# PaddlePaddle/Anakin

Hardware: AMD Instinct MI355X
Metric: ResNet50 INT8 images/sec + p50 latency @ batch 1/8, 1×MI355X (higher is better)
Workload: dtype int8

## Files before the change

### anakin_amd/csrc/api_chain.hip

```cpp
#include "api_internal.h"

enum : unsigned { CK_1X1 = 1, CK_3X3 = 2, CK_HEAD = 4, CK_PAIR = 8, CK_LED = CK_3X3 | CK_HEAD, CK_ANY = 15 };
static unsigned chain_kind(const saber_hip_chain* ch) { return !ch->c3 ? CK_1X1 : (ch->b2 ? CK_PAIR : (ch->b ? CK_3X3 : CK_HEAD)); }
static const struct { int c1; unsigned kinds; ChainForm f; } chain_forms[] = {
    {64, CK_ANY,            {4, 4, 4, 1, 1, CS_BASE, false}},
    {64, CK_ANY,            {2, 2, 4, 1, 1, CS_BASE, false}},
    {128, CK_1X1 | CK_LED,  {2, 2, 4, 1, 1, CS_BASE, false}},
    {128, CK_1X1 | CK_LED,  {1, 1, 4, 1, 1, CS_BASE, false}},
    {128, CK_1X1 | CK_LED,  {6, 2, 8, 1, 1, CS_W8, false}},
    {128, CK_1X1 | CK_LED,  {5, 1, 8, 1, 1, CS_W8, false}},
    {256, CK_1X1 | CK_LED,  {1, 1, 4, 1, 1, CS_BASE, false}},
    {256, CK_1X1,           {9, 1, 4, 2, 1, CS_SPLIT, false}},
    {256, CK_1X1,           {11, 1, 8, 2, 1, CS_SPLIT8, false}},
    {256, CK_LED,           {3, 1, 8, 1, 1, CS_W8, false}},
    {256, CK_3X3,           {7, 1, 8, 1, 2, CS_COOP2, true}},
    {256, CK_3X3,           {15, 2, 8, 1, 4, CS_COOP4, true}},
    {512, CK_1X1,           {1, 1, 4, 1, 1, CS_BASE, false}},
    {512, CK_1X1,           {9, 1, 4, 2, 1, CS_SPLIT, false}},
};
static void for_each_chain_form(const saber_hip_chain* ch, const std::function<void(const ChainForm&)>& fn) {
    for (const auto& r : chain_forms)
        if (r.c1 == ch->c1 && (r.kinds & chain_kind(ch))) fn(r.f);
}
static ChainForm chain_form_where(const saber_hip_chain* ch, const std::function<bool(const ChainForm& row, const ChainForm& found)>& take) {
    ChainForm f;
    for_each_chain_form(ch, [&](const ChainForm& c) { if (take(c, f)) f = c; });
    return f;
}
ChainForm chain_form(const saber_hip_chain* ch, int code) { return chain_form_where(ch, [&](const ChainForm& c, const ChainForm&) { return c.code == code; }); }
ChainForm chain_form_default(const saber_hip_chain* ch) { return chain_form_where(ch, [](const ChainForm&, const ChainForm& f) { return !f.code; }); }
ChainForm chain_form_plain(const saber_hip_chain* ch) { return chain_form_where(ch, [](const ChainForm& c, const ChainForm&) { return !c.placement; }); }
bool chain_form_valid(const saber_hip_chain* ch, int code) {
    const ChainForm f = chain_form(ch, code);
    return f.code && ch->d_stream[f.stream].p && (f.coop != 4 || ch->stage1);
}
std::string chain_form_name(const saber_hip_chain* ch) {
    const ChainForm& f = ch->form;
    const std::string c = std::to_string(ch->c1), w8 = f.waves == 8 && f.coop == 1 ? "_w8" : "";
    if (!ch->c3) return "chain1x1_c" + c + "_px" + std::to_string(16 * f.rows) + (f.split == 2 ? "_split2" : "") + w8;
    return std::string("conv3x3+") + (ch->b2 ? "conv1x1+pair1x1_c" : (ch->b ? "chain1x1_c" : "conv1x1_c")) + c + "_" + std::to_string(f.rows) + "x16" + w8 +
           (f.coop == 2 ? "_coop2" : "") + (f.coop == 4 ? "_coop4" : "");
}
void for_each_chain_candidate(const saber_hip_chain* ch, bool shared_device, const std::function<void(const ChainForm&)>& fn) {
    for_each_chain_form(ch, [&](const ChainForm& c) { if (!(shared_device && c.placement) && chain_form_valid(ch, c.code)) fn(c); });
}

static bool chain_1x1(const saber_hip_conv* o, bool sub_res_ok = false) {
    const saber_hip_conv_desc& d = o->d;
    return o->is_i8 && o->weights_set && !o->gpool && o->algo == ALGO_IGEMM_I8 && o->epi == EPI_I8_CONV && d.kh == 1 && d.kw == 1 &&
           d.stride_h == 1 && d.stride_w == 1 && d.pad_h == 0 && d.pad_w == 0 && d.group == 1 && !o->pair_k2 &&
           !o->pool_fused && !o->pool2 && !o->pre_quant && !o->pre_pad && o->c_eff == d.c && d.act_negative_slope == 0.f &&
           d.in_layout == SABER_HIP_NHWC && d.out_layout == SABER_HIP_NHWC && (d.res_stride <= 1 || sub_res_ok);
}
static void pack_chain_params(const saber_hip_conv* o, size_t chunks_pad, std::vector<uint8_t>& out) {
    const int K = o->d.k;
    out.assign(chunks_pad * 16, 0);
    for (int k4 = 0; k4 < K / 4; ++k4) {
        float* f = (float*)(out.data() + (size_t)k4 * 48);
        int* ip = (int*)(out.data() + (size_t)k4 * 48 + 32);
        for (int r = 0; r < 4; ++r) {
            const int k = k4 * 4 + r;
            f[r] = o->scale_host.empty() ? 1.f : o->scale_host[k];
            f[4 + r] = (o->has_bias && !o->bias_p_host.empty()) ? o->bias_p_host[k] : 0.f;
            ip[r] = o->comp_host.empty() ? 0 : o->comp_host[k];
        }
    }
}
static void pack_chain_weights(const int8_t* w, int K, int C, int mfg, int wave, std::vector<uint8_t>& out, int kbase = 0,
                               int nw = 4, int ks0 = 0) {
    const int kw = K / nw, groups = kw / (16 * mfg), ksn = C / 64;
    for (int g = 0; g < groups; ++g)
        for (int ksi = 0; ksi < ksn; ++ksi)
            for (int mf = 0; mf < mfg; ++mf) {
                const int ks = (ks0 + ksi) % ksn;
                for (int lane = 0; lane < 64; ++lane) {
                    const int rho = lane & 15, kq = lane >> 4;
                    const int ch = kbase + wave * kw + g * 16 * mfg + (rho >> 2) * 4 * mfg + mf * 4 + (rho & 3);
                    const int8_t* src = w + (size_t)ch * C + ks * 64 + kq * 16;
                    out.insert(out.end(), (const uint8_t*)src, (const uint8_t*)src + 16);
                }
            }
}
static void pack_chain_weights3(const int8_t* w, int C, int wave, std::vector<uint8_t>& out, int nw = 4, int kbase = 0, int kcount = 0) {
    const int kw = (kcount ? kcount : C) / nw, mf0 = kw / 16, ksn = C / 64;
    for (int tap = 0; tap < 9; ++tap)
        for (int ks = 0; ks < ksn; ++ks)
            for (int mf = 0; mf < mf0; ++mf)
                for (int lane = 0; lane < 64; ++lane) {
                    const int rho = lane & 15, kq = lane >> 4;
                    const int ch = kbase + wave * kw + (rho >> 2) * 4 * mf0 + mf * 4 + (rho & 3);
                    for (int t = 0; t < 16; ++t) {
                        const int c = ks * 64 + kq * 16 + t;
                        out.push_back((uint8_t)w[((size_t)ch * C + c) * 9 + tap]);
                    }
                }
}
static void pack_frag1(const int8_t* w, int C, int ch_base, int mfg, int mf, int ks, std::vector<uint8_t>& out) {
    for (int lane = 0; lane < 64; ++lane) {
        const int rho = lane & 15, kq = lane >> 4;
        const int8_t* src = w + (size_t)(ch_base + (rho >> 2) * 4 * mfg + mf * 4 + (rho & 3)) * C + ks * 64 + kq * 16;
        out.insert(out.end(), (const uint8_t*)src, (const uint8_t*)src + 16);
    }
}
static void pack_frag3(const int8_t* w, int C, int ch_base, int tap, int ks, std::vector<uint8_t>& out) {
    for (int lane = 0; lane < 64; ++lane) {
        const int rho = lane & 15, kq = lane >> 4;
        for (int t = 0; t < 16; ++t) out.push_back((uint8_t)w[((size_t)(ch_base + rho) * C + ks * 64 + kq * 16 + t) * 9 + tap]);
    }
}
static void pack_coop4_stream(const saber_hip_conv* c3, const saber_hip_conv* a, const saber_hip_conv* b, std::vector<uint8_t>& out) {
    const int C = 256, K1 = 1024;
    for (int q = 0; q < 4; ++q)
        for (int w = 0; w < 8; ++w) {
            const int nt = w & 3, kh = w >> 2;
            for (int tap = 0; tap < 9; ++tap)
                for (int kl = 0; kl < 2; ++kl) pack_frag3(c3->wq_oihw.data(), C, q * 64 + nt * 16, tap, kh * 2 + kl, out);
            for (int i = 0; i < 4; ++i)
                for (int mf = 0; mf < 2; ++mf) pack_frag1(a->wq_oihw.data(), C, q * 256 + w * 32, 2, mf, (q + i) & 3, out);
            for (int jj = 0; b && jj < 8; ++jj) {
                const int j = jj < 2 ? kh * 2 + jj : 4 + kh * 6 + (jj - 2);
                pack_frag1(b->wq_oihw.data(), K1, q * 64 + nt * 16, 1, 0, (q * 4 + j) & 15, out);
            }
        }
}
static void pack_stage_head_stream(const saber_hip_conv* a, const saber_hip_conv* b, std::vector<uint8_t>& out) {
    const int C0 = 512;
    for (int q = 0; q < 4; ++q)
        for (int w = 0; w < 8; ++w) {
            const int nt = w & 3, kh = w >> 2;
            for (int ks = 0; ks < 8; ++ks)
                for (int mf = 0; mf < 2; ++mf) pack_frag1(a->wq_oihw.data(), C0, q * 256 + w * 32, 2, mf, ks, out);
            for (int j = 0; j < 4; ++j) pack_frag1(b->wq_oihw.data(), C0, q * 64 + nt * 16, 1, 0, kh * 4 + j, out);
        }
}
static void pack_stage1_c128_stream(const saber_hip_conv* c3, const saber_hip_conv* a, const saber_hip_conv* b, std::vector<uint8_t>& out) {
    const int C = 128, K1 = 512;
    for (int w = 0; w < 8; ++w) {
        for (int tap = 0; tap < 9; ++tap)
            for (int ks = 0; ks < 2; ++ks) pack_frag3(c3->wq_oihw.data(), C, w * 16, tap, ks, out);
        for (int ks = 0; ks < 2; ++ks)
            for (int mf = 0; mf < 4; ++mf) pack_frag1(a->wq_oihw.data(), C, w * 64, 4, mf, ks, out);
        for (int ks = 0; ks < 8; ++ks) pack_frag1(b->wq_oihw.data(), K1, w * 16, 1, 0, ks, out);
    }
}
int saber_hip_conv2d_stem_pair_create(saber_hip_conv_t* stem, const saber_hip_conv_t* a, const saber_hip_conv_t* b, saber_hip_stem_pair_t** out) {
    if (!stem || !a || !b || !out) return fail(SABER_HIP_INVALID_VALUE, "null argument");
    const saber_hip_conv_desc& ds = stem->d;
    if (!stem->pool_fused || !stem->weights_set || ds.k != 64 || (ds.out_dtype != SABER_HIP_U8 && ds.out_dtype != SABER_HIP_S8))
        return fail(SABER_HIP_INVALID_VALUE, "stem pair: the head must be the fused stem conv + max pooling with 64 output channels (8-bit)");
    auto plain1x1 = [&](const saber_hip_conv* o) {
        const saber_hip_conv_desc& d = o->d;
        return o->is_i8 && o->weights_set && o->algo == ALGO_IGEMM_I8 && o->epi == EPI_I8_CONV && d.res_mode == SABER_HIP_RES_NONE &&
               !o->pair_k2 && !o->pool_fused && !o->pool2 && !o->pre_quant && !o->pre_pad && d.kh == 1 && d.kw == 1 && d.stride_h == 1 &&
               d.stride_w == 1 && d.pad_h == 0 && d.pad_w == 0 && d.group == 1 && d.c == 64 && o->c_eff == 64 && d.k % 32 == 0 &&
               d.in_layout == SABER_HIP_NHWC && d.out_layout == SABER_HIP_NHWC && d.act_negative_slope == 0.f &&
               (d.out_dtype == SABER_HIP_S8 || d.out_dtype == SABER_HIP_U8) && d.n == ds.n && d.h == stem->pool_oh && d.w == stem->pool_ow &&
               (o->x_dtype == DT_U8) == (ds.out_dtype == SABER_HIP_U8) && (int)o->wq_oihw.size() == d.k * 64;
    };
    if (!plain1x1(a) || !plain1x1(b) || a->d.k + b->d.k > 320)
        return fail(SABER_HIP_INVALID_VALUE, "stem pair: two plain 1x1 / stride-1 INT8 convs (64 -> k, k % 32 == 0, k_a + k_b <= 320, 8-bit NHWC outputs) "
                                              "on the pooled tensor");
    auto* sp = new saber_hip_stem_pair();
    sp->stem = stem; sp->a = a; sp->b = b;
    const int K1 = a->d.k, Kt = K1 + b->d.k;
    std::vector<int8_t> wcat((size_t)Kt * 64);
    std::memcpy(wcat.data(), a->wq_oihw.data(), (size_t)K1 * 64);
    std::memcpy(wcat.data() + (size_t)K1 * 64, b->wq_oihw.data(), (size_t)b->d.k * 64);
    std::vector<uint8_t> w, pa, pb, prm(256 * 16, 0);
    w.reserve((size_t)Kt * 64);
    for (int g = 0; g < Kt / 32; ++g)
        for (int mf = 0; mf < 2; ++mf) pack_frag1(wcat.data(), 64, g * 32, 2, mf, 0, w);
    pack_chain_params(a, (size_t)K1 / 4 * 3, pa);
    pack_chain_params(b, (size_t)b->d.k / 4 * 3, pb);
    std::memcpy(prm.data(), pa.data(), pa.size());
    std::memcpy(prm.data() + pa.size(), pb.data(), pb.size());
    hipError_t e = sp->d_w.upload(w);
    if (e == hipSuccess) e = sp->d_prm.upload(prm);
    if (e != hipSuccess) {
        delete sp;
        return hip_fail(e, "stem pair: device copies");
    }
    *out = sp;
    return SABER_HIP_OK;
}
void saber_hip_conv2d_stem_pair_destroy(saber_hip_stem_pair_t* sp) { delete sp; }
int saber_hip_conv2d_stem_pair_run(saber_hip_stem_pair_t* sp, const void* x, void* y_pool, void* y_a, void* y_b, void* workspace,
                                   saber_hip_stream_t stream) {
    if (g_capture) return capture_unsupported("saber_hip_conv2d_stem_pair_run (an executor-level object: saber_hip_net_optimize forms it itself)");
    if (!sp || !x || !y_a || !y_b) return fail(SABER_HIP_INVALID_VALUE, "null argument");
    saber_hip_conv* op = sp->stem;
    if (op->ws_bytes && !workspace) return fail(SABER_HIP_INVALID_VALUE, "workspace required");
    saber_mi355x::StemPairKArgs ka;
    const int rc = stem_pool_args(op, x, y_pool, workspace, (hipStream_t)stream, &ka.c);
    if (rc) return rc;
    ka.t.w = sp->d_w.p; ka.t.prm = sp->d_prm.p; ka.t.y1 = y_a; ka.t.y2 = y_b;
    ka.t.K1 = sp->a->d.k; ka.t.K2 = sp->b->d.k;
    ka.t.relu1 = sp->a->d.act == SABER_HIP_ACT_RELU; ka.t.relu2 = sp->b->d.act == SABER_HIP_ACT_RELU;
    ka.t.u8_1 = sp->a->d.out_dtype == SABER_HIP_U8; ka.t.u8_2 = sp->b->d.out_dtype == SABER_HIP_U8;
    HIP_TRY(saber_mi355x::launch_conv_stem_pool_pair(op->pre_quant ? 1 : 0, ka, (hipStream_t)stream));
    return SABER_HIP_OK;
}
saber_hip_chain::~saber_hip_chain() {
    if (h_coop_err) (void)hipHostFree(h_coop_err);
    delete stage1;
}
static unsigned div_magic(int d) { return d >= 2 ? (unsigned)((0x100000000ull + (unsigned)d - 1) / (unsigned)d) : 0u; }
static int stage_build(saber_hip_chain* const* chains, int n, bool per_image, saber_hip_chain* tail, saber_hip_chain_stage** out,
                       const saber_hip_conv* head_a = nullptr, const saber_hip_conv* head_b = nullptr) {
    if (!chains || n <= 0 || n > saber_mi355x::STAGE4_LONG || !out) return fail(SABER_HIP_INVALID_VALUE, "stage: 1..24 chains");
    if (head_a || head_b) {
        if (!head_a || !head_b) return fail(SABER_HIP_INVALID_VALUE, "null argument");
        if (!chains[0] || chains[0]->c1 != 256) return fail(SABER_HIP_INVALID_VALUE, "stage: a head goes with a C = 256 stage only");
        if (!per_image) return fail(SABER_HIP_INVALID_VALUE, "stage: a head needs an image per XCD");
        for (const saber_hip_conv* o : {head_a, head_b})
            if (o->d.res_mode != SABER_HIP_RES_NONE) return fail(SABER_HIP_INVALID_VALUE, "stage: the head's convs carry no residual");
        for (const saber_hip_conv* o : {head_a, head_b}) {
            const saber_hip_conv_desc& d = o->d;
            if (!o->is_i8 || !o->weights_set || o->algo != ALGO_IGEMM_I8 || o->epi != EPI_I8_CONV || o->pair_k2 || o->pool_fused || o->pool2 || o->gpool ||
                o->pre_quant || o->pre_pad || d.kh != 1 || d.kw != 1 || d.stride_h != 1 || d.stride_w != 1 || d.pad_h != 0 || d.pad_w != 0 || d.group != 1 ||
                o->c_eff != d.c || d.act_negative_slope != 0.f || d.in_layout != SABER_HIP_NHWC || d.out_layout != SABER_HIP_NHWC ||
                (d.out_dtype != SABER_HIP_S8 && d.out_dtype != SABER_HIP_U8))
                return fail(SABER_HIP_INVALID_VALUE, "stage: the head must be two plain 1x1 / stride 1 / pad 0 INT8 NHWC convs with weights set");
        }
        if (head_a->d.c != 512 || head_b->d.c != 512) return fail(SABER_HIP_INVALID_VALUE, "stage: the head's convs read 512 channels");
        if (head_a->d.k != 1024 || head_b->d.k != 256) return fail(SABER_HIP_INVALID_VALUE, "stage: the head's convs write 1024 and 256 channels");
        const saber_hip_conv_desc &d0 = chains[0]->a->d, &da = head_a->d, &db = head_b->d;
        if (!chains[0]->c3 || da.n != d0.n || da.h != d0.h || da.w != d0.w || db.n != d0.n || db.h != d0.h || db.w != d0.w || head_a->x_dtype != head_b->x_dtype ||
            da.out_dtype != SABER_HIP_S8 || (db.out_dtype == SABER_HIP_U8) != (chains[0]->c3->x_dtype == DT_U8))
            return fail(SABER_HIP_INVALID_VALUE, "stage: the head's outputs must be the first block's shortcut (s8) and 3x3 input (its dtype), one input tensor");
    }
    if (tail) {
        if (!chains[0] || chains[0]->c1 != 256 || tail->c1 != 256) return fail(SABER_HIP_INVALID_VALUE, "stage: a tail goes with a C = 256 stage only");
        if (n < 2 || !per_image || n + 1 > saber_mi355x::STAGE4_LONG) return fail(SABER_HIP_INVALID_VALUE, "stage: a tail needs 2..23 blocks, an image per XCD");
        if (!tail->c3 || tail->b || tail->b2 || tail->c3->d.stride_h != 2 || tail->c3->d.stride_w != 2)
            return fail(SABER_HIP_INVALID_VALUE, "stage: the tail must be a conv3x3 / stride 2 + conv1x1 chain without a second 1x1 conv");
        if (tail->a->d.res_stride != 2) return fail(SABER_HIP_INVALID_VALUE, "stage: the tail's shortcut must be sub-sampled by 2");
    }
    if (n > 1 && !per_image) return fail(SABER_HIP_INVALID_VALUE, "stage: several blocks need an image per XCD");
    if (n < 2 && chains[0] && chains[0]->c1 == 128) return fail(SABER_HIP_INVALID_VALUE, "stage: at C = 128 a stage is at least two blocks");
    const saber_hip_chain* c0 = chains[0];
    std::vector<saber_mi355x::StageBlk> blk;
    for (int k = 0; k < n; ++k) {
        const saber_hip_chain* ch = chains[k];
        const uint8_t* stream = !ch ? nullptr : (ch->c1 == 256 ? ch->d_stream[CS_COOP4].p : (ch->c1 == 128 ? ch->d_stream_stage1.p : nullptr));
        if (!ch || ch->c1 != c0->c1 || !ch->c3 || !ch->b || !stream || ch->c3->d.stride_h != 1)
            return fail(SABER_HIP_INVALID_VALUE, "stage: every block must be a conv3x3 (stride 1) + conv1x1 + conv1x1 chain at C = 256 (or all at C = 128)");
        const saber_hip_conv_desc& da = ch->a->d;
        if (da.n != c0->a->d.n || da.h != c0->a->d.h || da.w != c0->a->d.w) return fail(SABER_HIP_INVALID_VALUE, "stage: blocks of one tensor shape");
        if (k && ((ch->c3->x_dtype == DT_U8) != (chains[k - 1]->b->d.out_dtype == SABER_HIP_U8)))
            return fail(SABER_HIP_INVALID_VALUE, "stage: a block's 3x3 conv reads what the previous block's last conv writes");
        saber_mi355x::StageBlk B;
        std::memset(&B, 0, sizeof B);
        B.wstream = stream; B.prm0 = ch->d_prm0.p; B.prm1 = ch->d_prm1.p; B.prm2 = ch->d_prm2.p;
        B.coeff_conv = da.coeff_conv; B.scale_conv = ch->a->out_scale; B.coeff_res = da.coeff_res; B.scale_res = da.scale_res;
        B.in0_u8 = ch->c3->x_dtype == DT_U8; B.relu0 = ch->c3->d.act == SABER_HIP_ACT_RELU;
        B.in_u8 = ch->a->x_dtype == DT_U8; B.relu1 = da.act == SABER_HIP_ACT_RELU; B.res_relu = da.res_act == SABER_HIP_ACT_RELU;
        B.relu2 = ch->b->d.act == SABER_HIP_ACT_RELU; B.out_u8_2 = ch->b->d.out_dtype == SABER_HIP_U8;
        blk.push_back(B);
    }
    const saber_hip_conv_desc& d0 = c0->a->d;
    if (tail) {
        const saber_hip_conv_desc &d3 = tail->c3->d, &da = tail->a->d;
        if (d3.n != d0.n || d3.h != d0.h || d3.w != d0.w || da.res_h != d0.h || da.res_w != d0.w)
            return fail(SABER_HIP_INVALID_VALUE, "stage: the tail's 3x3 conv and shortcut read tensors of the blocks' shape");
        if ((tail->c3->x_dtype == DT_U8) != (chains[n - 1]->b->d.out_dtype == SABER_HIP_U8))
            return fail(SABER_HIP_INVALID_VALUE, "stage: the tail's 3x3 conv reads what the last block's last conv writes");
    }
    saber_hip_chain_stage* st = new saber_hip_chain_stage();
    st->chains.assign(chains, chains + n);
    st->c1 = c0->c1;
    st->n = d0.n; st->h = d0.h; st->w = d0.w;
    st->tiles_x = (d0.w + 15) / 16;
    st->tiles_per_img = st->tiles_x * ((d0.h + 1) / 2);
    st->per_image = per_image;
    const int wg_per_tile = st->c1 == 256 ? 4 : 1;
    const bool fits = d0.n <= 8 && st->tiles_per_img * wg_per_tile <= 32 &&
                      (st->c1 == 256 ? st->tiles_x == 1 : (st->tiles_x == 1 || st->tiles_x == 2 || st->tiles_x == 4));
    if ((per_image && !fits) || (st->c1 == 128 && !per_image)) {
        delete st;
        return fail(SABER_HIP_INVALID_VALUE, "stage: an image per XCD needs batch <= 8 and <= 32 workgroups per image (C = 256: width <= 16, <= 8 tiles "
                    "of 2 x 16 pixels; C = 128: width <= 64, <= 32 tiles)");
    }
    const size_t tiles = (size_t)d0.n * st->tiles_per_img;
    hipError_t e = hipSuccess;
    if (tail) {
        std::vector<uint8_t> ts;
        pack_coop4_stream(tail->c3, tail->a, nullptr, ts);
        e = st->d_tail_stream.upload(ts);
        const saber_hip_conv_desc& da = tail->a->d;
        saber_mi355x::StageBlk B;
        std::memset(&B, 0, sizeof B);
        B.wstream = st->d_tail_stream.p; B.prm0 = tail->d_prm0.p; B.prm1 = tail->d_prm1.p; B.prm2 = tail->d_prm0.p;
        B.coeff_conv = da.coeff_conv; B.scale_conv = tail->a->out_scale; B.coeff_res = da.coeff_res; B.scale_res = da.scale_res;
        B.in0_u8 = tail->c3->x_dtype == DT_U8; B.relu0 = tail->c3->d.act == SABER_HIP_ACT_RELU;
        B.in_u8 = tail->a->x_dtype == DT_U8; B.relu1 = da.act == SABER_HIP_ACT_RELU; B.res_relu = da.res_act == SABER_HIP_ACT_RELU;
        blk.push_back(B);
        st->tail = tail;
    }
    if (head_a) {
        std::vector<uint8_t> hs, p1, p2;
        pack_stage_head_stream(head_a, head_b, hs);
        pack_chain_params(head_a, (size_t)head_a->d.k / 4 * 3, p1);
        pack_chain_params(head_b, ((size_t)head_b->d.k / 4 * 3 + 63) / 64 * 64 + 64, p2);
        if (e == hipSuccess) e = st->d_head_stream.upload(hs);
        if (e == hipSuccess) e = st->d_head_prm1.upload(p1);
        if (e == hipSuccess) e = st->d_head_prm2.upload(p2);
        saber_mi355x::StageBlk B;
        std::memset(&B, 0, sizeof B);
        B.wstream = st->d_head_stream.p; B.prm0 = st->d_head_prm2.p; B.prm1 = st->d_head_prm1.p; B.prm2 = st->d_head_prm2.p;
        B.in_u8 = head_a->x_dtype == DT_U8; B.relu1 = head_a->d.act == SABER_HIP_ACT_RELU;
        B.relu2 = head_b->d.act == SABER_HIP_ACT_RELU; B.out_u8_2 = head_b->d.out_dtype == SABER_HIP_U8;
        blk.insert(blk.begin(), B);
        st->head_a = head_a; st->head_b = head_b;
    }
    if (e == hipSuccess) e = st->d_blk.upload(blk);
    if (e == hipSuccess && st->c1 == 256) e = st->d_grp_ctr.alloc_zero(tiles * 32);
    if (e == hipSuccess) e = st->d_img_ctr.alloc_zero((size_t)d0.n * (st->tiles_per_img + 1) * 16);
    if (e == hipSuccess) e = st->d_xcc.alloc_zero(tiles * 32);
    if (e == hipSuccess && st->c1 == 256) e = st->d_xch.alloc_zero(tiles * 32 * 256);
    if (e == hipSuccess) e = hipHostMalloc((void**)&st->h_err, sizeof(unsigned), hipHostMallocMapped);
    if (e != hipSuccess) {
        delete st;
        return hip_fail(e, "stage: device buffers");
    }
    *st->h_err = 0u;
    *out = st;
    return SABER_HIP_OK;
}
template <int MAXB>
static int stage_launch(saber_hip_chain_stage* st, const void* x, const void* res, void* const* y1, void* const* y2, void* y_tail, void* y_head, hipStream_t s) {
    saber_mi355x::Stage4KArgs<MAXB> k;
    std::memset(&k, 0, sizeof k);
    k.x = x; k.res = res; k.zero = zero_page();
    if (!k.zero) return fail(SABER_HIP_RUNTIME_ERROR, "stage: zero page");
    k.blk = st->d_blk.p + (st->head_a ? 1 : 0); k.grp_ctr = st->d_grp_ctr.p; k.img_ctr = st->d_img_ctr.p; k.xch = st->d_xch.p; k.xcc = st->d_xcc.p; k.err = st->h_err;
    k.nblk = (int)st->chains.size(); k.N = st->n; k.H = st->h; k.W = st->w;
    k.tiles_x = st->tiles_x; k.tiles_per_img = st->tiles_per_img;
    k.mg_tiles_x = div_magic(st->tiles_x); k.mg_tpi = div_magic(st->tiles_per_img); k.mg_wpi = div_magic(st->tiles_per_img * 4);
    k.per_image = st->per_image;
    for (int i = 0; i < k.nblk; ++i) { k.y1[i] = y1[i]; k.y2[i] = y2[i]; }
    if (y_tail) k.y1[k.nblk] = y_tail;
    k.head_y = y_head;
    HIP_TRY(st->c1 == 256 ? saber_mi355x::launch_conv_stage4(k, y_tail != nullptr, y_head != nullptr, s) : saber_mi355x::launch_conv_stage1_c128(k, s));
    return SABER_HIP_OK;
}
int stage_run(saber_hip_chain_stage* st, const void* x, const void* res, void* const* y1, void* const* y2, hipStream_t s, void* y_tail, void* y_head) {
    if (y_tail && !st->tail) return fail(SABER_HIP_INVALID_VALUE, "stage: created without a tail");
    if (y_head && !st->head_a) return fail(SABER_HIP_INVALID_VALUE, "stage: created without a head");
    if (*(volatile unsigned*)st->h_err) {
        *(volatile unsigned*)st->h_err = 0u;
        return fail(SABER_HIP_RUNTIME_ERROR, "cooperative stage: an earlier launch's workgroups did not share an XCD or timed out at a barrier "
                    "(its outputs are not valid)");
    }
    return (int)st->chains.size() + (y_tail ? 1 : 0) <= saber_mi355x::STAGE4_SHORT ? stage_launch<saber_mi355x::STAGE4_SHORT>(st, x, res, y1, y2, y_tail, y_head, s)
                                                                                   : stage_launch<saber_mi355x::STAGE4_LONG>(st, x, res, y1, y2, y_tail, y_head, s);
}
int saber_hip_conv2d_stage_create(saber_hip_chain_t* const* chains, int n, saber_hip_chain_stage_t** out) {
    if (!xcd_round_robin()) return fail(SABER_HIP_UNIMPL, "stage: this device does not place workgroup b on XCD b % 8");
    return stage_build(chains, n, true, nullptr, out);
}
int saber_hip_conv2d_stage_create_tail(saber_hip_chain_t* const* chains, int n, saber_hip_chain_t* tail, saber_hip_chain_stage_t** out) {
    if (!tail) return fail(SABER_HIP_INVALID_VALUE, "null argument");
    if (!xcd_round_robin()) return fail(SABER_HIP_UNIMPL, "stage: this device does not place workgroup b on XCD b % 8");
    return stage_build(chains, n, true, tail, out);
}
int saber_hip_conv2d_stage_create_head(saber_hip_chain_t* const* chains, int n, saber_hip_chain_t* tail, const saber_hip_conv_t* head_a,
                                       const saber_hip_conv_t* head_b, saber_hip_chain_stage_t** out) {
    if (!head_a || !head_b) return fail(SABER_HIP_INVALID_VALUE, "null argument");
    if (!xcd_round_robin()) return fail(SABER_HIP_UNIMPL, "stage: this device does not place workgroup b on XCD b % 8");
    return stage_build(chains, n, true, tail, out, head_a, head_b);
}
void saber_hip_conv2d_stage_destroy(saber_hip_chain_stage_t* st) { delete st; }
int saber_hip_conv2d_stage_run(saber_hip_chain_stage_t* st, const void* x, const void* res, void* const* y1, void* const* y2, saber_hip_stream_t stream) {
    if (g_capture) return capture_unsupported("saber_hip_conv2d_stage_run (saber_hip_net_optimize forms stages itself)");
    if (!st || !x || !res || !y1 || !y2) return fail(SABER_HIP_INVALID_VALUE, "null argument");
    for (size_t i = 0; i < st->chains.size(); ++i)
        if (!y1[i] || !y2[i]) return fail(SABER_HIP_INVALID_VALUE, "stage: an output pointer per block");
    return stage_run(st, x, res, y1, y2, (hipStream_t)stream);
}
int saber_hip_conv2d_stage_run_tail(saber_hip_chain_stage_t* st, const void* x, const void* res, void* const* y1, void* const* y2, void* y_tail,
                                    saber_hip_stream_t stream) {
    if (g_capture) return capture_unsupported("saber_hip_conv2d_stage_run_tail (saber_hip_net_optimize forms stages itself)");
    if (!st || !x || !res || !y1 || !y2 || !y_tail) return fail(SABER_HIP_INVALID_VALUE, "null argument");
    for (size_t i = 0; i < st->chains.size(); ++i)
        if (!y1[i] || !y2[i]) return fail(SABER_HIP_INVALID_VALUE, "stage: an output pointer per block");
    return stage_run(st, x, res, y1, y2, (hipStream_t)stream, y_tail);
}
int saber_hip_conv2d_stage_run_head(saber_hip_chain_stage_t* st, const void* x_head, void* y_head_b, void* const* y1, void* const* y2, void* y_tail,
                                    saber_hip_stream_t stream) {
    if (g_capture) return capture_unsupported("saber_hip_conv2d_stage_run_head (saber_hip_net_optimize forms stages itself)");
    if (!st || !x_head || !y_head_b || !y1 || !y2) return fail(SABER_HIP_INVALID_VALUE, "null argument");
    for (size_t i = 0; i < st->chains.size(); ++i)
        if (!y1[i] || !y2[i]) return fail(SABER_HIP_INVALID_VALUE, "stage: an output pointer per block");
    return stage_run(st, x_head, nullptr, y1, y2, (hipStream_t)stream, y_tail, y_head_b);
}
static void pack_chain_stream(const saber_hip_chain* ch, ChainStream layout, std::vector<uint8_t>& out) {
    const saber_hip_conv *c3 = ch->c3, *a = ch->a, *b = ch->b;
    const int c = ch->c1, k1 = ch->k1, k2 = ch->k2, c2 = b ? b->d.c : 0, k2w = k2 / 2;
    const int nw = layout == CS_BASE || layout == CS_SPLIT ? 4 : 8;
    const int8_t *w3 = c3 ? c3->wq_oihw.data() : nullptr, *wa = a->wq_oihw.data(), *wb = b ? b->wq_oihw.data() : nullptr;
    std::vector<int8_t> wcat;
    if (ch->b2) {
        wcat.assign(b->wq_oihw.begin(), b->wq_oihw.end());
        wcat.insert(wcat.end(), ch->b2->wq_oihw.begin(), ch->b2->wq_oihw.end());
        wb = wcat.data();
    }
    auto mfg = [&](int k) { return ch->b2 ? 2 : std::min(4, k / nw / 16); };
    switch (layout) {
    case CS_BASE: case CS_W8:
        for (int w = 0; w < nw; ++w) {
            if (c3) pack_chain_weights3(w3, c, w, out, nw);
            pack_chain_weights(wa, k1, c, 4, w, out, 0, nw);
            if (b) pack_chain_weights(wb, k2, c2, mfg(k2), w, out, 0, nw);
        }
        break;
    case CS_SPLIT: case CS_SPLIT8:
        for (int half = 0; half < 2; ++half)
            for (int w = 0; w < nw; ++w) {
                pack_chain_weights(wa, k1, c, 4, w, out, 0, nw);
                pack_chain_weights(wb, k2w, c2, mfg(k2w), w, out, half * k2w, nw);
            }
        break;
    case CS_COOP2:
        for (int half = 0; half < 2; ++half)
            for (int w = 0; w < nw; ++w) {
                pack_chain_weights3(w3, c, w, out, nw, half * (c / 2), c / 2);
                pack_chain_weights(wa, k1 / 2, c, 4, w, out, half * (k1 / 2), nw, half * (c / 128));
                pack_chain_weights(wb, k2w, c2, 1, w, out, half * k2w, nw, half * (c2 / 128));
            }
        break;
    default: pack_coop4_stream(c3, a, b, out);
    }
}
static int chain_build(saber_hip_conv* c3, saber_hip_conv* a, saber_hip_conv* b, saber_hip_chain_t** out, saber_hip_conv* b2 = nullptr) {
    if (!a || !out || (!b && !c3) || (b2 && (!b || !c3))) return fail(SABER_HIP_INVALID_VALUE, "null argument");
    const bool pair2 = b2 != nullptr;
    const bool strided = c3 && (!b || pair2) && c3->d.stride_h == 2 && c3->d.stride_w == 2;
    if (pair2 && !strided) return fail(SABER_HIP_INVALID_VALUE, "chain: a sibling pair follows the strided head (conv3x3 / stride 2 + conv1x1 + eltwise) only");
    if (!chain_1x1(a, strided) || (b && !chain_1x1(b)) || (b2 && !chain_1x1(b2)))
        return fail(SABER_HIP_INVALID_VALUE, "chain: both ops must be plain 1x1 stride-1 INT8 NHWC convs with weights set");
    if (strided != (a->d.res_stride > 1) || (strided && a->d.res_stride != 2))
        return fail(SABER_HIP_INVALID_VALUE, "chain: a stride-2 head goes with a shortcut sub-sampled by 2 (and only with one)");
    const saber_hip_conv_desc& da = a->d;
    if (da.res_mode != SABER_HIP_RES_ELTWISE || da.out_dtype != SABER_HIP_S8 || (da.res_has_dtype && da.res_dtype != SABER_HIP_S8))
        return fail(SABER_HIP_INVALID_VALUE, "chain: the first conv must carry the fused eltwise epilogue with s8 residual and output");
    if (b) {
        const saber_hip_conv_desc& db = b->d;
        if (db.res_mode != SABER_HIP_RES_NONE || b->x_dtype != DT_S8 || (db.out_dtype != SABER_HIP_S8 && db.out_dtype != SABER_HIP_U8))
            return fail(SABER_HIP_INVALID_VALUE, "chain: the second conv must be a plain s8-input conv with an 8-bit output");
        if (db.n != da.n || db.h != a->oh || db.w != a->ow || db.c != da.k || (!pair2 && db.k != da.c))
            return fail(SABER_HIP_INVALID_VALUE, "chain: shapes must be C -> 4C -> C with C in {64,128,256,512} on the same pixels");
    }
    if (pair2) {
        const saber_hip_conv_desc &db = b->d, &d2 = b2->d;
        if (d2.res_mode != SABER_HIP_RES_NONE || b2->x_dtype != DT_S8 || (d2.out_dtype != SABER_HIP_S8 && d2.out_dtype != SABER_HIP_U8) || d2.n != da.n ||
            d2.h != a->oh || d2.w != a->ow || d2.c != da.k || da.c != 64 || db.k % 32 || db.k + d2.k != 640 || d2.k <= 0)
            return fail(SABER_HIP_INVALID_VALUE, "chain: the sibling pair after a strided head: 64 -> 256 (+ eltwise) -> k_b | k_b2 with k_b + k_b2 = 640, k_b % 32 == 0, 8-bit outputs");
    }
    if (!conv1x1_chain_ok(da.c, da.k, da.c))
        return fail(SABER_HIP_INVALID_VALUE, "chain: shapes must be C -> 4C -> C with C in {64,128,256,512} on the same pixels");
    if (c3) {
        const saber_hip_conv_desc& d3 = c3->d;
        const bool ok = c3->is_i8 && c3->weights_set && c3->algo == ALGO_IGEMM_I8 && c3->epi == EPI_I8_CONV && d3.kh == 3 && d3.kw == 3 &&
                        d3.stride_h == (strided ? 2 : 1) && d3.stride_w == d3.stride_h && d3.pad_h == 1 && d3.pad_w == 1 && d3.dil_h == 1 && d3.dil_w == 1 &&
                        d3.group == 1 && !c3->pair_k2 && !c3->pool_fused && !c3->pool2 && !c3->pre_quant && !c3->pre_pad &&
                        c3->c_eff == d3.c && d3.act_negative_slope == 0.f && d3.in_layout == SABER_HIP_NHWC &&
                        d3.out_layout == SABER_HIP_NHWC && d3.res_mode == SABER_HIP_RES_NONE && d3.c == da.c && d3.k == da.c &&
                        d3.n == da.n && c3->oh == da.h && c3->ow == da.w && da.c <= 256 &&
                        (d3.out_dtype == SABER_HIP_S8 || d3.out_dtype == SABER_HIP_U8) &&
                        (d3.out_dtype == SABER_HIP_U8) == (a->x_dtype == DT_U8);
        if (!ok) return fail(SABER_HIP_INVALID_VALUE, "chain: the head must be the 3x3 pad-1 INT8 conv (C -> C, C <= 256; stride 1, or 2 in front of a lone 1x1 conv) whose 8-bit output the first 1x1 conv reads");
    }
    saber_hip_chain* ch = new saber_hip_chain();
    const int k2 = b ? b->d.k + (pair2 ? b2->d.k : 0) : 0;
    ch->c3 = c3; ch->a = a; ch->b = b; ch->b2 = b2; ch->c1 = da.c; ch->k1 = da.k; ch->k2 = k2;
    ch->form = chain_form_default(ch);
    std::vector<uint8_t> p0, p1, p2;
    hipError_t e = hipSuccess;
    for (int l = 0; l < CS_COUNT && e == hipSuccess; ++l) {
        bool needed = false;
        for_each_chain_form(ch, [&](const ChainForm& f) { needed = needed || (f.stream == l && (!f.placement || xcd_round_robin())); });
        if (!needed) continue;
        std::vector<uint8_t> stream;
        pack_chain_stream(ch, (ChainStream)l, stream);
        e = ch->d_stream[l].upload(stream);
    }
    pack_chain_params(a, (size_t)da.k / 4 * 3, p1);
    if (b) pack_chain_params(b, ((size_t)k2 / 4 * 3 + 63) / 64 * 64 + 64, p2);
    if (pair2) {
        std::vector<uint8_t> pb2;
        pack_chain_params(b2, (size_t)b2->d.k / 4 * 3, pb2);
        std::memcpy(p2.data() + (size_t)b->d.k / 4 * 48, pb2.data(), pb2.size());
    }
    if (e == hipSuccess && ch->d_stream[CS_COOP2].p) {
        ch->coop_tiles = da.n * da.h * ((da.w + 15) / 16);
        e = ch->d_coop_ctr.alloc_zero((size_t)ch->coop_tiles * 32);
        if (e == hipSuccess) e = ch->d_coop_xcc.alloc_zero((size_t)ch->coop_tiles * 32);
        if (e == hipSuccess) e = ch->d_coop_xch.alloc_zero((size_t)ch->coop_tiles * 16 * da.c);
        if (e == hipSuccess) e = hipHostMalloc((void**)&ch->h_coop_err, sizeof(unsigned), hipHostMallocMapped);
        if (e == hipSuccess) *ch->h_coop_err = 0u;
    }
    if (e == hipSuccess && da.c == 128 && c3 && b && c3->d.stride_h == 1 && xcd_round_robin()) {
        std::vector<uint8_t> s1;
        pack_stage1_c128_stream(c3, a, b, s1);
        e = ch->d_stream_stage1.upload(s1);
    }
    if (e == hipSuccess) e = ch->d_prm1.upload(p1);
    if (e == hipSuccess && b) e = ch->d_prm2.upload(p2);
    if (e == hipSuccess && c3) {
        pack_chain_params(c3, ((size_t)da.c / 4 * 3 + 63) / 64 * 64 + 64, p0);
        e = ch->d_prm0.upload(p0);
    }
    if (e != hipSuccess) {
        delete ch;
        return hip_fail(e, "chain: device copies");
    }
    if (ch->d_stream[CS_COOP4].p) {
        const int rc = stage_build(&ch, 1, false, nullptr, &ch->stage1);
        if (rc != SABER_HIP_OK) {
            delete ch;
            return rc;
        }
    }
    *out = ch;
    return SABER_HIP_OK;
}
int saber_hip_conv2d_chain_create(saber_hip_conv_t* a, saber_hip_conv_t* b, saber_hip_chain_t** out) {
    if (!b) return fail(SABER_HIP_INVALID_VALUE, "null argument");
    return chain_build(nullptr, a, b, out);
}
int saber_hip_conv2d_chain_create3(saber_hip_conv_t* conv3x3, saber_hip_conv_t* a, saber_hip_conv_t* b, saber_hip_chain_t** out) {
    if (!conv3x3) return fail(SABER_HIP_INVALID_VALUE, "null argument");
    return chain_build(conv3x3, a, b, out);
}
int saber_hip_conv2d_chain_create3_pair(saber_hip_conv_t* conv3x3, saber_hip_conv_t* a, saber_hip_conv_t* pair_a, saber_hip_conv_t* pair_b,
                                        saber_hip_chain_t** out) {
    if (!conv3x3 || !pair_a || !pair_b) return fail(SABER_HIP_INVALID_VALUE, "null argument");
    return chain_build(conv3x3, a, pair_a, out, pair_b);
}
void saber_hip_conv2d_chain_destroy(saber_hip_chain_t* ch) { delete ch; }
int saber_hip_conv2d_chain_set_tile(saber_hip_chain_t* ch, int tn) {
    if (!ch) return fail(SABER_HIP_INVALID_VALUE, "null argument");
    if (!chain_form_valid(ch, tn)) return fail(SABER_HIP_INVALID_VALUE, "chain: no kernel form with that code for this chain");
    ch->form = chain_form(ch, tn);
    return SABER_HIP_OK;
}
int saber_hip_conv2d_chain_get_tile(const saber_hip_chain_t* ch) { return ch ? ch->form.code : 0; }
int saber_hip_conv2d_chain_run(saber_hip_chain_t* ch, const void* x, const void* res, void* y_a, void* y_b,
                               saber_hip_stream_t stream) {
    return saber_hip_conv2d_chain_run3(ch, x, res, y_a, y_b, nullptr, stream);
}
int saber_hip_conv2d_chain_run3(saber_hip_chain_t* ch, const void* x, const void* res, void* y_a, void* y_b, void* y_c,
                                saber_hip_stream_t stream) {
    if (g_capture) return capture_unsupported("saber_hip_conv2d_chain_run (saber_hip_net_optimize forms chains itself)");
    if (!ch || !x || !res || !y_a || (ch->b && !y_b) || (ch->b2 && !y_c)) return fail(SABER_HIP_INVALID_VALUE, "null argument");
    const saber_hip_conv *a = ch->a, *b = ch->b;
    ChainKArgs k;
    std::memset(&k, 0, sizeof k);
    k.x = x; k.res = res;
    const ChainForm f = ch->form;
    k.wstream = ch->d_stream[f.stream].p;
    k.prm1 = ch->d_prm1.p;
    k.prm2 = ch->d_prm2.p;
    k.y1 = y_a; k.y2 = y_b;
    k.M = a->d.n * a->oh * a->ow;
    k.in_u8 = a->x_dtype == DT_U8;
    k.relu1 = a->d.act == SABER_HIP_ACT_RELU;
    k.res_relu = a->d.res_act == SABER_HIP_ACT_RELU;
    k.coeff_conv = a->d.coeff_conv; k.scale_conv = a->out_scale; k.coeff_res = a->d.coeff_res; k.scale_res = a->d.scale_res;
    if (b) {
        k.relu2 = b->d.act == SABER_HIP_ACT_RELU;
        k.out_u8_2 = b->d.out_dtype == SABER_HIP_U8;
    }
    if (ch->b2) {
        k.y2b = y_c;
        k.k2_split = b->d.k;
        k.relu2b = ch->b2->d.act == SABER_HIP_ACT_RELU;
        k.out_u8_2b = ch->b2->d.out_dtype == SABER_HIP_U8;
    }
    if (ch->c3) {
        k.prm0 = ch->d_prm0.p;
        k.zero = zero_page();
        if (!k.zero) return fail(SABER_HIP_RUNTIME_ERROR, "chain: zero page");
        k.N = a->d.n; k.H = a->d.h; k.W = a->d.w;
        k.tiles_x = (k.W + 15) / 16;
        k.tiles_per_img = k.tiles_x * ((k.H + f.rows - 1) / f.rows);
        k.mg_tiles_x = div_magic(k.tiles_x);
        k.mg_tpi = div_magic(k.tiles_per_img);
        k.in0_u8 = ch->c3->x_dtype == DT_U8;
        k.relu0 = ch->c3->d.act == SABER_HIP_ACT_RELU;
        k.s0 = ch->c3->d.stride_h;
        k.H0 = ch->c3->d.h; k.W0 = ch->c3->d.w;
        if (a->d.res_stride > 1) { k.res_sub = a->d.res_stride; k.res_H = a->d.res_h; k.res_W = a->d.res_w; }
    }
    if (f.coop == 4) {
        const int rc = stage_run(ch->stage1, x, res, &y_a, &y_b, (hipStream_t)stream);
        if (rc != SABER_HIP_OK) ch->form = chain_form_plain(ch);
        return rc;
    }
    if (f.coop == 2) {
        if (*(volatile unsigned*)ch->h_coop_err) {
            *(volatile unsigned*)ch->h_coop_err = 0u;
            ch->form = chain_form_plain(ch);
            return fail(SABER_HIP_RUNTIME_ERROR, "cooperative chain: an earlier launch's workgroup pairs did not share an XCD or timed out at their "
                        "barrier (its outputs are not valid); the chain now runs the single-workgroup form");
        }
        const CoopKArgs ck{k, ch->d_coop_ctr.p, ch->d_coop_xch.p, ch->d_coop_xcc.p, ch->h_coop_err, ch->coop_tiles};
        HIP_TRY(launch_conv_chain_coop(ck, (hipStream_t)stream));
        return SABER_HIP_OK;
    }
    HIP_TRY(launch_conv1x1_chain(k, ch->c1, ch->k1, ch->k2, f.rows, f.waves, f.split, ch->c3 ? 1 : 0, (hipStream_t)stream));
    return SABER_HIP_OK;
}
```

### anakin_amd/csrc/api_internal.h

```cpp
#pragma once
#include "../../include/saber_hip.h"
#include "kernels.h"

#include <cmath>
#include <cstdio>
#include <algorithm>
#include <cstdlib>
#include <cstring>
#include <functional>
#include <memory>
#include <mutex>
#include <string>
#include <utility>
#include <type_traits>
#include <vector>

using namespace saber_mi355x;

namespace saber_api {

extern thread_local std::string g_err;
inline int fail(int code, const std::string& msg) {
    g_err = msg;
    return code;
// ... 197 lines not shown
    DevBuf<uint8_t> d_head_stream, d_head_prm1, d_head_prm2;
    DevBuf<saber_mi355x::StageBlk> d_blk;
    DevBuf<unsigned long long> d_grp_ctr, d_img_ctr;
    DevBuf<uint8_t> d_xch;
    DevBuf<unsigned> d_xcc;
    unsigned* h_err = nullptr;
    int c1 = 0, n = 0, h = 0, w = 0, tiles_x = 0, tiles_per_img = 0;
    bool per_image = false;
    ~saber_hip_chain_stage() {
        if (h_err) (void)hipHostFree(h_err);
    }
};

struct saber_hip_sep {
    saber_hip_conv* dw = nullptr;
    saber_hip_conv* pw = nullptr;
    int form = 0;
    DevBuf<uint8_t> d_wdw, d_wpw, d_prm;
    DevBuf<float> d_dw_bias, d_dw_scale;
    std::string name;
};

struct saber_hip_ir {
    saber_hip_conv* expand = nullptr;
    saber_hip_conv* dw = nullptr;
    saber_hip_conv* project = nullptr;
    int form = 0;
    DevBuf<uint8_t> d_we, d_eprm, d_wdw, d_wp, d_pprm;
    DevBuf<float> d_dw_bias, d_dw_scale;
    std::string name;
};

struct saber_hip_fire {
    saber_hip_conv* squeeze = nullptr;
    saber_hip_conv* e1 = nullptr;
    saber_hip_conv* e3 = nullptr;
    int form = 0;
    DevBuf<uint8_t> d_ws, d_sprm, d_w1, d_prm1, d_w3, d_prm3;
    std::string name;
};

struct saber_hip_fc {
    saber_hip_fc_desc d;
    saber_hip_conv* conv = nullptr;
    bool pre_quant = false;
    float in_scale = 1.f;
};

namespace saber_api {
struct EventPair {
    hipEvent_t e0 = nullptr, e1 = nullptr;
    hipError_t init() {
        hipError_t e = hipEventCreate(&e0);
        return e != hipSuccess ? e : hipEventCreate(&e1);
    }
    ~EventPair() {
        if (e0) (void)hipEventDestroy(e0);
        if (e1) (void)hipEventDestroy(e1);
    }
};
struct ColdBench {
    size_t kBytes = (size_t)64 << 20;
    void* buf = nullptr;
    std::vector<hipEvent_t> ev;
    int reps = 0;
    hipError_t init(int r, size_t bytes = 0) {
        if (bytes) kBytes = std::min<size_t>(std::max<size_t>(bytes, (size_t)64 << 20), (size_t)512 << 20) & ~(size_t)0xfffff;
        reps = r < 3 ? 3 : (r > 32 ? 32 : r);
        hipError_t e = hipMalloc(&buf, kBytes + 256);
        if (e != hipSuccess) return e;
        e = hipMemset(buf, 1, kBytes + 256);
        if (e != hipSuccess) return e;
        ev.assign(2 * (size_t)reps, nullptr);
        for (hipEvent_t& x : ev)
            if ((e = hipEventCreate(&x)) != hipSuccess) return e;
        return hipStreamSynchronize(nullptr);
    }
    ~ColdBench() {
        for (hipEvent_t x : ev)
            if (x) (void)hipEventDestroy(x);
        if (buf) (void)hipFree(buf);
    }
    float run(hipStream_t s, const std::function<int()>& fn) {
        if (fn() != 0) return -1.f;
        for (int r = 0; r < reps; ++r) {
            if (launch_l2_flush(buf, kBytes, (unsigned*)((char*)buf + kBytes), s) != hipSuccess) return -1.f;
            if (hipEventRecord(ev[2 * r], s) != hipSuccess) return -1.f;
            if (fn() != 0) return -1.f;
            if (hipEventRecord(ev[2 * r + 1], s) != hipSuccess) return -1.f;
        }
        if (hipEventSynchronize(ev[2 * reps - 1]) != hipSuccess) return -1.f;
        std::vector<float> t(reps);
        for (int r = 0; r < reps; ++r)
            if (hipEventElapsedTime(&t[r], ev[2 * r], ev[2 * r + 1]) != hipSuccess) return -1.f;
        std::sort(t.begin(), t.end());
        return t[reps / 2] * 1000.f;
    }
};

extern thread_local ColdBench* g_cold;
int time_enqueued(hipStream_t s, const std::function<int()>& fn, int warm_iters, float* t);
extern thread_local std::vector<unsigned long long>* g_used_kernels;
constexpr float g_reuse_tol = 0.03f;
struct ColdScope {
    ColdBench local;
    bool owner = false;
    hipError_t enter(int reps, size_t flush_bytes = 0) {
        const char* w = std::getenv("SABER_HIP_AUTOTUNE_WARM");
        if (w && w[0] == '1') return hipSuccess;
        if (g_cold) return hipSuccess;
        hipError_t e = local.init(reps, flush_bytes);
        if (e != hipSuccess) return e;
        g_cold = &local;
        owner = true;
        return hipSuccess;
    }
    ~ColdScope() {
        if (owner) g_cold = nullptr;
    }
};

}

namespace saber_api {
enum OpKind { OP_CONV, OP_CONV_PAIR, OP_FC, OP_QUANT, OP_DEQUANT, OP_TRANSPOSE_IN, OP_ELT_I8, OP_ELT_F32, OP_POOL_I8, OP_POOL_F32, OP_POOL_F32_I8, OP_FC_Q, OP_SOFTMAX, OP_RELU_F32, OP_ACT_F32, OP_CONCAT };
enum Launch { LAUNCH_NONE, LAUNCH_OWN, LAUNCH_CHAIN, LAUNCH_CHAIN3, LAUNCH_STAGE, LAUNCH_STEM_PAIR, LAUNCH_SEP, LAUNCH_IR, LAUNCH_FIRE };
struct NetOp {
    OpKind kind;
    std::string name;
    saber_hip_conv* conv = nullptr;
    saber_hip_fc* fc = nullptr;
    int in = -1, in2 = -1, out = -1, out2 = -1;
    std::vector<int> ins, cat_c;
    std::vector<float> cat_m;
    Launch launch = LAUNCH_OWN;
    int absorbed_by = -1;
    bool skip = false;
    std::string res_note;
    saber_hip_chain* chain = nullptr;
    int chain_out = -1;
    bool chain_on = false;
    saber_hip_chain* chain3 = nullptr;
    int chain3_res = -1, chain3_y1 = -1, chain3_y2 = -1;
    int chain3_y3 = -1;
    bool led_on = false;
    saber_hip_chain_stage* stage = nullptr;
    int stage_n = 0;
    bool stage_on = false;
    bool stage_name_kept = false;
    bool tail_on = false;
    int tail_of = -1;
    bool head_on = false;
    int head_of = -1;
    saber_hip_stem_pair* stem_pair = nullptr;
    int stem_y1 = -1, stem_y2 = -1;
    saber_hip_sep* sep = nullptr;
    int sep_out = -1;
    bool sep_on = false;
    saber_hip_ir* ir = nullptr;
    int ir_out = -1;
    bool ir_on = false;
    saber_hip_fire* fire = nullptr;
    int fire_out = -1;
    bool fire_on = false;
    int lane = 0;
    bool record = false;
    int p[16] = {0};
    float f[6] = {0};
    size_t count = 0;
};
template <typename F>
inline void op_for_each_input(const NetOp& o, F&& f) {
    if (o.kind == OP_CONCAT) {
        for (int t : o.ins) f(t);
        return;
    }
    if (o.in >= 0) f(o.in);
    if (o.in2 >= 0) f(o.in2);
}
inline int op_reads(const NetOp& o, int t) {
    int n = 0;
    op_for_each_input(o, [&](int u) { n += u == t; });
    return n;
}
inline bool op_touches(const NetOp& o, int t) { return op_reads(o, t) || o.out == t || o.out2 == t; }
}

struct saber_hip_net {
    std::vector<size_t> tensor_bytes;
    std::vector<size_t> tensor_off;
    std::vector<void*> tensor_ext;
    std::vector<std::pair<const void*, int>> captured_ptr;
    void* ptr(int id) const {
        if (id < 0) return nullptr;
        if ((size_t)id < tensor_ext.size() && tensor_ext[id]) return tensor_ext[id];
        return (void*)(arena + tensor_off[id]);
    }
    std::vector<NetOp> ops;
    char* arena = nullptr;
    size_t arena_bytes = 0, ws_off = 0, ws_bytes = 0;
    hipGraph_t graph = nullptr;
    hipGraphExec_t exec = nullptr;
    bool finalized = false;
    bool compacted = false;
    bool shared_device = false;
    bool reproducible_fp32 = false;
    bool inplace_external = false;
    int coop_fallbacks = 0;
    hipStream_t side = nullptr;
    hipEvent_t ev_start = nullptr, ev_join = nullptr;
    std::vector<hipEvent_t> ev_op;
    std::vector<int> writer;
    bool lanes_ready = false, has_side = false;
    std::vector<saber_hip_conv*> owned;
    std::vector<saber_hip_chain*> owned_chains;
    std::vector<saber_hip_chain_stage*> owned_stages;
    std::vector<saber_hip_stem_pair*> owned_stem_pairs;
    std::vector<saber_hip_sep*> owned_seps;
    std::vector<saber_hip_ir*> owned_irs;
    std::vector<saber_hip_fire*> owned_fires;
};

namespace saber_api {
struct Capture;
extern thread_local Capture* g_capture;
int capture_conv(saber_hip_conv* op, const void* x, void* y, const void* res);
int capture_fc(saber_hip_fc* fc, const void* x, float* y, bool quantised_input);
int capture_unsupported(const char* what);
int capture_concat(size_t pixels, int n_inputs, const void* const* xs, const int* channels, const float* mult, int dtype, void* y);
int capture_stream_op(OpKind kind, const char* name, const int* p, int np, const float* f, int nf, size_t count, const void* in,
                      size_t in_bytes, const void* in2, size_t in2_bytes, void* out, size_t out_bytes, void* out2, size_t out2_bytes);
}

bool sel_valid(const saber_hip_conv* op, const saber_api::ConvSel& s);
int sel_set(saber_hip_conv* op, const saber_api::ConvSel& s);
void sel_release_unused(saber_hip_conv* op);
void sel_name(saber_hip_conv* op);
unsigned long long sel_kernel_key(const saber_hip_conv* op, const saber_api::ConvSel& s);
int sel_launch(saber_hip_conv* op, saber_mi355x::ConvKArgs& a, hipStream_t s);
void for_each_candidate(const saber_hip_conv* op, const saber_api::ConvSel* best, const std::function<void(const saber_api::ConvSel&)>& fn);
bool dw_ok(const saber_hip_conv* op);
bool group_ok(const saber_hip_conv* op);
bool stem_ok(const saber_hip_conv* op);
bool fc_small_ok(const saber_hip_conv* op);
bool b3_tile_ok(const saber_hip_conv* op, int tile, int ks);
int dw_static_form(const saber_hip_conv* op);
int group_static_form(const saber_hip_conv* op);
constexpr long DW_STRIP_MIN_LANES = 150000;
void conv_fill_args(const saber_hip_conv* op, saber_mi355x::ConvKArgs& a, const void* x, void* y, const void* res);
int stem_pool_args(const saber_hip_conv* op, const void* x, void* y, void* workspace, hipStream_t s, saber_mi355x::ConvKArgs* a);
bool xcd_round_robin();
int split_prepare(saber_hip_conv* op);
bool img_conv_ok(const saber_hip_conv* op);
int img_conv_prepare(saber_hip_conv* op);
int pw_prepare(saber_hip_conv* op);
bool pw_eligible(const saber_hip_conv* op);
int img_conv_run(saber_hip_conv* op, const void* x, void* y, const void* res, void* y_pool, hipStream_t stream);
void img_conv_release(saber_hip_conv* op);
int net_launch(saber_hip_net* net, const NetOp& o, hipStream_t s);
bool fc_softmax_ok(const saber_hip_fc* fc, bool quantised_input = false);
int fc_run_softmax(saber_hip_fc* fc, const void* x, float* y, float* prob, void* workspace, hipStream_t s, bool quantised_input);
int fc_softmax_prepare(saber_hip_fc* fc);
int concat_check(int n_inputs, const int* channels, const float* mult, int dtype, int* row_bytes);
void net_resolve(saber_hip_net* net);
void net_drop_graph(saber_hip_net* net);
void net_set_chain_mode(saber_hip_net* net, int ia, int mode);
int net_chain_mode(const saber_hip_net* net, int ia);
void net_set_stage(saber_hip_net* net, int i0, bool on);
void net_set_head(saber_hip_net* net, int i0, bool on);
void net_set_tail(saber_hip_net* net, int i0, bool on);
ChainForm chain_form(const saber_hip_chain* ch, int code);
bool chain_form_valid(const saber_hip_chain* ch, int code);
ChainForm chain_form_default(const saber_hip_chain* ch);
ChainForm chain_form_plain(const saber_hip_chain* ch);
std::string chain_form_name(const saber_hip_chain* ch);
void for_each_chain_candidate(const saber_hip_chain* ch, bool shared_device, const std::function<void(const ChainForm&)>& fn);
bool conv_sep_ok(const saber_hip_conv* dw, const saber_hip_conv* pw, std::string* why);
bool sep_form_valid(const saber_hip_sep* sp, int code);
void for_each_sep_form(const saber_hip_sep* sp, const std::function<void(int code)>& fn);
int sep_static_form(const saber_hip_sep* sp);
void net_set_sep(saber_hip_net* net, int i, int code);
bool conv_ir_ok(const saber_hip_conv* expand, const saber_hip_conv* dw, const saber_hip_conv* project, std::string* why);
bool ir_form_valid(const saber_hip_ir* ir, int code);
void for_each_ir_form(const saber_hip_ir* ir, const std::function<void(int code)>& fn);
int ir_static_form(const saber_hip_ir* ir);
void net_set_ir(saber_hip_net* net, int i, int code);
bool conv_fire_ok(const saber_hip_conv* squeeze, const saber_hip_conv* e1, const saber_hip_conv* e3, std::string* why);
bool fire_form_valid(const saber_hip_fire* fr, int code);
void for_each_fire_form(const saber_hip_fire* fr, const std::function<void(int code)>& fn);
int fire_static_form(const saber_hip_fire* fr);
void net_set_fire(saber_hip_net* net, int i, int code);
int stage_run(saber_hip_chain_stage* st, const void* x, const void* res, void* const* y1, void* const* y2, hipStream_t s, void* y_tail = nullptr,
              void* y_head = nullptr);
```

### anakin_amd/csrc/api_net.hip

```cpp
#include "api_internal.h"

#include <atomic>
static std::atomic<int> g_coop_fallbacks_total{0};

void net_drop_graph(saber_hip_net* net) {
    if (net->exec) (void)hipGraphExecDestroy(net->exec);
    if (net->graph) (void)hipGraphDestroy(net->graph);
    net->exec = nullptr;
    net->graph = nullptr;
}
int net_launch(saber_hip_net* net, const NetOp& o, hipStream_t s) {
    auto T = [&](int id) -> void* { return net->ptr(id); };
    void* ws = net->arena + net->ws_off;
    switch (o.kind) {
    case OP_CONV:
        switch (o.launch) {
        case LAUNCH_NONE: return SABER_HIP_OK;
        case LAUNCH_STAGE: {
            void* y1[saber_mi355x::STAGE4_LONG];
            void* y2[saber_mi355x::STAGE4_LONG];
            const NetOp* ops = &o;
            for (int k = 0; k < o.stage_n; ++k) {
                y1[k] = T(ops[3 * k].chain3_y1);
                y2[k] = T(ops[3 * k].chain3_y2);
            }
            void* const y_tail = o.tail_on ? T(ops[3 * o.stage_n].chain3_y1) : nullptr;
            const int rc = o.head_on ? stage_run(o.stage, T(ops[-1].in), nullptr, y1, y2, s, y_tail, T(o.in))
                                     : stage_run(o.stage, T(o.in), T(o.chain3_res), y1, y2, s, y_tail);
            if (rc == SABER_HIP_RUNTIME_ERROR) {
                ++net->coop_fallbacks;
                ++g_coop_fallbacks_total;
                net_set_stage(net, (int)(&o - net->ops.data()), false);
                net_drop_graph(net);
            }
            return rc;
        }
        case LAUNCH_STEM_PAIR: return saber_hip_conv2d_stem_pair_run(o.stem_pair, T(o.in), nullptr, T(o.stem_y1), T(o.stem_y2), ws, s);
        case LAUNCH_CHAIN3: {
            const int rc = saber_hip_conv2d_chain_run3(o.chain3, T(o.in), T(o.chain3_res), T(o.chain3_y1), T(o.chain3_y2), T(o.chain3_y3), s);
            if (rc == SABER_HIP_RUNTIME_ERROR) {
                ++net->coop_fallbacks;
                ++g_coop_fallbacks_total;
            }
            return rc;
        }
        case LAUNCH_CHAIN: return saber_hip_conv2d_chain_run(o.chain, T(o.in), T(o.in2), T(o.out), T(o.chain_out), s);
        case LAUNCH_SEP: return saber_hip_conv2d_sep_run(o.sep, T(o.in), nullptr, T(o.sep_out), s);
        case LAUNCH_IR: return saber_hip_conv2d_ir_run(o.ir, T(o.in), nullptr, nullptr, T(o.ir_out), s);
        case LAUNCH_FIRE: return saber_hip_conv2d_fire_run(o.fire, T(o.in), nullptr, T(o.fire_out), s);
        case LAUNCH_OWN: break;
        }
        if (o.conv->gpool) return saber_hip_conv2d_run_gpool(o.conv, T(o.in), T(o.out), T(o.in2), T(o.out2), s);
        return saber_hip_conv2d_run(o.conv, T(o.in), T(o.out), T(o.in2), ws, s);
    case OP_CONV_PAIR:
        if (o.skip) return SABER_HIP_OK;
        return saber_hip_conv2d_run_pair(o.conv, T(o.in), T(o.out), T(o.out2), s);
    case OP_FC:
        if (o.out2 >= 0) return fc_run_softmax(o.fc, T(o.in), (float*)T(o.out), (float*)T(o.out2), ws, s, false);
        return saber_hip_fc_run(o.fc, T(o.in), (float*)T(o.out), ws, s);
    case OP_QUANT:
        return saber_hip_quantize_nchw_to_nhwc(o.p[0], o.p[1], o.p[2], o.p[3], o.p[4], o.p[5], o.f[0],
                                               (const float*)T(o.in), T(o.out), s);
    case OP_DEQUANT:
        return saber_hip_dequantize_nhwc_to_nchw(o.p[0], o.p[1], o.p[2], o.p[3], o.p[4], o.f[0], T(o.in),
                                                 (float*)T(o.out), s);
    case OP_TRANSPOSE_IN:
        return saber_hip_transpose_nchw_to_nhwc_f32(o.p[0], o.p[1], o.p[2], o.p[3], o.p[4], (const float*)T(o.in),
                                                    (float*)T(o.out), s);
    case OP_ELT_I8:
        return saber_hip_eltwise_sum_i8(o.count, (const int8_t*)T(o.in), (const int8_t*)T(o.in2), o.f[0], o.f[1],
                                        o.f[2], o.f[3], o.p[0], (int8_t*)T(o.out), s);
    case OP_ELT_F32:
        return saber_hip_eltwise_sum_f32(o.count, (const float*)T(o.in), (const float*)T(o.in2), o.f[0], o.f[1],
                                         o.p[0], (float*)T(o.out), s);
    case OP_POOL_I8:
        return saber_hip_pool2d_i8_nhwc(o.p[0], o.p[1], o.p[2], o.p[3], o.p[4], o.p[5], o.p[6], o.p[7], o.p[8],
                                        o.p[9], o.p[10], o.p[11], o.p[12], o.p[13], o.p[14], T(o.in), T(o.out), s);
    case OP_POOL_F32:
        return saber_hip_pool2d_f32(o.p[0], o.p[1], o.p[2], o.p[3], o.p[4], o.p[5], o.p[6], o.p[7], o.p[8], o.p[9],
                                    o.p[10], o.p[11], o.p[12], o.p[13], (const float*)T(o.in), (float*)T(o.out), s);
    case OP_POOL_F32_I8:
        return saber_hip_pool2d_f32_from_i8_q(o.p[0], o.p[1], o.p[2], o.p[3], o.p[4], o.p[5], o.p[6], o.p[7], o.p[8],
                                              o.p[9], o.p[10], o.p[11], o.p[12], o.p[13], o.f[0], T(o.in),
                                              (float*)T(o.out), o.f[1], (int8_t*)T(o.out2), s);
    case OP_FC_Q:
        if (o.out2 >= 0) return fc_run_softmax(o.fc, T(o.in), (float*)T(o.out), (float*)T(o.out2), ws, s, true);
        return saber_hip_fc_run_q(o.fc, (const int8_t*)T(o.in), (float*)T(o.out), s);
    case OP_SOFTMAX:
        if (o.skip) return SABER_HIP_OK;
        return saber_hip_softmax_f32(o.p[0], o.p[1], (const float*)T(o.in), (float*)T(o.out), s);
    case OP_RELU_F32: return saber_hip_relu_f32(o.count, (const float*)T(o.in), (float*)T(o.out), s);
    case OP_ACT_F32: return saber_hip_activation_f32(o.p[0], o.count, o.f[0], o.f[1], (const float*)T(o.in), (float*)T(o.out), s);
    case OP_CONCAT: {
        if (o.skip) return SABER_HIP_OK;
        const void* xs[CONCAT_MAX_INPUTS];
        for (size_t k = 0; k < o.ins.size(); ++k) xs[k] = T(o.ins[k]);
        return saber_hip_concat_nhwc(o.count, (int)o.ins.size(), xs, o.cat_c.data(), o.cat_m.empty() ? nullptr : o.cat_m.data(), o.p[0], T(o.out), s);
    }
    }
    return SABER_HIP_UNIMPL;
}


int saber_hip_net_create(saber_hip_net_t** out) {
    *out = new saber_hip_net();
    return SABER_HIP_OK;
}
int saber_hip_net_add_tensor(saber_hip_net_t* net, size_t bytes) {
    net->tensor_bytes.push_back(bytes);
    net->tensor_ext.push_back(nullptr);
    return (int)net->tensor_bytes.size() - 1;
}
int saber_hip_net_num_tensors(const saber_hip_net_t* net) { return net ? (int)net->tensor_bytes.size() : 0; }
size_t saber_hip_net_tensor_bytes(const saber_hip_net_t* net, int id) {
    return (net && id >= 0 && id < (int)net->tensor_bytes.size()) ? net->tensor_bytes[id] : 0;
}
int saber_hip_net_bind_tensor(saber_hip_net_t* net, int id, void* ptr) {
    if (!net || id < 0 || id >= (int)net->tensor_bytes.size()) return fail(SABER_HIP_INVALID_VALUE, "bad tensor id");
    if (net->finalized && !ptr && !net->tensor_ext[id]) return SABER_HIP_OK;
    if (net->finalized && !net->tensor_ext[id]) return fail(SABER_HIP_INVALID_VALUE, "bind_tensor: an arena tensor cannot become external after finalize");
    if (net->finalized && !ptr) return fail(SABER_HIP_INVALID_VALUE, "bind_tensor: an external tensor has no arena slot to fall back to after finalize");
    net->tensor_ext[id] = ptr;
    net_drop_graph(net);
    return SABER_HIP_OK;
}
int saber_hip_net_tensor_of_ptr(const saber_hip_net_t* net, const void* ptr) {
    if (!net) return -1;
    for (const auto& pr : net->captured_ptr)
        if (pr.first == ptr) return pr.second;
    return -1;
}
static int push(saber_hip_net* net, NetOp&& o) {
    const int nt = (int)net->tensor_bytes.size();
    if (o.in >= nt || o.in2 >= nt || o.out >= nt || o.in < 0 || o.out < 0) return fail(SABER_HIP_INVALID_VALUE, "bad tensor id");
    net->ops.push_back(std::move(o));
    return (int)net->ops.size() - 1;
}
int saber_hip_net_add_conv(saber_hip_net_t* net, saber_hip_conv_t* op, int in_id, int out_id, int res_id) {
    NetOp o;
    o.kind = OP_CONV; o.conv = op; o.in = in_id; o.out = out_id; o.in2 = res_id;
    o.name = std::string("conv:") + op->algo_name;
    if (op->ws_bytes > net->ws_bytes) net->ws_bytes = op->ws_bytes;
    return push(net, std::move(o));
}
int saber_hip_net_add_conv_pair(saber_hip_net_t* net, saber_hip_conv_t* op, int in_id, int out_a_id, int out_b_id) {
    if (!op || !op->pair_k2) return fail(SABER_HIP_INVALID_VALUE, "not a sibling pair");
    if (out_b_id < 0 || out_b_id >= (int)net->tensor_bytes.size()) return fail(SABER_HIP_INVALID_VALUE, "bad tensor id");
    NetOp o;
    o.kind = OP_CONV_PAIR; o.conv = op; o.in = in_id; o.out = out_a_id; o.out2 = out_b_id;
    o.name = std::string("conv:") + op->algo_name;
    return push(net, std::move(o));
}
int saber_hip_net_add_fc(saber_hip_net_t* net, saber_hip_fc_t* op, int in_id, int out_id) {
    NetOp o;
    o.kind = OP_FC; o.fc = op; o.in = in_id; o.out = out_id;
    o.name = std::string("fc:") + op->conv->algo_name;
    const size_t w = saber_hip_fc_workspace_bytes(op);
    if (w > net->ws_bytes) net->ws_bytes = w;
    return push(net, std::move(o));
}
int saber_hip_net_add_quantize(saber_hip_net_t* net, int n, int c, int h, int w, int c_pad, int out_dtype, float scale,
                               int in_id, int out_id) {
    NetOp o;
    o.kind = OP_QUANT; o.in = in_id; o.out = out_id; o.name = "quantize_nchw_to_nhwc";
    o.p[0] = n; o.p[1] = c; o.p[2] = h; o.p[3] = w; o.p[4] = c_pad; o.p[5] = out_dtype; o.f[0] = scale;
    return push(net, std::move(o));
}
int saber_hip_net_add_dequantize(saber_hip_net_t* net, int n, int c, int h, int w, int in_dtype, float scale,
                                 int in_id, int out_id) {
    NetOp o;
    o.kind = OP_DEQUANT; o.in = in_id; o.out = out_id; o.name = "dequantize_nhwc_to_nchw";
    o.p[0] = n; o.p[1] = c; o.p[2] = h; o.p[3] = w; o.p[4] = in_dtype; o.f[0] = scale;
    return push(net, std::move(o));
}
int saber_hip_net_add_transpose_in_f32(saber_hip_net_t* net, int n, int c, int h, int w, int c_pad, int in_id,
                                       int out_id) {
// ... 337 lines not shown
}
int saber_hip_net_capture(saber_hip_net_t* net, saber_hip_stream_t stream) {
    hipStream_t s = (hipStream_t)stream;
    net_drop_graph(net);
    if (net_coop_error_pending(net)) return saber_hip_net_status(net);
    HIP_TRY(hipStreamBeginCapture(s, hipStreamCaptureModeThreadLocal));
    int rc = saber_hip_net_run(net, stream);
    hipError_t e = hipStreamEndCapture(s, &net->graph);
    if (rc == SABER_HIP_OK && e != hipSuccess) rc = hip_fail(e, "hipStreamEndCapture");
    if (rc == SABER_HIP_OK && (e = hipGraphInstantiate(&net->exec, net->graph, nullptr, nullptr, 0)) != hipSuccess) rc = hip_fail(e, "hipGraphInstantiate");
    if (rc != SABER_HIP_OK) net_drop_graph(net);
    return rc;
}
int saber_hip_net_replay(saber_hip_net_t* net, saber_hip_stream_t stream) {
    if (!net->exec) return fail(SABER_HIP_INVALID_VALUE, "net not captured");
    if (net_coop_error_pending(net)) return saber_hip_net_status(net);
    HIP_TRY(hipGraphLaunch(net->exec, (hipStream_t)stream));
    return SABER_HIP_OK;
}
int saber_hip_net_coop_fallbacks(const saber_hip_net_t* net) { return net ? net->coop_fallbacks : 0; }
int saber_hip_coop_fallbacks_total(void) { return g_coop_fallbacks_total.load(); }
static void conv_work(const saber_hip_conv* c, double& bytes, double& flops) {
    const saber_hip_conv_desc& d = c->d;
    const double esz_in = d.in_dtype == SABER_HIP_F32 ? 4 : 1, esz_out = d.out_dtype == SABER_HIP_F32 ? 4 : 1;
    const double esz_w = c->is_i8 ? 1 : 4;
    const double in_el = (double)d.n * d.h * d.w * d.c;
    const int oh = c->oh, ow = c->ow;
    const double out_el = (double)d.n * ((c->pool_fused || c->pool2) ? c->pool_oh * c->pool_ow : oh * ow) * d.k;
    bytes += in_el * esz_in + out_el * esz_out + (double)d.k * (d.c / d.group) * d.kh * d.kw * esz_w;
    if (d.res_mode != SABER_HIP_RES_NONE) bytes += (double)d.n * oh * ow * d.k * esz_out;
    flops += 2.0 * d.n * oh * ow * (double)d.k * (d.c / d.group) * d.kh * d.kw;
}
int saber_hip_net_op_work(const saber_hip_net_t* net, int index, double* bytes, double* flops) {
    if (!net || index < 0 || index >= (int)net->ops.size() || !bytes || !flops) return fail(SABER_HIP_INVALID_VALUE, "bad argument");
    *bytes = 0; *flops = 0;
    const NetOp& o = net->ops[index];
    auto tb = [&](int t) { return t >= 0 ? (double)net->tensor_bytes[t] : 0.0; };
    switch (o.kind) {
    case OP_CONV:
        if (o.skip) return SABER_HIP_OK;
        conv_work(o.conv, *bytes, *flops);
        for (int j = index + 1; j < (int)net->ops.size(); ++j)
            if (net->ops[j].absorbed_by == index && net->ops[j].conv) conv_work(net->ops[j].conv, *bytes, *flops);
        return SABER_HIP_OK;
    case OP_CONV_PAIR:
        if (!o.skip) conv_work(o.conv, *bytes, *flops);
        return SABER_HIP_OK;
    case OP_FC:
    case OP_FC_Q: {
        const saber_hip_fc_desc& d = o.fc->d;
        const double esz = d.int8_weights ? 1 : 4;
        *bytes = (double)d.m * d.k * (o.kind == OP_FC_Q || d.in_dtype != SABER_HIP_F32 ? 1 : 4) + (double)d.m * d.n * 4 + (double)d.n * d.k * esz;
        *flops = 2.0 * d.m * d.n * d.k;
        if (o.out2 >= 0) *bytes += 2.0 * tb(o.out2);
        return SABER_HIP_OK;
    }
    default:
        if (o.skip) return SABER_HIP_OK;
        *bytes = tb(o.out) + tb(o.out2);
        op_for_each_input(o, [&](int t) { *bytes += tb(t); });
        return SABER_HIP_OK;
    }
}
int saber_hip_net_time_pass(saber_hip_net_t* net, saber_hip_stream_t stream, int iters, float* out_us) {
    if (!net || !net->finalized || iters <= 0 || !out_us) return fail(SABER_HIP_INVALID_VALUE, "bad argument");
    hipStream_t s = (hipStream_t)stream;
    const size_t n = net->ops.size();
    struct Events {
        std::vector<hipEvent_t> v;
        ~Events() {
            for (hipEvent_t e : v)
                if (e) (void)hipEventDestroy(e);
        }
    } evs;
    evs.v.assign(n + 1, nullptr);
    std::vector<hipEvent_t>& ev = evs.v;
    for (auto& e : ev) HIP_TRY(hipEventCreate(&e));
    std::vector<double> acc(n, 0.0);
    for (int it = 0; it < iters + 1; ++it) {
        HIP_TRY(hipEventRecord(ev[0], s));
        size_t last = 0;
        std::vector<size_t> prev(n, 0);
        for (size_t i = 0; i < n; ++i) {
            const NetOp& o = net->ops[i];
            int rc = net_launch(net, o, s);
            if (rc) return rc;
            prev[i] = last;
            if (o.skip) continue;
            HIP_TRY(hipEventRecord(ev[i + 1], s));
            last = i + 1;
        }
        HIP_TRY(hipEventSynchronize(ev[last]));
        if (!it) continue;
        for (size_t i = 0; i < n; ++i) {
            const NetOp& o = net->ops[i];
            if (o.skip) continue;
            float ms = 0;
            HIP_TRY(hipEventElapsedTime(&ms, ev[prev[i]], ev[i + 1]));
            acc[i] += ms;
        }
    }
    for (size_t i = 0; i < n; ++i) out_us[i] = (float)(acc[i] * 1000.0 / iters);
    return SABER_HIP_OK;
}
int saber_hip_net_time_op_in_pass(saber_hip_net_t* net, saber_hip_stream_t stream, int index, int iters, float* out_us) {
    if (!net || !net->finalized || iters <= 0 || !out_us || index < 0 || index >= (int)net->ops.size())
        return fail(SABER_HIP_INVALID_VALUE, "bad argument");
    hipStream_t s = (hipStream_t)stream;
    EventPair evp;
    HIP_TRY(evp.init());
    double acc = 0.0;
    for (int it = 0; it < iters + 1; ++it) {
        for (size_t i = 0; i < net->ops.size(); ++i) {
            if ((int)i == index) HIP_TRY(hipEventRecord(evp.e0, s));
            int rc = net_launch(net, net->ops[i], s);
            if (rc) return rc;
            if ((int)i == index) HIP_TRY(hipEventRecord(evp.e1, s));
        }
        HIP_TRY(hipStreamSynchronize(s));
        float ms = 0;
        HIP_TRY(hipEventElapsedTime(&ms, evp.e0, evp.e1));
        if (it) acc += ms;
    }
    *out_us = (float)(acc * 1000.0 / iters);
    return SABER_HIP_OK;
}
int saber_hip_net_time_ops(saber_hip_net_t* net, saber_hip_stream_t stream, int iters, float* out_us) {
    hipStream_t s = (hipStream_t)stream;
    EventPair evp;
    HIP_TRY(evp.init());
    hipEvent_t e0 = evp.e0, e1 = evp.e1;
    for (size_t i = 0; i < net->ops.size(); ++i) {
        int rc = net_launch(net, net->ops[i], s);
        if (rc) return rc;
        HIP_TRY(hipEventRecord(e0, s));
        for (int it = 0; it < iters; ++it) net_launch(net, net->ops[i], s);
        HIP_TRY(hipEventRecord(e1, s));
        HIP_TRY(hipEventSynchronize(e1));
        float ms = 0;
        HIP_TRY(hipEventElapsedTime(&ms, e0, e1));
        out_us[i] = ms * 1000.f / iters;
    }
    return SABER_HIP_OK;
}
int saber_hip_net_tensor_unwritten(const saber_hip_net_t* net, int id) {
    if (id < 0 || id >= (int)net->tensor_bytes.size()) return 0;
    if (net->tensor_bytes[id] == 0) return 1;
    for (const NetOp& o : net->ops) {
        const Launch by = o.skip ? net->ops[o.absorbed_by].launch : o.launch;
        if (o.out == id && (o.launch == LAUNCH_CHAIN3 || o.launch == LAUNCH_STEM_PAIR || o.launch == LAUNCH_SEP || (o.chain3 && by == LAUNCH_STAGE))) return 1;
        if (o.out == id && (o.launch == LAUNCH_IR || (o.skip && by == LAUNCH_IR && (int)(&o - net->ops.data()) == o.absorbed_by + 1))) return 1;
        if (o.out == id && o.kind == OP_CONV && (o.launch == LAUNCH_FIRE || (o.skip && by == LAUNCH_FIRE))) return 1;
        if (o.launch == LAUNCH_STAGE && o.head_on && o.chain3_res == id) return 1;
    }
    return 0;
}
int saber_hip_net_status(saber_hip_net_t* net) {
    if (!net || !net->finalized) return fail(SABER_HIP_INVALID_VALUE, "net not finalized");
    int bad = 0;
    for (size_t i = 0; i < net->ops.size(); ++i) {
        NetOp& o = net->ops[i];
        if (o.stage && o.stage->h_err && *(volatile unsigned*)o.stage->h_err) {
            *(volatile unsigned*)o.stage->h_err = 0u;
            if (o.stage_on) net_set_stage(net, (int)i, false);
            ++bad;
        }
        saber_hip_chain* ch = o.chain3;
        if (ch) {
            unsigned* words[2] = {ch->h_coop_err, ch->stage1 ? ch->stage1->h_err : nullptr};
            for (unsigned* w : words)
                if (w && *(volatile unsigned*)w) {
                    *(volatile unsigned*)w = 0u;
                    if (ch->form.placement) ch->form = chain_form_plain(ch);
                    ++bad;
                }
        }
    }
    if (!bad) return SABER_HIP_OK;
    net->coop_fallbacks += bad;
    g_coop_fallbacks_total += bad;
    net_resolve(net);
    net_drop_graph(net);
    return fail(SABER_HIP_RUNTIME_ERROR, "a cooperative launch of the last pass did not complete (workgroups on different XCDs, or a hand-off "
                "timed out: another kernel held the CUs); its outputs are not valid - those sites now launch block by block: run the pass again");
}
int saber_hip_net_inject_coop_error(saber_hip_net_t* net) {
    if (!net) return fail(SABER_HIP_INVALID_VALUE, "null argument");
    for (NetOp& o : net->ops)
        if (o.stage && o.stage_on && o.stage->h_err) { *(volatile unsigned*)o.stage->h_err = 1u; return SABER_HIP_OK; }
    for (NetOp& o : net->ops) {
        if (o.stage && o.stage->h_err) { *(volatile unsigned*)o.stage->h_err = 1u; return SABER_HIP_OK; }
        if (o.chain3 && o.chain3->h_coop_err) { *(volatile unsigned*)o.chain3->h_coop_err = 1u; return SABER_HIP_OK; }
    }
    return fail(SABER_HIP_INVALID_VALUE, "the net has no cooperative launch site");
}
int saber_hip_net_num_launches(const saber_hip_net_t* net) {
    int n = 0;
    for (const NetOp& o : net->ops) n += o.skip ? 0 : 1;
    return n;
}
void saber_hip_net_destroy(saber_hip_net_t* net) {
    if (!net) return;
    net_drop_graph(net);
    if (net->arena) (void)hipFree(net->arena);
    for (saber_hip_stem_pair* sp : net->owned_stem_pairs) saber_hip_conv2d_stem_pair_destroy(sp);
    for (saber_hip_chain_stage* st : net->owned_stages) saber_hip_conv2d_stage_destroy(st);
    for (saber_hip_chain* c : net->owned_chains) saber_hip_conv2d_chain_destroy(c);
    for (saber_hip_sep* sp : net->owned_seps) saber_hip_conv2d_sep_destroy(sp);
    for (saber_hip_ir* ir : net->owned_irs) saber_hip_conv2d_ir_destroy(ir);
    for (saber_hip_fire* fr : net->owned_fires) saber_hip_conv2d_fire_destroy(fr);
    for (saber_hip_conv* c : net->owned) saber_hip_conv2d_destroy(c);
    for (hipEvent_t e : net->ev_op)
        if (e) (void)hipEventDestroy(e);
    if (net->ev_start) (void)hipEventDestroy(net->ev_start);
    if (net->ev_join) (void)hipEventDestroy(net->ev_join);
    if (net->side) (void)hipStreamDestroy(net->side);
    delete net;
}
```

### anakin_amd/csrc/api_net_autotune.hip

```cpp
#include "api_internal.h"

static saber_hip_conv* net_op_conv(saber_hip_net* net, int index) {
    if (index < 0 || index >= (int)net->ops.size()) return nullptr;
    NetOp& o = net->ops[index];
    if (o.kind == OP_CONV || o.kind == OP_CONV_PAIR) return o.conv;
    if (o.kind == OP_FC || o.kind == OP_FC_Q) return o.fc ? o.fc->conv : nullptr;
    return nullptr;
}
int saber_hip_net_get_choice(saber_hip_net_t* net, int index) {
    saber_hip_conv* c = net_op_conv(net, index);
    int choice = (c && !c->pool_fused && (c->algo <= ALGO_IGEMM_F32 || dw_ok(c) || group_ok(c))) ? saber_hip_conv2d_get_tile(c) : 0;
    if (!c) return choice;
    const NetOp& o = net->ops[index];
    if (o.chain) choice |= (1 << 28) | ((o.chain_on ? o.chain->form.code : 0) << 24);
    if (o.chain3) choice |= (1 << 29) | ((o.led_on ? o.chain3->form.code : 0) << 24);
    if (o.sep) choice |= (3 << 28) | ((o.sep_on ? o.sep->form : 0) << 24);
    if (o.ir) choice |= (int)0x80000000u | ((o.ir_on ? o.ir->form : 0) << 24);
    if (o.fire) choice |= (int)0x80000000u | ((o.fire_on ? o.fire->form : 0) << 24);
    if (o.stage && o.stage_on) choice |= 1 << 30;
    if (o.stage && o.stage_on && o.tail_on) choice |= (int)0x80000000u;
    if (o.head_of >= 0 && net->ops[o.head_of].stage_on && net->ops[o.head_of].head_on) choice |= 1 << 29;
    return choice;
}
int saber_hip_net_stage_blocks(const saber_hip_net_t* net, int index) {
    if (!net || index < 0 || index >= (int)net->ops.size()) return 0;
    return net->ops[index].stage ? net->ops[index].stage_n : 0;
}
int saber_hip_net_stage_head(const saber_hip_net_t* net, int index) {
    if (!net || index < 1 || index >= (int)net->ops.size() || !net->ops[index].stage) return -1;
    return net->ops[index - 1].head_of == index ? index - 1 : -1;
}
int saber_hip_net_set_choice(saber_hip_net_t* net, int index, int choice) {
    saber_hip_conv* c = net_op_conv(net, index);
    const bool ir_bits = c && net->ops[index].ir && ((unsigned)choice >> 30) == 2u;
    const int ir_tn = (choice >> 24) & 15;
    if (ir_bits && ir_tn && !ir_form_valid(net->ops[index].ir, ir_tn)) return saber_hip_conv2d_ir_set_tile(net->ops[index].ir, ir_tn);
    const bool fire_bits = c && net->ops[index].fire && ((unsigned)choice >> 30) == 2u;
    if (fire_bits && ir_tn && !fire_form_valid(net->ops[index].fire, ir_tn)) return saber_hip_conv2d_fire_set_tile(net->ops[index].fire, ir_tn);
    if (fire_bits && !(choice & 0xffffff)) {
        net_set_fire(net, index, ir_tn);
        net_drop_graph(net);
        return SABER_HIP_OK;
    }
    if (ir_bits && !(choice & 0xffffff)) {
        net_set_ir(net, index, ir_tn);
        net_drop_graph(net);
        return SABER_HIP_OK;
    }
    if (!c || !choice || c->pool_fused || (c->algo > ALGO_IGEMM_F32 && !dw_ok(c) && !group_ok(c))) return SABER_HIP_OK;
    if (net->reproducible_fp32 && !c->is_i8) return SABER_HIP_OK;
    if (net->ops[index].kind == OP_CONV_PAIR && index > 0 && net->ops[index - 1].stem_pair) return SABER_HIP_OK;
    const int chain_bits = (choice >> 24) & 63;
    const bool stage_on = ((choice >> 30) & 1) && !net->shared_device;
    const bool tail_on = stage_on && (((unsigned)choice >> 31) & 1u);
    choice &= 0xffffff;
    if (net->shared_device && ((choice >> 16) & 0xff) == 11) choice &= ~(0xf << 12);
    NetOp& o = net->ops[index];
    saber_hip_chain* ch = index + 1 >= (int)net->ops.size() ? nullptr : ((o.chain3 && (chain_bits & 32)) ? o.chain3 : ((o.chain && (chain_bits & 16)) ? o.chain : nullptr));
    int tn = chain_bits & 15;
    if (ch && net->shared_device && chain_form(ch, tn).placement) tn = chain_form_plain(ch).code;
    if (ch && tn && !chain_form_valid(ch, tn)) return saber_hip_conv2d_chain_set_tile(ch, tn);
    const bool sep_bits = o.sep && (chain_bits & 48) == 48;
    if (sep_bits && tn && !sep_form_valid(o.sep, tn)) return saber_hip_conv2d_sep_set_tile(o.sep, tn);
    int rc = choice ? saber_hip_conv2d_set_tile(c, choice) : SABER_HIP_OK;
    if (rc) return rc;
    o.res_note.clear();
    o.stage_name_kept = false;
    if (ch && tn) (void)saber_hip_conv2d_chain_set_tile(ch, tn);
    const bool in_stage = o.chain3 && o.skip && !o.stage && o.tail_of < 0;
    const int mode = ch ? net_chain_mode(net, ch == o.chain3 ? index + 1 : index) : 0;
    if (ch && ch == o.chain3) net_set_chain_mode(net, index + 1, (tn || in_stage) ? 2 : std::min(mode, 1));
    else if (ch) net_set_chain_mode(net, index, mode == 2 ? 2 : (tn ? 1 : 0));
    if (o.stage) net_set_stage(net, index, stage_on);
    if (o.stage) net_set_tail(net, index, tail_on);
    if (o.head_of >= 0) net_set_head(net, o.head_of, (chain_bits & 32) && !net->shared_device);
    if (sep_bits) net_set_sep(net, index, tn);
    if (ir_bits) net_set_ir(net, index, ir_tn);
    if (fire_bits) net_set_fire(net, index, ir_tn);
    net_resolve(net);
    net_drop_graph(net);
    return SABER_HIP_OK;
}

static int net_consolidate_kernels(saber_hip_net* net, hipStream_t s) {
    if (net->has_side) return SABER_HIP_OK;
    if (const char* e = std::getenv("SABER_HIP_NO_CONSOLIDATE"))
        if (e[0] == '1') return SABER_HIP_OK;
    struct Site { int op; unsigned long long key; ConvSel choice; };
    auto conv_of = [&](const NetOp& o) -> saber_hip_conv* {
        if (o.launch != LAUNCH_OWN) return nullptr;
        if (o.kind != OP_CONV && o.kind != OP_CONV_PAIR) return nullptr;
        if (net->reproducible_fp32 && o.conv && !o.conv->is_i8) return nullptr;
        return (o.conv && !o.conv->pool_fused && o.conv->algo <= ALGO_IGEMM_F32) ? o.conv : nullptr;
    };
    auto collect = [&]() {
        std::vector<Site> v;
        for (int i = 0; i < (int)net->ops.size(); ++i)
            if (saber_hip_conv* c = conv_of(net->ops[i])) v.push_back({i, sel_kernel_key(c, c->sel), c->sel});
        return v;
    };
    EventPair ev;
    HIP_TRY(ev.init());
    auto forward_ms = [&](float* ms) -> int {
        int rc = 0;
        for (int i = 0; i < 3 && !rc; ++i) rc = saber_hip_net_run(net, s);
        if (rc) return rc;
        HIP_TRY(hipEventRecord(ev.e0, s));
        for (int i = 0; i < 30 && !rc; ++i) rc = saber_hip_net_run(net, s);
        HIP_TRY(hipEventRecord(ev.e1, s));
        HIP_TRY(hipEventSynchronize(ev.e1));
        HIP_TRY(hipEventElapsedTime(ms, ev.e0, ev.e1));
        return rc;
    };
    std::vector<Site> sites = collect();
    for (size_t si = 0; si < sites.size(); ++si) {
        const Site cur = sites[si];
        if ((cur.key >> 8 & 0xff) != 5) continue;
        int uses = 0;
        for (const Site& t : sites) uses += t.key == cur.key;
        if (uses != 1) continue;
        saber_hip_conv* c = conv_of(net->ops[cur.op]);
        std::vector<Site> alts;
        for (const Site& t : sites) {
            if (t.op == cur.op || (t.key & 0xff) != (cur.key & 0xff) || (t.key >> 8 & 0xff) != 5 || t.key == cur.key) continue;
            if ((net->ops[t.op].kind == OP_CONV_PAIR) != (net->ops[cur.op].kind == OP_CONV_PAIR)) continue;
            bool dup = false;
            for (const Site& a : alts) dup |= a.key == t.key;
            if (!dup) alts.push_back(t);
        }
        if (alts.empty()) continue;
        float base = 0.f, base2 = 0.f;
        int rc = forward_ms(&base);
        if (rc) return rc;
        ConvSel best_c = cur.choice;
        float best = base;
        for (const Site& a : alts) {
            const ConvSel cc = sel_igemm(cur.choice, a.choice.tile, a.choice.ks, a.choice.dma);
            float ms = 0.f;
            if (sel_set(c, cc) != SABER_HIP_OK) continue;
            if (forward_ms(&ms) != SABER_HIP_OK) { (void)hipGetLastError(); continue; }
            if (ms < best) { best = ms; best_c = cc; }
        }
        (void)sel_set(c, cur.choice);
        if (best < base * 0.996f) {
            rc = forward_ms(&base2);
            if (rc) return rc;
            if (best < base2 * 0.996f) {
                (void)sel_set(c, best_c);
                net_resolve(net);
                sites = collect();
            }
        }
    }
    return saber_hip_net_run(net, s);
}

int saber_hip_net_autotune(saber_hip_net_t* net, saber_hip_stream_t stream, int iters) {
    if (net->inplace_external)
        return fail(SABER_HIP_INVALID_VALUE, "autotune: an in-place sum of this captured list accumulates into a tensor of the caller's that the "
                    "list itself never writes - timing passes would change it (run the pass that writes it inside the capture)");
    net_drop_graph(net);
    auto T = [&](int id) -> void* { return net->ptr(id); };
    ColdScope scope;
    HIP_TRY(scope.enter(iters < 7 ? 7 : (iters > 15 ? 15 : iters), net->arena_bytes > ((size_t)256 << 20) ? net->arena_bytes : 0));
    std::vector<unsigned long long> used_kernels;
    struct UsedScope {
        UsedScope(std::vector<unsigned long long>* v) { g_used_kernels = g_cold ? v : nullptr; }
        ~UsedScope() { g_used_kernels = nullptr; }
    } used_scope(&used_kernels);
    for (NetOp& o : net->ops) {
        if (o.kind == OP_CONV_PAIR && o.skip && &o != net->ops.data() && (&o)[-1].stem_pair) continue;
        if (net->reproducible_fp32 && o.conv && !o.conv->is_i8) continue;
        if (net->reproducible_fp32 && o.fc && o.fc->conv && !o.fc->conv->is_i8) continue;
        if (o.kind == OP_CONV_PAIR) {
            int rc = saber_hip_conv2d_autotune_pair(o.conv, T(o.in), T(o.out), T(o.out2), stream, iters);
            if (rc) return rc;
            continue;
        }
        saber_hip_conv* c = o.kind == OP_CONV ? o.conv : ((o.kind == OP_FC || o.kind == OP_FC_Q) ? o.fc->conv : nullptr);
        if (!c) continue;
        const void* xin = T(o.in);
        if (o.kind == OP_FC && o.fc->pre_quant) {
            int rq = net_launch(net, o, (hipStream_t)stream);
            if (rq) return rq;
            xin = net->arena + net->ws_off;
        }
        int rc = saber_hip_conv2d_autotune(c, xin, T(o.out), T(o.in2), net->arena + net->ws_off, stream, iters);
        if (rc) return rc;
        o.res_note.clear();
    }
    net_resolve(net);
    const char* log_env = std::getenv("SABER_HIP_AUTOTUNE_LOG");
    const bool log_cands = g_cold && log_env && log_env[0] == '1';
    auto log_cand = [&](const saber_hip_conv* c, const std::string& name, float t) {
        if (log_cands) std::fprintf(stderr, "autotune [%dx%dx%d c%d k%d %dx%d] %-40s %8.2f us\n", c->d.n, c->d.h, c->d.w, c->d.c, c->d.k, c->d.kh, c->d.kw, name.c_str(), t);
    };
    for (size_t i = 0; i < net->ops.size(); ++i)
        if (net->ops[i].stage) net_set_stage(net, (int)i, false);
    for (size_t i = 0; i < net->ops.size(); ++i) {
        NetOp& A = net->ops[i];
        const int ia = (int)i;
        NetOp* H = (ia > 0 && net->ops[ia - 1].chain3) ? &net->ops[ia - 1] : nullptr;
        if (!A.chain && !H) continue;
        const int first = H ? ia - 1 : ia;
        const int last = (A.chain || (H && H->chain3->b2)) ? ia + 1 : ia;
        hipStream_t s = (hipStream_t)stream;
        auto run_all = [&]() -> int {
            int rc = 0;
            for (int k = first; k <= last; ++k) rc |= net_launch(net, net->ops[k], s);
            return rc;
        };
        auto timed = [&](float* t) { return time_enqueued(s, run_all, 20, t); };
        float best = 0.f;
        int best_mode = 0, best_tn = 0;
        net_set_chain_mode(net, ia, 0);
        int rc = timed(&best);
        if (rc) return rc;
        log_cand(A.conv, "separate", best);
        for (int mode = A.chain ? 1 : 2; mode <= (H ? 2 : 1); ++mode) {
            saber_hip_chain* ch = mode == 2 ? H->chain3 : A.chain;
            for_each_chain_candidate(ch, net->shared_device, [&](const ChainForm& f) {
                float ms = -1.f;
                if (saber_hip_conv2d_chain_set_tile(ch, f.code) != SABER_HIP_OK) return;
                net_set_chain_mode(net, ia, mode);
                const int rt = timed(&ms);
                log_cand(A.conv, (mode == 2 ? H->name : A.name).substr(5), ms);
                if (rt == SABER_HIP_OK && ms < best) { best = ms; best_mode = mode; best_tn = f.code; }
            });
        }
        if (best_mode) (void)saber_hip_conv2d_chain_set_tile(best_mode == 2 ? H->chain3 : A.chain, best_tn);
        net_set_chain_mode(net, ia, best_mode);
        rc = run_all();
        if (rc) return rc;
    }
    for (size_t i = 0; i < net->ops.size(); ++i) {
        NetOp& H0 = net->ops[i];
        if (!H0.stage || net->shared_device) continue;
        const bool has_tail = H0.stage->tail != nullptr;
        const bool has_head = saber_hip_net_stage_head(net, (int)i) >= 0;
        const int first = (int)i, last = first + 3 * H0.stage_n - 1 + (has_tail ? 2 : 0);
        hipStream_t s = (hipStream_t)stream;
        auto run_all = [&]() -> int {
            int rc = 0;
            for (int k = first - (has_head ? 1 : 0); k <= last; ++k) rc |= net_launch(net, net->ops[k], s);
            return rc;
        };
        auto timed = [&](float* t) { return time_enqueued(s, run_all, 20, t); };
        std::vector<int> modes(H0.stage_n), tns(H0.stage_n);
        for (int k = 0; k < H0.stage_n; ++k) {
            modes[k] = net_chain_mode(net, first + 3 * k + 1);
            tns[k] = net->ops[first + 3 * k].chain3->form.code;
        }
        float sep = 0.f, one = 0.f;
        int rc = timed(&sep);
        if (rc) return rc;
        log_cand(H0.conv, "separate", sep);
        net_set_stage(net, first, true);
        net_set_tail(net, first, false);
        bool ok = timed(&one) == SABER_HIP_OK && hipStreamSynchronize(s) == hipSuccess && !*(volatile unsigned*)H0.stage->h_err;
        log_cand(H0.conv, H0.name.substr(5), ok ? one : -1.f);
        if (ok && has_tail) {
            float wt = 0.f;
            net_set_tail(net, first, true);
            const bool ok_t = timed(&wt) == SABER_HIP_OK && hipStreamSynchronize(s) == hipSuccess && !*(volatile unsigned*)H0.stage->h_err;
            log_cand(H0.conv, H0.name.substr(5), ok_t ? wt : -1.f);
            if (*(volatile unsigned*)H0.stage->h_err) ok = false;
            else if (ok_t && wt < one) one = wt;
            else net_set_tail(net, first, false);
        }
        if (ok && one < sep && has_head) {
            float wh = 0.f;
            net_set_head(net, first, true);
            const bool ok_h = timed(&wh) == SABER_HIP_OK && hipStreamSynchronize(s) == hipSuccess && !*(volatile unsigned*)H0.stage->h_err;
            log_cand(H0.conv, H0.name.substr(5), ok_h ? wh : -1.f);
            if (*(volatile unsigned*)H0.stage->h_err) ok = false;
            else if (ok_h && wh < one * 0.99f) one = wh;
            else net_set_head(net, first, false);
        }
        if (!ok || one >= sep) {
            *(volatile unsigned*)H0.stage->h_err = 0u;
            net_set_stage(net, first, false);
            for (int k = 0; k < H0.stage_n; ++k) {
                (void)saber_hip_conv2d_chain_set_tile(net->ops[first + 3 * k].chain3, tns[k]);
                net_set_chain_mode(net, first + 3 * k + 1, modes[k]);
            }
        }
        rc = run_all();
        if (rc) return rc;
    }
    for (size_t i = 0; i + 1 < net->ops.size(); ++i) {
        NetOp& D = net->ops[i];
        if (!D.sep) continue;
        hipStream_t s = (hipStream_t)stream;
        auto run_all = [&]() -> int { return net_launch(net, net->ops[i], s) | net_launch(net, net->ops[i + 1], s); };
        auto timed = [&](float* t) { return time_enqueued(s, run_all, 20, t); };
        float best = 0.f;
        int best_code = 0;
        net_set_sep(net, (int)i, 0);
        int rc = timed(&best);
        if (rc) return rc;
        log_cand(D.conv, "separate", best);
        for_each_sep_form(D.sep, [&](int code) {
            float us = -1.f;
            net_set_sep(net, (int)i, code);
            const int rt = timed(&us);
            log_cand(D.conv, D.name.substr(5), us);
            if (rt == SABER_HIP_OK && us < best) { best = us; best_code = code; }
        });
        net_set_sep(net, (int)i, best_code);
        rc = run_all();
        if (rc) return rc;
    }
    for (size_t i = 0; i + 2 < net->ops.size(); ++i) {
        NetOp& E = net->ops[i];
        if (!E.ir) continue;
        hipStream_t s = (hipStream_t)stream;
        auto run_all = [&]() -> int { return net_launch(net, net->ops[i], s) | net_launch(net, net->ops[i + 1], s) | net_launch(net, net->ops[i + 2], s); };
        auto timed = [&](float* t) { return time_enqueued(s, run_all, 20, t); };
        float best = 0.f;
        int best_code = 0;
        net_set_ir(net, (int)i, 0);
        int rc = timed(&best);
        if (rc) return rc;
        log_cand(E.conv, "separate", best);
        for_each_ir_form(E.ir, [&](int code) {
            float us = -1.f;
            net_set_ir(net, (int)i, code);
            const int rt = timed(&us);
            log_cand(E.conv, E.name.substr(5), us);
            if (rt == SABER_HIP_OK && us < best) { best = us; best_code = code; }
        });
        net_set_ir(net, (int)i, best_code);
        rc = run_all();
        if (rc) return rc;
    }
    for (size_t i = 0; i + 3 < net->ops.size(); ++i) {
        NetOp& Q = net->ops[i];
        if (!Q.fire) continue;
        hipStream_t s = (hipStream_t)stream;
        auto run_all = [&]() -> int {
            int r = 0;
            for (size_t j = i; j <= i + 3; ++j) r |= net_launch(net, net->ops[j], s);
            return r;
        };
        auto timed = [&](float* t) { return time_enqueued(s, run_all, 20, t); };
        float best = 0.f;
        int best_code = 0;
        net_set_fire(net, (int)i, 0);
        int rc = timed(&best);
        if (rc) return rc;
        log_cand(Q.conv, "separate", best);
        for_each_fire_form(Q.fire, [&](int code) {
            float us = -1.f;
            net_set_fire(net, (int)i, code);
            const int rt = timed(&us);
            log_cand(Q.conv, Q.name.substr(5), us);
            if (rt == SABER_HIP_OK && us < best) { best = us; best_code = code; }
        });
        net_set_fire(net, (int)i, best_code);
        rc = run_all();
        if (rc) return rc;
    }
    return g_cold ? net_consolidate_kernels(net, (hipStream_t)stream) : SABER_HIP_OK;
}
```

### anakin_amd/csrc/api_net_optimize.hip

```cpp
#include "api_internal.h"

void net_resolve(saber_hip_net* net) {
    std::vector<NetOp>& ops = net->ops;
    const int n = (int)ops.size();
    enum { IN_CHAIN, IN_STAGE, IN_STEM, IN_SEP, IN_IR, IN_FIRE };
    static const char* const covered[] = {"conv:(in the chain launch)", "conv:(in the stage launch)", "conv:(in the stem launch)", "conv:(in the separable launch)",
                                          "conv:(in the inverted-residual launch)", "conv:(in the fire launch)"};
    std::vector<int> in(n, IN_CHAIN);
    for (NetOp& o : ops) {
        o.launch = LAUNCH_OWN;
        o.absorbed_by = -1;
    }
    auto absorb = [&](int j, int by, int what) {
        ops[j].launch = LAUNCH_NONE;
        ops[j].absorbed_by = by;
        in[j] = what;
    };
    for (int i = 0; i < n; ++i) {
        NetOp& o = ops[i];
        if (o.launch == LAUNCH_NONE) continue;
        if ((o.kind == OP_FC || o.kind == OP_FC_Q) && o.out2 >= 0) {
            for (int j = i + 1; j < n; ++j)
                if (ops[j].kind == OP_SOFTMAX && ops[j].out == o.out2) { absorb(j, i, IN_CHAIN); break; }
        }
// ... 364 lines not shown
            if (P.kind != OP_CONV_PAIR || !P.conv || P.lane || P.in != S.out || !P.conv->pair_src_a || !P.conv->pair_src_b) continue;
            if (readers(S.out) != 1) continue;
            saber_hip_stem_pair* sp = nullptr;
            if (saber_hip_conv2d_stem_pair_create(S.conv, P.conv->pair_src_a, P.conv->pair_src_b, &sp) != SABER_HIP_OK) continue;
            net->owned_stem_pairs.push_back(sp);
            S.stem_pair = sp;
            S.stem_y1 = P.out;
            S.stem_y2 = P.out2;
            ++removed;
        }
        net_resolve(net);
    }
    bool two_lanes = false;
    for (const NetOp& o : ops) two_lanes |= o.lane != 0;
    if (two_lanes) flags &= ~(16 | 32);
    if ((flags & SABER_HIP_NET_FIRE) && !two_lanes) {
        auto free_op = [&](size_t j) {
            const NetOp& o = ops[j];
            if (o.chain || o.chain3 || o.stem_pair || o.sep || o.stage || o.skip || o.lane || in_ir(o)) return false;
            if (j > 0 && (ops[j - 1].chain || ops[j - 1].chain3 || ops[j - 1].stem_pair || ops[j - 1].sep)) return false;
            return !(j > 1 && ops[j - 2].chain3 != nullptr);
        };
        for (size_t i = 0; i + 3 < ops.size(); ++i) {
            NetOp& Q = ops[i];
            NetOp& A = ops[i + 1];
            NetOp& B = ops[i + 2];
            NetOp& K = ops[i + 3];
            if (Q.kind != OP_CONV || A.kind != OP_CONV || B.kind != OP_CONV || K.kind != OP_CONCAT || !Q.conv || !A.conv || !B.conv) continue;
            if (!free_op(i) || !free_op(i + 1) || !free_op(i + 2) || !free_op(i + 3)) continue;
            if (Q.in2 >= 0 || A.in2 >= 0 || B.in2 >= 0 || Q.out2 >= 0 || A.out2 >= 0 || B.out2 >= 0 || A.in != Q.out || B.in != Q.out) continue;
            if (K.ins.size() != 2 || K.ins[0] != A.out || K.ins[1] != B.out || K.p[0] != SABER_HIP_U8) continue;
            bool copy = true;
            for (float m : K.cat_m) copy = copy && m == 1.0f;
            if (!copy || readers(Q.out) != 2 || readers(A.out) != 1 || readers(B.out) != 1) continue;
            if (K.cat_c[0] != A.conv->d.k || K.cat_c[1] != B.conv->d.k || K.count != (size_t)Q.conv->d.n * Q.conv->oh * Q.conv->ow) continue;
            saber_hip_fire* fr = nullptr;
            if (saber_hip_conv2d_fire_create(Q.conv, A.conv, B.conv, &fr) != SABER_HIP_OK) continue;
            net->owned_fires.push_back(fr);
            Q.fire = fr;
            Q.fire_out = K.out;
            net_set_fire(net, (int)i, fire_static_form(fr));
            ++removed;
            i += 3;
        }
    }
    if ((flags & SABER_HIP_NET_INVERTED_RESIDUAL) && !two_lanes) {
        auto taken = [&](size_t j) {
            const NetOp& o = ops[j];
            if (o.chain || o.chain3 || o.stem_pair || o.sep || o.stage || in_ir(o)) return true;
            if (j > 0 && (ops[j - 1].chain || ops[j - 1].chain3 || ops[j - 1].stem_pair || ops[j - 1].sep)) return true;
            return j > 1 && ops[j - 2].chain3 != nullptr;
        };
        for (size_t i = 0; i + 2 < ops.size(); ++i) {
            NetOp& E = ops[i];
            NetOp& D = ops[i + 1];
            NetOp& P = ops[i + 2];
            if (E.kind != OP_CONV || D.kind != OP_CONV || P.kind != OP_CONV || !E.conv || !D.conv || !P.conv || E.skip || D.skip || P.skip || E.lane ||
                D.lane || P.lane || E.in2 >= 0 || D.in2 >= 0 || E.out2 >= 0 || D.out2 >= 0 || P.out2 >= 0 || D.in != E.out || P.in != D.out)
                continue;
            if (taken(i) || taken(i + 1) || taken(i + 2)) continue;
            if (readers(E.out) != 1 || readers(D.out) != 1) continue;
            const bool elt = P.conv->d.res_mode == SABER_HIP_RES_ELTWISE;
            if (elt ? P.in2 != E.in : P.in2 >= 0) continue;
            saber_hip_ir* ir = nullptr;
            if (saber_hip_conv2d_ir_create(E.conv, D.conv, P.conv, &ir) != SABER_HIP_OK) continue;
            net->owned_irs.push_back(ir);
            E.ir = ir;
            E.ir_out = P.out;
            net_set_ir(net, (int)i, ir_static_form(ir));
            ++removed;
            i += 2;
        }
    }
    if ((flags & SABER_HIP_NET_SEPARABLE) && !two_lanes) {
        for (size_t i = 0; i + 1 < ops.size(); ++i) {
            NetOp& D = ops[i];
            NetOp& P = ops[i + 1];
            if (D.kind != OP_CONV || P.kind != OP_CONV || !D.conv || !P.conv || D.sep || D.skip || P.skip || D.lane || P.lane || D.chain || D.chain3 ||
                D.stem_pair || P.chain || P.chain3 || P.stem_pair || P.sep || in_ir(D) || in_ir(P) || D.in2 >= 0 || P.in2 >= 0 || D.out2 >= 0 || P.out2 >= 0 || P.in != D.out)
                continue;
            if (!D.conv->is_i8 || !dw_ok(D.conv)) continue;
            if (readers(D.out) != 1) continue;
            saber_hip_sep* sp = nullptr;
            if (saber_hip_conv2d_sep_create(D.conv, P.conv, &sp) != SABER_HIP_OK) continue;
            net->owned_seps.push_back(sp);
            D.sep = sp;
            D.sep_out = P.out;
            net_set_sep(net, (int)i, sep_static_form(sp));
            ++removed;
        }
    }
    if (flags & 16) {
        for (size_t i = 0; i + 1 < ops.size(); ++i) {
            NetOp& A = ops[i];
            NetOp& B = ops[i + 1];
            if (A.kind != OP_CONV || B.kind != OP_CONV || !A.conv || !B.conv || A.chain || A.skip || B.chain || A.lane || B.lane ||
                A.chain3 || B.chain3 || in_ir(A) || in_ir(B))
                continue;
            if (A.conv->d.res_mode != SABER_HIP_RES_ELTWISE || B.in != A.out || A.in2 < 0 || B.in2 >= 0) continue;
            saber_hip_chain* ch = nullptr;
            if (saber_hip_conv2d_chain_create(A.conv, B.conv, &ch) != SABER_HIP_OK) continue;
            net->owned_chains.push_back(ch);
            A.chain = ch;
            A.chain_out = B.out;
            net_set_chain_mode(net, (int)i, ch->c1 <= 256 ? 1 : 0);
            if (A.chain_on) ++removed;
        }
    }
    if (flags & 32) {
        for (size_t i = 0; i + 2 < ops.size(); ++i) {
            NetOp& Hd = ops[i];
            NetOp& A = ops[i + 1];
            NetOp& B = ops[i + 2];
            if (!A.chain || Hd.kind != OP_CONV || !Hd.conv || Hd.chain3 || Hd.chain || Hd.skip || Hd.lane || Hd.in2 >= 0 ||
                A.in != Hd.out)
                continue;
            if (readers(Hd.out) != 1) continue;
            saber_hip_chain* ch = nullptr;
            if (saber_hip_conv2d_chain_create3(Hd.conv, A.conv, B.conv, &ch) != SABER_HIP_OK) continue;
            net->owned_chains.push_back(ch);
            Hd.chain3 = ch;
            Hd.chain3_res = A.in2; Hd.chain3_y1 = A.out; Hd.chain3_y2 = B.out;
            const bool was = A.chain_on;
            net_set_chain_mode(net, (int)i + 1, ch->c1 <= 128 ? 2 : (was ? 1 : 0));
            if (Hd.led_on) removed += was ? 1 : 2;
        }
        for (size_t i = 0; i + 1 < ops.size(); ++i) {
            NetOp& Hd = ops[i];
            NetOp& A = ops[i + 1];
            if (A.chain || A.skip || A.kind != OP_CONV || !A.conv || A.conv->d.res_mode != SABER_HIP_RES_ELTWISE || A.in2 < 0 || A.lane ||
                Hd.kind != OP_CONV || !Hd.conv || Hd.chain3 || Hd.chain || Hd.skip || Hd.lane || Hd.in2 >= 0 || A.in != Hd.out || in_ir(Hd) || in_ir(A))
                continue;
            if (readers(Hd.out) != 1) continue;
            saber_hip_chain* ch = nullptr;
            NetOp* P = (flags & 1024) && i + 2 < ops.size() ? &ops[i + 2] : nullptr;
            if (P && (P->kind != OP_CONV_PAIR || P->lane || P->skip || P->in != A.out || !P->conv || !P->conv->pair_src_a || !P->conv->pair_src_b)) P = nullptr;
            if (P) {
                if (readers(A.out) != 1 || saber_hip_conv2d_chain_create3_pair(Hd.conv, A.conv, const_cast<saber_hip_conv*>(P->conv->pair_src_a),
                                                                   const_cast<saber_hip_conv*>(P->conv->pair_src_b), &ch) != SABER_HIP_OK)
                    P = nullptr;
            }
            if (!P && saber_hip_conv2d_chain_create3(Hd.conv, A.conv, nullptr, &ch) != SABER_HIP_OK) continue;
            net->owned_chains.push_back(ch);
            Hd.chain3 = ch;
            Hd.chain3_res = A.in2; Hd.chain3_y1 = A.out; Hd.chain3_y2 = P ? P->out : -1; Hd.chain3_y3 = P ? P->out2 : -1;
            net_set_chain_mode(net, (int)i + 1, ch->c1 <= 128 ? 2 : 0);
            if (Hd.led_on) removed += P ? 2 : 1;
        }
    }
    if ((flags & 256) && (flags & 32) && !two_lanes) {
        for (size_t i = 0; i + 2 < ops.size();) {
            auto block_ok = [&](size_t j) {
                return j + 2 < ops.size() && ops[j].chain3 && ops[j].chain3->b && !ops[j].stage && ops[j].chain3_y2 >= 0 &&
                       ((ops[j].chain3->c1 == 256 && ops[j].chain3->stage1) || (ops[j].chain3->c1 == 128 && ops[j].chain3->d_stream_stage1.p));
            };
            if (!block_ok(i)) { ++i; continue; }
            std::vector<saber_hip_chain*> run{ops[i].chain3};
            while ((int)run.size() < saber_mi355x::STAGE4_LONG) {
                const size_t p = i + 3 * (run.size() - 1), j = p + 3;
                if (!block_ok(j) || ops[j].chain3->c1 != run[0]->c1 || ops[j].in != ops[p].chain3_y2 || ops[j].chain3_res != ops[p].chain3_y1) break;
                run.push_back(ops[j].chain3);
            }
            if (run.size() >= 2) {
                saber_hip_chain_stage* st = nullptr;
                const size_t pl = i + 3 * (run.size() - 1), jt = pl + 3;
                saber_hip_chain* tail = nullptr;
                if (jt + 1 < ops.size() && run[0]->c1 == 256 && ops[jt].chain3 && !ops[jt].chain3->b && !ops[jt].chain3->b2 && !ops[jt].stage &&
                    ops[jt].chain3->c1 == 256 && ops[jt].chain3->c3->d.stride_h == 2 && ops[jt].in == ops[pl].chain3_y2 &&
                    ops[jt].chain3_res == ops[pl].chain3_y1 && ops[jt].chain3_y1 >= 0)
                    tail = ops[jt].chain3;
                const saber_hip_conv *head_a = nullptr, *head_b = nullptr;
                if (i >= 1 && run[0]->c1 == 256 && ops[i - 1].kind == OP_CONV_PAIR && !ops[i - 1].skip && !ops[i - 1].lane && ops[i - 1].conv &&
                    ops[i - 1].conv->pair_src_a && ops[i - 1].conv->pair_src_b && !(i >= 3 && ops[i - 3].chain3 && ops[i - 3].chain3->b2)) {
                    const NetOp& P = ops[i - 1];
                    const int t_res = ops[i].chain3_res, t_x = ops[i].in;
                    const bool fwd = P.out == t_res && P.out2 == t_x, rev = P.out == t_x && P.out2 == t_res;
                    if ((fwd || rev) && t_res != t_x && readers(t_res) == 1 && readers(t_x) == 1) {
                        head_a = fwd ? P.conv->pair_src_a : P.conv->pair_src_b;
                        head_b = fwd ? P.conv->pair_src_b : P.conv->pair_src_a;
                    }
                }
                if (head_a && saber_hip_conv2d_stage_create_head(run.data(), (int)run.size(), tail, head_a, head_b, &st) != SABER_HIP_OK) head_a = head_b = nullptr;
                if (!head_a && tail && saber_hip_conv2d_stage_create_tail(run.data(), (int)run.size(), tail, &st) != SABER_HIP_OK) tail = nullptr;
                if (head_a || tail || saber_hip_conv2d_stage_create(run.data(), (int)run.size(), &st) == SABER_HIP_OK) {
                    net->owned_stages.push_back(st);
                    ops[i].stage = st;
                    ops[i].stage_n = (int)run.size();
                    if (tail) ops[jt].tail_of = (int)i;
                    if (head_a) ops[i - 1].head_of = (int)i;
                    int before = 0;
                    for (size_t k = 0; k < run.size(); ++k) before += 3 - (ops[i + 3 * k].skip + ops[i + 3 * k + 1].skip + ops[i + 3 * k + 2].skip);
                    if (tail) before += 2 - (ops[jt].skip + ops[jt + 1].skip);
                    const bool on = run[0]->a->d.n >= 4 && run[0]->c1 == 256;
                    net_set_stage(net, (int)i, on);
                    if (on) removed += before - 1;
                }
            }
            i += 3 * run.size();
        }
    }
    if (flags & 4096) {
        for (size_t i = 0; i + 1 < ops.size(); ++i) {
            NetOp& F = ops[i];
            if (dead[i] || (F.kind != OP_FC && F.kind != OP_FC_Q) || !F.fc || F.out2 >= 0 || F.lane) continue;
            size_t j = i + 1;
            while (j < ops.size() && dead[j]) ++j;
            if (j >= ops.size()) break;
            NetOp& S = ops[j];
            if (S.kind != OP_SOFTMAX || S.in != F.out || S.skip || S.lane || S.p[0] != F.fc->d.m || S.p[1] != F.fc->d.n) continue;
            if (F.kind == OP_FC && F.fc->pre_quant) continue;
            if (!fc_softmax_ok(F.fc, F.kind == OP_FC_Q) || fc_softmax_prepare(F.fc) != SABER_HIP_OK) continue;
            F.out2 = S.out;
            ++removed;
        }
    }
    if (net->shared_device) {
        for (NetOp& o : ops) {
            saber_hip_conv* c = (o.kind == OP_FC || o.kind == OP_FC_Q) ? (o.fc ? o.fc->conv : nullptr) : o.conv;
            if (c) {
                c->no_placement = true;
                if (c->sel.fam == FAM_B3 && c->sel.ksplit) (void)sel_set(c, sel_b3(c->sel, c->sel.tile, c->sel.ks, 0));
            }
            for (saber_hip_chain* ch : {o.chain, o.chain3})
                if (ch && ch->form.placement) ch->form = chain_form_plain(ch);
        }
    }
    net_resolve(net);
    net->ws_bytes = 0;
    for (const NetOp& o : ops) {
        size_t w = 0;
        if ((o.kind == OP_CONV) && o.conv) w = o.conv->ws_bytes;
        if (o.kind == OP_FC && o.fc) w = saber_hip_fc_workspace_bytes(o.fc);
        if (w > net->ws_bytes) net->ws_bytes = w;
    }
    return removed;
}
```

### anakin_amd/csrc/conv_stage_coop.hip

```cpp
#include "coop_sync.h"

namespace saber_mi355x {

template <int MAXB, bool TAIL, bool HEAD>
__global__ __launch_bounds__(512) void conv_stage4_c256_kernel(const Stage4KArgs<MAXB> ka) {
    constexpr int C1 = 256, K1 = 1024, K2 = 256, NW = 8;
    constexpr int F0 = 18, F1 = 8, F2 = 8;
    constexpr int FB = F0 + F1 + F2, FT = F0 + F1;
    constexpr int K0Q = C1 / 4, K1Q = K1 / 4, K2Q = K2 / 4;
    constexpr int CH1 = C1 / 16, PCH = CH1 + 1, HW = 18, HP = 4 * HW;
    constexpr int HCH = (HP * PCH + 63) / 64 * 64;
    constexpr int CPRW = K1Q / 16;
    constexpr int P0C = (K0Q / 4 * 3 + 63) / 64 * 64, P1C = K1Q / 4 * 3, P2C = (K2Q / 4 * 3 + 63) / 64 * 64;
    constexpr int MPC = K0Q / 16 + 1;
    constexpr int YPC = (K1 - K1Q) / 16 + 1;
    constexpr int YCH = (32 * YPC + 63) / 64 * 64;
    static_assert(P1C % 64 == 0 && (32 * CPRW) == 64 * NW, "DMA granularity");
    __shared__ v4i halo[HCH];
    __shared__ v4i tile[32 * CPRW];
    __shared__ v4i ptile[YCH];
    __shared__ v4i mid_own[32 * MPC];
    __shared__ v4i red[4 * 2 * 64];
    __shared__ v4i prm0[P0C];
    __shared__ v4i prm1[P1C];
// ... 592 lines not shown
    wait_vm_older_than<F0 + 2>();
    __builtin_amdgcn_s_barrier();
    SABER_TL(1);
    unsigned my_xcc;
    asm volatile("s_getreg_b32 %0, hwreg(HW_REG_XCC_ID)" : "=s"(my_xcc));
    my_xcc = (my_xcc & 7u) + 1u;
    if (rem == 0 && tid == 0) ka.xcc[(size_t)t * 32 + 4] = my_xcc;

    StageBlk B = ka.blk[0];
    for (int k = 0; k < ka.nblk; ++k) {
        const v4i z = {0, 0, 0, 0};
        v4i fs[F1 - 2 + F2];
        {
            const v4i* wsb = stream_of(B);
#pragma unroll
            for (int r = 0; r < F1 - 2 + F2; ++r) {
                fs[r] = wsb[(F0 + 2 + r) * 64];
                asm volatile("" ::: "memory");
            }
        }
        {
            const int xm0 = B.in0_u8 ? (int)0x80808080u : 0;
            const int c0 = wave * 16 + fq * 4;
            const v4i* pp = prm0 + (c0 / 4) * 3;
            v4i acc0 = pp[2], acc1 = acc0;
            const v4i* hb = halo + frow * PCH + fq;
#pragma unroll
            for (int s = 0; s < F0; ++s) {
                const int kl = s % 2, tap = s / 2;
                const int dy = tap / 3, dx = tap % 3;
                v4i b0 = hb[(dy * HW + dx) * PCH + kl * 4];
                v4i b1 = hb[((dy + 1) * HW + dx) * PCH + kl * 4];
                b0.x ^= xm0; b0.y ^= xm0; b0.z ^= xm0; b0.w ^= xm0;
                b1.x ^= xm0; b1.y ^= xm0; b1.z ^= xm0; b1.w ^= xm0;
                acc0 = mma_step(fr[s], b0, acc0);
                acc1 = mma_step(fr[s], b1, acc1);
            }
            const float lo0 = B.relu0 ? 0.f : -3.0e38f;
            const float off0 = B.in_u8 ? 0.f : 128.f;
            const unsigned xo0 = B.in_u8 ? 0u : 0x80808080u;
            const unsigned o0 = chain_out_pack(acc0, z, __builtin_bit_cast(v4f, pp[1]), __builtin_bit_cast(v4f, pp[0]), lo0, off0, xo0);
            const unsigned o1 = chain_out_pack(acc1, z, __builtin_bit_cast(v4f, pp[1]), __builtin_bit_cast(v4f, pp[0]), lo0, off0, xo0);
            *(unsigned*)((char*)mid + frow * (MPC * 16) + c0) = o0;
            *(unsigned*)((char*)mid + (16 + frow) * (MPC * 16) + c0) = o1;
        }
        asm volatile("s_waitcnt lgkmcnt(0)" ::: "memory");
        __builtin_amdgcn_s_barrier();
        SABER_TL(2);

        {
            const int xmask = B.in_u8 ? (int)0x80808080u : 0;
            const int cg = wave * 64 + fq * 16;
            const v4i* pp = prm1 + (cg / 4) * 3;
            v4i acc[2][4];
#pragma unroll
            for (int m = 0; m < 2; ++m)
#pragma unroll
                for (int mf = 0; mf < 4; ++mf) acc[m][mf] = pp[mf * 3 + 2];
#pragma unroll
            for (int ks = 0; ks < 2; ++ks)
#pragma unroll
                for (int m = 0; m < 2; ++m) {
                    v4i bo = mid[(m * 16 + frow) * MPC + ks * 4 + fq];
                    bo.x ^= xmask; bo.y ^= xmask; bo.z ^= xmask; bo.w ^= xmask;
#pragma unroll
                    for (int mf = 0; mf < 4; ++mf) {
                        const int f = ks * 4 + mf;
                        acc[m][mf] = mma_step(f < 2 ? fr[F0 + f] : fs[f - 2], bo, acc[m][mf]);
                    }
                }
            const float lo_s8 = B.relu1 ? 0.f : -128.f;
            const float res_lo = B.res_relu ? 0.f : -3.0e38f;
#pragma unroll
            for (int m = 0; m < 2; ++m) {
                v4i* tp = tile + (m * 16 + frow) * CPRW + ((cg / 16) ^ frow);
                const v4i rs = *tp;
                v4i o;
                o.x = (int)chain_elt_pack(acc[m][0], z, __builtin_bit_cast(v4f, pp[1]), __builtin_bit_cast(v4f, pp[0]), (unsigned)rs.x, lo_s8, res_lo, B);
                o.y = (int)chain_elt_pack(acc[m][1], z, __builtin_bit_cast(v4f, pp[4]), __builtin_bit_cast(v4f, pp[3]), (unsigned)rs.y, lo_s8, res_lo, B);
                o.z = (int)chain_elt_pack(acc[m][2], z, __builtin_bit_cast(v4f, pp[7]), __builtin_bit_cast(v4f, pp[6]), (unsigned)rs.z, lo_s8, res_lo, B);
                o.w = (int)chain_elt_pack(acc[m][3], z, __builtin_bit_cast(v4f, pp[10]), __builtin_bit_cast(v4f, pp[9]), (unsigned)rs.w, lo_s8, res_lo, B);
                *tp = o;
            }
        }
        asm volatile("s_waitcnt lgkmcnt(0)" ::: "memory");
        __builtin_amdgcn_s_barrier();
#pragma unroll
        for (int j = 0; j < 32 * CPRW / 512; ++j) {
            const int L = tid + j * 512;
            const int px = L / CPRW, c = (L % CPRW) ^ (px & 15);
            bool okp;
            const int pp_ = pix(px, okp);
            if (okp) *(v4i*)((char*)ka.y1[k] + (size_t)pp_ * K1 + c * 16) = tile[L];
        }
        SABER_TL(4);
        const StageBlk Bn = ka.blk[k + 1 < ka.nblk ? k + 1 : k];
        if (k + 1 < ka.nblk) {
            const v4i* wsb = stream_of(Bn);
#pragma unroll
            for (int r = 0; r < F0 + 2; ++r) {
                fr[r] = wsb[r * 64];
                asm volatile("" ::: "memory");
            }
        }

        {
            const int c2 = wave * 16 + fq * 4;
            const v4i* pp = prm2 + (c2 / 4) * 3;
            v4i acc0 = pp[2], acc1 = acc0;
#pragma unroll
            for (int ks = 0; ks < F2; ++ks) {
                const int ch = (ks * 4 + fq) ^ frow;
                acc0 = mma_step(fs[F1 - 2 + ks], tile[frow * CPRW + ch], acc0);
                acc1 = mma_step(fs[F1 - 2 + ks], tile[(16 + frow) * CPRW + ch], acc1);
            }
            const float lo2 = B.relu2 ? 0.f : -3.0e38f;
            const float off2 = B.out_u8_2 ? 0.f : 128.f;
            const unsigned xm2 = B.out_u8_2 ? 0u : 0x80808080u;
            const unsigned o0 = chain_out_pack(acc0, z, __builtin_bit_cast(v4f, pp[1]), __builtin_bit_cast(v4f, pp[0]), lo2, off2, xm2);
            const unsigned o1 = chain_out_pack(acc1, z, __builtin_bit_cast(v4f, pp[1]), __builtin_bit_cast(v4f, pp[0]), lo2, off2, xm2);
            if (ok0) *(unsigned*)((char*)ka.y2[k] + (size_t)p0 * K2 + c2) = o0;
            if (ok1) *(unsigned*)((char*)ka.y2[k] + (size_t)p1 * K2 + c2) = o1;
        }
        SABER_TL(6);
        if (k + 1 < ka.nblk) {
            asm volatile("s_waitcnt vmcnt(0)" ::: "memory");
            __builtin_amdgcn_s_barrier();
            unsigned long long* const e_k = e_up + (k & 1);
            if (wave == 0 && lane == 0) {
                (void)__hip_atomic_fetch_add(e_k, 1ull, __ATOMIC_RELAXED, __HIP_MEMORY_SCOPE_WORKGROUP);
                (void)__hip_atomic_fetch_add(e_k + 16, 1ull, __ATOMIC_RELAXED, __HIP_MEMORY_SCOPE_WORKGROUP);
            }
            dma_prm(Bn);
            if (wave == 0) {
                const unsigned long long one = (unsigned long long)ka.tiles_x;
                coop_wait_mask2(e_k, (ty > 0 ? 2 * one : one) - 1, e_k + 16, (ty + 1 < tile_rows ? 2 * one : one) - 1, ka.err);
            }
            __builtin_amdgcn_s_barrier();
            dma_halo(ka.y2[k], true);
            wait_vm_older_than<0>();
            __builtin_amdgcn_s_barrier();
            B = Bn;
            SABER_TL(7);
        }
    }
    if (tid == 0 && ka.err) {
        const unsigned first = (unsigned)L2Reader(ka.xcc).load16((unsigned)(n * ka.tiles_per_img) * 128u + 16u).x;
        if (first && first != my_xcc) __hip_atomic_fetch_add(ka.err, 1u, __ATOMIC_RELAXED, __HIP_MEMORY_SCOPE_SYSTEM);
    }
    SABER_TL_FLUSH();
}

template <int MAXB>
static hipError_t launch_stage1(const Stage4KArgs<MAXB>& ka, hipStream_t s) {
    if (ka.nblk <= 1 || ka.nblk > MAXB || ka.N <= 0 || !ka.blk || !ka.xcc || !ka.per_image || !ka.img_ctr ||
        (ka.tiles_x != 1 && ka.tiles_x != 2 && ka.tiles_x != 4))
        return hipErrorInvalidValue;
    const dim3 grid((ka.N + 7) / 8 * ka.tiles_per_img * 8), block(512);
    hipLaunchKernelGGL(conv_stage1_c128_kernel<MAXB>, grid, block, 0, s, ka);
    return hipGetLastError();
}
hipError_t launch_conv_stage1_c128(const Stage4KArgs<STAGE4_SHORT>& a, hipStream_t s) { return launch_stage1(a, s); }
hipError_t launch_conv_stage1_c128(const Stage4KArgs<STAGE4_LONG>& a, hipStream_t s) { return launch_stage1(a, s); }
template <int MAXB>
static hipError_t launch_stage4(const Stage4KArgs<MAXB>& ka, bool tail, bool head, hipStream_t s) {
    if (tail && (ka.nblk < 2 || ka.nblk + 1 > MAXB || !ka.y1[ka.nblk])) return hipErrorInvalidValue;
    if (head && (!ka.per_image || !ka.img_ctr || ka.tiles_x != 1 || !ka.head_y)) return hipErrorInvalidValue;
    if (ka.nblk <= 0 || ka.nblk > MAXB || ka.N <= 0 || !ka.blk || !ka.grp_ctr || !ka.xch || !ka.xcc ||
        (ka.nblk > 1 && (!ka.per_image || !ka.img_ctr || ka.tiles_x != 1)))
        return hipErrorInvalidValue;
    const int tiles = ka.N * ka.tiles_per_img;
    const dim3 grid(ka.per_image ? (ka.N + 7) / 8 * ka.tiles_per_img * 4 * 8 : (tiles + 7) / 8 * 32), block(512);
    if (head && tail) hipLaunchKernelGGL((conv_stage4_c256_kernel<MAXB, true, true>), grid, block, 0, s, ka);
    else if (head) hipLaunchKernelGGL((conv_stage4_c256_kernel<MAXB, false, true>), grid, block, 0, s, ka);
    else if (tail) hipLaunchKernelGGL((conv_stage4_c256_kernel<MAXB, true, false>), grid, block, 0, s, ka);
    else hipLaunchKernelGGL((conv_stage4_c256_kernel<MAXB, false, false>), grid, block, 0, s, ka);
    return hipGetLastError();
}
hipError_t launch_conv_stage4(const Stage4KArgs<STAGE4_SHORT>& a, bool tail, bool head, hipStream_t s) { return launch_stage4(a, tail, head, s); }
hipError_t launch_conv_stage4(const Stage4KArgs<STAGE4_LONG>& a, bool tail, bool head, hipStream_t s) { return launch_stage4(a, tail, head, s); }

}
```

### anakin_amd/csrc/kernels.h

```cpp
#pragma once
#include <hip/hip_runtime.h>
#include <stddef.h>
#include <stdint.h>

#ifdef SABER_TIMELINE
extern __device__ unsigned long long* saber_tl_buf;
#define SABER_TL_DECL unsigned long long tl_[16] = {0, 0, 0, 0, 0, 0, 0, 0, 0, 0, 0, 0, 0, 0, 0, 0}
#define SABER_TL(i) tl_[i] = wall_clock64()
#define SABER_TL_FLUSH()                                                                   \
    do {                                                                                   \
        if (threadIdx.x == 0 && saber_tl_buf)                                              \
            for (int i_ = 0; i_ < 16; ++i_) saber_tl_buf[(size_t)blockIdx.x * 16 + i_] = tl_[i_]; \
    } while (0)
#else
#define SABER_TL_DECL do { } while (0)
#define SABER_TL(i) do { } while (0)
#define SABER_TL_FLUSH() do { } while (0)
#endif

namespace saber_mi355x {

enum { DT_F32 = 0, DT_S8 = 1, DT_U8 = 2 };

enum {
    EPI_I8_CONV = 0,
    EPI_I8_FC_S8 = 1,
    EPI_I8_FC_U8 = 2,
    EPI_F32 = 3,
    EPI_I8_RAW_S32 = 4
};
enum { RES_NONE = 0, RES_SUM_INPLACE = 1, RES_ELTWISE = 2 };

struct ConvKArgs {
    const void* x;
    const void* w;
    const void* zero;
    int npx, nky;
    unsigned mg_npx;
    int Kg_pad;
    int M;
    int OH, OW;
    float inv_ohw, inv_ow;
    int H, W, C;
    int stride_h, stride_w, pad_h, pad_w, dil_h, dil_w;
    int kh, kw;
    int steps;
    int adv_c, adv_i, adv_j;
    int in_u8;
    int kw_pad;
    void* y;
    const void* res;
    const float* bias;
    const float* scale;
    const int* comp;
    int N, K;
    int Kg;
    int Cin;
    float qinv;
    int out_dtype;
    int out_nchw;
    int relu;
    float neg_slope;
    int epi;
    int res_mode, res_relu, res_dtype;
    float sum_scale, coeff_conv, coeff_res, scale_conv, scale_res;
    void* y2;
    int K1, K2, relu2, out_dtype2;
    int pool_oh, pool_ow;
    int res_sub, res_H, res_W;
    int w_plane_chunks;
    int ksplit_sh;
    float* part;
    unsigned* part_ctr;
    unsigned* part_err;
};

struct ImgKArgs {
    ConvKArgs c;
    int ib, rb, nw, nrs;
    unsigned mg[6];
};
static_assert(offsetof(ConvKArgs, y) == 128, "hot kernel arguments fill exactly the first two 64-byte lines");

struct StemPairTail {
    const void* w;
    const void* prm;
    void* y1;
    void* y2;
    int K1, K2;
    int relu1, relu2, u8_1, u8_2;
};
struct StemPairKArgs {
    ConvKArgs c;
    StemPairTail t;
};

constexpr int STAGE_MAX_TENSORS = 24;
struct ChainKArgs {
    const void* x;
    const void* wstream;
    const void* res;
    const void* prm1;
    const void* prm2;
    void* y1;
    void* y2;
    int M, in_u8;
    int relu1, res_relu;
    float coeff_conv, scale_conv, coeff_res, scale_res;
    int relu2, out_u8_2;
    const void* prm0;
    const void* zero;
    int N, H, W;
    int tiles_x, tiles_per_img;
    unsigned mg_tiles_x, mg_tpi;
    int in0_u8, relu0;
    int s0, H0, W0;
    int res_sub, res_H, res_W;
    void* y2b;
    int k2_split, relu2b, out_u8_2b;
};
struct CoopKArgs {
    ChainKArgs c;
    unsigned long long* coop_ctr;
    void* coop_xch;
    unsigned* coop_xcc;
    unsigned* coop_err;
    int n_tiles;
};
bool conv1x1_chain_ok(int c1, int k1, int k2);
hipError_t launch_conv1x1_chain(const ChainKArgs& a, int c1, int k1, int k2, int rows, int waves, int split, int with3x3, hipStream_t s);
hipError_t launch_conv_chain_coop(const CoopKArgs& a, hipStream_t s);

struct StageBlk {
    const void* wstream;
    const void* prm0;
    const void* prm1;
    const void* prm2;
    float coeff_conv, scale_conv, coeff_res, scale_res;
    int in0_u8, relu0, in_u8, relu1, res_relu, relu2, out_u8_2, pad_;
};
template <int MAXB>
struct Stage4KArgs {
    const void* x;
    const void* res;
    const void* zero;
    const StageBlk* blk;
    unsigned long long* grp_ctr;
    unsigned long long* img_ctr;
    void* xch;
    unsigned* xcc;
    unsigned* err;
    int nblk, N, H, W;
    int tiles_x, tiles_per_img;
    unsigned mg_tiles_x, mg_tpi, mg_wpi;
    int per_image;
    void* y1[MAXB];
    void* y2[MAXB];
    void* head_y;
};
constexpr int STAGE4_SHORT = 8, STAGE4_LONG = 24;
hipError_t launch_conv_stage4(const Stage4KArgs<STAGE4_SHORT>& a, bool tail, bool head, hipStream_t s);
hipError_t launch_conv_stage4(const Stage4KArgs<STAGE4_LONG>& a, bool tail, bool head, hipStream_t s);
hipError_t launch_conv_stage1_c128(const Stage4KArgs<STAGE4_SHORT>& a, hipStream_t s);
hipError_t launch_conv_stage1_c128(const Stage4KArgs<STAGE4_LONG>& a, hipStream_t s);

struct StagePhase {
    int type;
    int cin, cout;
    int in_t, out_t, res_t;
    int in_u8, relu, out_u8;
    int elt, res_relu;
    float coeff_conv, scale_conv, coeff_res, scale_res;
    unsigned w_chunk, prm_chunk;
    int barrier;
    int reload;
    unsigned pch, mg_pch;
    int red_chunk;
    int pool_t;
    float pool_idiv;
};
static_assert(sizeof(StagePhase) == 96, "StagePhase layout");
struct StageKArgs {
    const StagePhase* phases;
    const void* weights;
    const void* prm;
    const void* zero;
    unsigned long long* sync;
    int n_phases, n_barriers;
    int n_img, H, W;
    unsigned long long* trace;
    void* t[STAGE_MAX_TENSORS];
};
bool stage_xcd_type(int tiles_per_cu, int ksteps_per_wave, int is3x3, int* type);
hipError_t launch_stage_xcd(const StageKArgs& a, size_t lds_bytes, hipStream_t s);
hipError_t launch_img_conv(const StageKArgs& a, size_t lds_bytes, hipStream_t s);
struct GpoolKArgs {
    const void* x;
    void* y;
    const void* res;
    void* y_pool;
    const void* w;
    const void* prm;
    const void* zero;
    int n_img, hw, cout;
    int in_u8, relu, out_u8, elt, res_relu;
    float coeff_conv, scale_conv, coeff_res, scale_res;
    float pool_idiv;
};
bool conv1x1_gpool_ok(int cin, int cout, int hw);
hipError_t launch_conv1x1_gpool(const GpoolKArgs& a, hipStream_t s);

__device__ __forceinline__ void pin_hot_args(const ConvKArgs& a) {
    asm volatile("" ::"s"(a.x), "s"(a.w), "s"(a.zero), "s"(a.npx), "s"(a.nky), "s"(a.mg_npx), "s"(a.Kg_pad), "s"(a.M), "s"(a.OH),
                 "s"(a.OW), "s"(a.inv_ohw), "s"(a.inv_ow), "s"(a.H), "s"(a.W), "s"(a.C), "s"(a.stride_h), "s"(a.stride_w),
                 "s"(a.pad_h), "s"(a.pad_w), "s"(a.dil_h), "s"(a.dil_w), "s"(a.kh), "s"(a.kw), "s"(a.steps), "s"(a.in_u8));
}

enum { TILE_32x32 = 0, TILE_64x32 = 1, TILE_64x64 = 2, TILE_128x64 = 3, TILE_64x128 = 4, TILE_128x128 = 5,
       TILE_COUNT = 6,
       TILE_W8_64x64 = 6, TILE_W8_128x64 = 7, TILE_W8_128x128 = 8, TILE_W8_256x128 = 9, TILE_COUNT_B3 = 10 };
void tile_dims(int tile, int* bm_k, int* bn_pix);

hipError_t launch_conv_igemm(int mode, int tile, int ks, const ConvKArgs& a, hipStream_t s);
hipError_t launch_conv_igemm_dma(int mode, int tile, int ks, int wg, const ConvKArgs& a, hipStream_t s);
hipError_t launch_conv3x3_halo(int th, const ConvKArgs& a, hipStream_t s);
hipError_t launch_conv3x3_img(const ConvKArgs& a, int nw, int ib, int rb, hipStream_t s);
bool conv3x3_img_feasible(int C, int OW, int OH, int N, int nw, int ib, int rb);
bool conv3x3_b3h_variant(int variant, int* bmk, int* th, int* tm, int* threads);
bool conv1x1_pw_ok(int c, int k);
hipError_t launch_conv1x1_pw(const ConvKArgs& a, hipStream_t s);
bool conv1x1_pwk_variant(int v, int* tm, int* p, int* d, int* minb);
bool conv1x1_pwk_ok(int m, int c, int k);
hipError_t launch_conv1x1_pwk(int variant, const ConvKArgs& a, hipStream_t s);
hipError_t launch_conv3x3_b3h(int variant, const ConvKArgs& a, hipStream_t s);
hipError_t launch_fc_i8_small(const ConvKArgs& a, hipStream_t s);
bool fc_i8_small_ok(int m, int c, int kg_pad);
hipError_t launch_fc_f32_small(const ConvKArgs& a, bool packed, hipStream_t s);
int fc_f32_packed_steps(int c);
bool fc_f32_small_ok(int m, int c, int kg_pad);
bool fc_i8_small_softmax_ok(int m, int c, int kg_pad, int k);
hipError_t launch_fc_i8_small_softmax(const ConvKArgs& a, float* prob, unsigned* ctr, hipStream_t s);
bool fc_f32_splitk_ok(int m, int c, int kg_pad, int k, bool softmax);
size_t fc_f32_splitk_part_floats(int c, int k);
size_t fc_f32_splitk_counters(int k);
hipError_t launch_fc_f32_splitk(const ConvKArgs& a, float* part, unsigned* ctr, float* prob, hipStream_t s);
bool gemm_f32_rows_ok(int m, int k);
hipError_t launch_gemm_f32_rows(int m, int n, int k, float alpha, const float* A, const float* B, float beta, float* C, const void* zero,
                                hipStream_t s);
hipError_t launch_conv_stem(int f32_in, const ConvKArgs& a, hipStream_t s);
hipError_t launch_conv_stem_pool(int f32_in, const ConvKArgs& a, hipStream_t s);
hipError_t launch_conv_stem_pool_pair(int f32_in, const StemPairKArgs& a, hipStream_t s);
hipError_t launch_conv_direct(int is_f32, const ConvKArgs& a, int group, hipStream_t s);
constexpr int DW3X3_FORMS = 2;
const char* conv_dw3x3_form_name(int form, bool f32);
bool conv_dw3x3_ok(bool f32, int n, int c, int k, int group, int kh, int kw, int stride_h, int stride_w, int pad_h, int pad_w, int dil_h,
                   int dil_w, int oh, int ow);
hipError_t launch_conv_dw3x3(int form, bool f32, const ConvKArgs& a, hipStream_t s);
constexpr int G3X3_FORMS = 1;
const char* conv_group3x3_form_name(int form);
int conv_group3x3_steps(int cg);
bool conv_group3x3_ok(int n, int c, int k, int group, int kh, int kw, int stride_h, int stride_w, int pad_h, int pad_w, int dil_h, int dil_w,
                      int oh, int ow);
hipError_t launch_conv_group3x3(int form, const ConvKArgs& a, int group, hipStream_t s);

struct SepKArgs {
    const void* x;
    const void* wdw;
    const float* dw_bias;
    const float* dw_scale;
    const void* wpw;
    const void* prm;
    void* y_dw;
    void* y_pw;
    int N, H, W, C, OH, OW, K;
    int stride, pad;
    int tiles_x, tiles_per_img;
    int kgroups;
    int nslices;
    int dw_relu, mid_u8;
    int pw_relu, out_u8;
};
constexpr int SEP_MAX_CODE = 15;
bool conv_sep_form(int code, int* rows, int* kper, int* waves);
bool conv_sep_form_ok(int code, int c, int k);
size_t conv_sep_lds_bytes(int rows, int c);
void sep_pw_pack(const int8_t* w_kc, int k, int c, std::vector<uint8_t>& out);
hipError_t conv_sep_prepare();
hipError_t launch_conv_sep(int code, bool in_u8, const SepKArgs& a, hipStream_t s);

struct IrKArgs {
    const void* x;
    const void* we;
    const void* eprm;
    const void* wdw;
    const float* dw_bias;
    const float* dw_scale;
    const void* wp;
    const void* pprm;
    void* y_e;
    void* y_d;
    void* y;
    int N, H, W, Cin, Ce, OH, OW, Cout;
    int stride;
    int th, tw, nf;
    int hh, hw, hpf;
    int tiles_x, tiles_per_img;
    int out_u8, p_relu;
    int elt, res_relu;
    float coeff_conv, scale_conv, coeff_res, scale_res;
};
constexpr int IR_MAX_CODE = 7;
constexpr int IR_MAX_UNITS = 20;
constexpr size_t IR_LDS_LIMIT = 80 * 1024 - 64;
struct IrGeom { int th, tw, nf, hh, hw, hpf, tiles_x, tiles_y; size_t lds; };
const char* conv_ir_form_name(int code);
bool conv_ir_geom(int code, int cin, int ce, int cout, int oh, int ow, int stride, IrGeom* g);
void ir_pack(const int8_t* w_kc, int k, int c, std::vector<uint8_t>& out);
// ... 74 lines not shown
```

### anakin_amd/saber.py

```python
import ctypes as C

import numpy as np
import torch

from . import lib as L

_TORCH_DT = {L.F32: torch.float32, L.S8: torch.int8, L.U8: torch.uint8}


def _stream():
    return C.c_void_p(torch.cuda.current_stream().cuda_stream)


def _p(t):
    return None if t is None else C.c_void_p(t.data_ptr())


def _np_ptr(a):
    return None if a is None else a.ctypes.data_as(C.c_void_p)


def dtype_code(t):
    return {torch.float32: L.F32, torch.int8: L.S8, torch.uint8: L.U8}[t.dtype]

# ... 135 lines not shown
class SaberConv2DPooling:

    def __init__(self, int8=True):
        self.int8 = int8
        self.conv = SaberConv2D(int8)
        self.fused = False
        self.inner = None

    def init(self, in_shape_nchw, conv_param, pool_type, window, stride, pad, in_dtype, out_dtype, in_scale=1.0,
             out_scale=1.0, floor_mode=False, in_layout=None):
        if self.int8:
            self.conv.init(in_shape_nchw, conv_param, in_dtype, out_dtype, in_scale, out_scale, in_layout=in_layout)
        else:
            self.conv.init(in_shape_nchw, conv_param, L.F32, L.F32, in_layout=L.NHWC if in_layout is None else in_layout,
                           out_layout=L.NHWC)
        self.pool = (pool_type, tuple(window), tuple(stride), tuple(pad), floor_mode)
        n = in_shape_nchw[0]
        ch, cw = self.conv.out_hw
        rc = L.load().saber_hip_conv2d_set_pooling(self.conv.h, pool_type, window[0], window[1], stride[0], stride[1],
                                                   pad[0], pad[1], 1 if floor_mode else 0)
        if rc == 0:
            self.fused = True
            oh, ow = C.c_int(), C.c_int()
            L.load().saber_hip_conv2d_out_shape(self.conv.h, C.byref(oh), C.byref(ow))
            self.out_hw = (oh.value, ow.value)
        elif rc == L.UNIMPL:
            self.inner = torch.empty((n, ch, cw, self.conv.desc.k), dtype=_TORCH_DT[out_dtype], device="cuda")
            self.out_hw = pool_out_hw(ch, cw, pad, window, stride, floor_mode)
        else:
            L.check(rc)
        self.h = self.conv.h
        return self

    def new_output(self):
        d = self.conv.desc
        return torch.empty((d.n, self.out_hw[0], self.out_hw[1], d.k), dtype=_TORCH_DT[d.out_dtype], device="cuda")

    def algo(self):
        return self.conv.algo()

    def dispatch(self, x, y):
        if self.fused:
            return self.conv.dispatch(x, y)
        self.conv.dispatch(x, self.inner)
        pt, win, st, pd, _ = self.pool
        d = self.conv.desc
        n, ch, cw, k = self.inner.shape
        if not self.int8:
            L.check(L.load().saber_hip_pool2d_f32(n, ch, cw, k, self.out_hw[0], self.out_hw[1], win[0], win[1], st[0], st[1],
                                                  pd[0], pd[1], pt, L.NHWC, _p(self.inner), _p(y), _stream()))
            return y
        L.check(L.load().saber_hip_pool2d_i8_nhwc(n, ch, cw, k, self.out_hw[0], self.out_hw[1], win[0], win[1], st[0],
                                                  st[1], pd[0], pd[1], pt, d.out_dtype, d.out_dtype, _p(self.inner),
                                                  _p(y), _stream()))
        return y


class SaberConvPair:

    def __init__(self, a, b):
        self.a, self.b = a, b
        self.h = C.c_void_p()
        L.check(L.load().saber_hip_conv2d_create_pair(a.h, b.h, C.byref(self.h)))

    def dispatch(self, x, ya, yb):
        L.check(L.load().saber_hip_conv2d_run_pair(self.h, _p(x), _p(ya), _p(yb), _stream()))
        return ya, yb

    def algo(self):
        return L.load().saber_hip_conv2d_algo(self.h).decode()

    def set_tile(self, tile):
        L.check(L.load().saber_hip_conv2d_set_tile(self.h, tile))

    def autotune(self, x, ya, yb, iters=5):
        L.check(L.load().saber_hip_conv2d_autotune_pair(self.h, _p(x), _p(ya), _p(yb), _stream(), iters))

    def __del__(self):
        try:
            if self.h:
                L.load().saber_hip_conv2d_destroy(self.h)
        except Exception:
            pass


ACTIVE_SIGMOID, ACTIVE_RELU, ACTIVE_TANH, ACTIVE_CLIPPED_RELU, ACTIVE_ELU, ACTIVE_STANH, ACTIVE_PRELU, ACTIVE_GELU, ACTIVE_SWISH = \
    1, 2, 3, 4, 5, 9, 10, 11, 12


def activation(active, x, y=None, negative_slope=0.0, coef=1.0):
    import torch
    if y is None:
        y = torch.empty_like(x)
    L.check(L.load().saber_hip_activation_f32(int(active), x.numel(), float(negative_slope), float(coef), _p(x), _p(y), _stream()))
    return y


def prelu(x, slope, channels, inner, channel_shared=False, y=None):
    import torch
    if y is None:
        y = torch.empty_like(x)
    L.check(L.load().saber_hip_prelu_f32(x.numel(), int(channels), int(inner), int(bool(channel_shared)), _p(slope), _p(x), _p(y), _stream()))
    return y


class SaberConvChain:

    def __init__(self, a, b, conv3x3=None, pair_b=None):
        self.a, self.b, self.c3, self.b2 = a, b, conv3x3, pair_b
        self.h = C.c_void_p()
        if pair_b is not None:
            L.check(L.load().saber_hip_conv2d_chain_create3_pair(conv3x3.h, a.h, b.h, pair_b.h, C.byref(self.h)))
        elif conv3x3 is None:
            L.check(L.load().saber_hip_conv2d_chain_create(a.h, b.h, C.byref(self.h)))
        else:
            L.check(L.load().saber_hip_conv2d_chain_create3(conv3x3.h, a.h, None if b is None else b.h, C.byref(self.h)))

    def dispatch(self, x, res, ya, yb=None, yc=None):
        L.check(L.load().saber_hip_conv2d_chain_run3(self.h, _p(x), _p(res), _p(ya), _p(yb), _p(yc), _stream()))
        return ya, yb

    def set_tile(self, tn):
        L.check(L.load().saber_hip_conv2d_chain_set_tile(self.h, tn))

    def tile(self):
        return L.load().saber_hip_conv2d_chain_get_tile(self.h)

    def __del__(self):
        try:
            if self.h:
                L.load().saber_hip_conv2d_chain_destroy(self.h)
        except Exception:
            pass


class SaberChainStage:

    def __init__(self, chains, tail=None, head=None):
        self.chains = list(chains)
        self.tail = tail
        self.head = head
        arr = (C.c_void_p * len(chains))(*[c.h for c in chains])
        self.h = C.c_void_p()
        if head is not None:
            L.check(L.load().saber_hip_conv2d_stage_create_head(arr, len(chains), tail.h if tail is not None else None, head[0].h, head[1].h,
                                                                C.byref(self.h)))
        elif tail is None:
            L.check(L.load().saber_hip_conv2d_stage_create(arr, len(chains), C.byref(self.h)))
        else:
            L.check(L.load().saber_hip_conv2d_stage_create_tail(arr, len(chains), tail.h, C.byref(self.h)))

    def dispatch(self, x, res, y1s, y2s, y_tail=None):
        n = len(self.chains)
        a = (C.c_void_p * n)(*[t.data_ptr() for t in y1s])
        b = (C.c_void_p * n)(*[t.data_ptr() for t in y2s])
        if y_tail is None:
            L.check(L.load().saber_hip_conv2d_stage_run(self.h, _p(x), _p(res), a, b, _stream()))
        else:
            L.check(L.load().saber_hip_conv2d_stage_run_tail(self.h, _p(x), _p(res), a, b, _p(y_tail), _stream()))

    def dispatch_head(self, x_head, y_head_b, y1s, y2s, y_tail=None):
        n = len(self.chains)
        a = (C.c_void_p * n)(*[t.data_ptr() for t in y1s])
        b = (C.c_void_p * n)(*[t.data_ptr() for t in y2s])
        L.check(L.load().saber_hip_conv2d_stage_run_head(self.h, _p(x_head), _p(y_head_b), a, b, _p(y_tail) if y_tail is not None else None, _stream()))

    def __del__(self):
        try:
            if self.h:
                L.load().saber_hip_conv2d_stage_destroy(self.h)
        except Exception:
            pass


class SaberStemPair:

    def __init__(self, stem, a, b):
        self.ops = (stem, a, b)
        self.h = C.c_void_p()
        L.check(L.load().saber_hip_conv2d_stem_pair_create(stem.h, a.h, b.h, C.byref(self.h)))

    def dispatch(self, x, y_a, y_b, y_pool=None):
        stem = self.ops[0]
        ws = stem.ws if hasattr(stem, "ws") else stem.conv.ws
        L.check(L.load().saber_hip_conv2d_stem_pair_run(self.h, _p(x), _p(y_pool), _p(y_a), _p(y_b), _p(ws), _stream()))

    def __del__(self):
        try:
            if self.h:
                L.load().saber_hip_conv2d_stem_pair_destroy(self.h)
        except Exception:
            pass


class SaberConvSep:

    def __init__(self, dw, pw):
        self.ops = (dw, pw)
        self.h = C.c_void_p()
        L.check(L.load().saber_hip_conv2d_sep_create(dw.h, pw.h, C.byref(self.h)))

    def dispatch(self, x, y_pw, y_dw=None):
        L.check(L.load().saber_hip_conv2d_sep_run(self.h, _p(x), _p(y_dw), _p(y_pw), _stream()))
        return y_pw

    def set_tile(self, code):
        L.check(L.load().saber_hip_conv2d_sep_set_tile(self.h, code))

    def tile(self):
        return L.load().saber_hip_conv2d_sep_get_tile(self.h)

    def algo(self):
        return L.load().saber_hip_conv2d_sep_algo(self.h).decode()

    def __del__(self):
        try:
            if self.h:
                L.load().saber_hip_conv2d_sep_destroy(self.h)
        except Exception:
            pass


class SaberConvIR:

    def __init__(self, expand, dw, project):
        self.ops = (expand, dw, project)
        self.h = C.c_void_p()
        L.check(L.load().saber_hip_conv2d_ir_create(expand.h, dw.h, project.h, C.byref(self.h)))

    def dispatch(self, x, y, y_expand=None, y_dw=None):
        L.check(L.load().saber_hip_conv2d_ir_run(self.h, _p(x), _p(y_expand), _p(y_dw), _p(y), _stream()))
        return y

    def set_tile(self, code):
        L.check(L.load().saber_hip_conv2d_ir_set_tile(self.h, code))

    def tile(self):
        return L.load().saber_hip_conv2d_ir_get_tile(self.h)

    def algo(self):
        return L.load().saber_hip_conv2d_ir_algo(self.h).decode()

    def __del__(self):
        try:
            if self.h:
                L.load().saber_hip_conv2d_ir_destroy(self.h)
        except Exception:
            pass


class SaberConvFire:

    def __init__(self, squeeze, e1, e3):
        self.ops = (squeeze, e1, e3)
        self.h = C.c_void_p()
        L.check(L.load().saber_hip_conv2d_fire_create(squeeze.h, e1.h, e3.h, C.byref(self.h)))

    def dispatch(self, x, y, y_squeeze=None):
        L.check(L.load().saber_hip_conv2d_fire_run(self.h, _p(x), _p(y_squeeze), _p(y), _stream()))
        return y

    def set_tile(self, code):
        L.check(L.load().saber_hip_conv2d_fire_set_tile(self.h, code))

    def tile(self):
        return L.load().saber_hip_conv2d_fire_get_tile(self.h)

    def algo(self):
        return L.load().saber_hip_conv2d_fire_algo(self.h).decode()

    def __del__(self):
        try:
            if self.h:
                L.load().saber_hip_conv2d_fire_destroy(self.h)
        except Exception:
            pass


class SaberStage:

    def __init__(self, phases):
        self.convs = [p[0] for p in phases]
        arr = (L.StagePhase * len(phases))()
        for i, (c, a, b, r) in enumerate(phases):
            arr[i].conv, arr[i].in_, arr[i].out, arr[i].res = c.h, a, b, r
        self.h = C.c_void_p()
        L.check(L.load().saber_hip_stage_create(arr, len(phases), C.byref(self.h)))
        self.n = L.load().saber_hip_stage_num_tensors(self.h)

    def dispatch(self, tensors):
        ptrs = (C.c_void_p * self.n)(*[None if t is None else t.data_ptr() for t in tensors[:self.n]])
        L.check(L.load().saber_hip_stage_run(self.h, ptrs, self.n, _stream()))

    def trace(self, arm=False):
        if arm:
            return L.check_count(L.load().saber_hip_stage_trace(self.h, None, 0))
        n = 256 * len(self.convs) * 8
        out = np.zeros(n, np.uint64)
        L.check_count(L.load().saber_hip_stage_trace(self.h, _np_ptr(out), n))
        return out.reshape(256, len(self.convs), 8)

    def status(self):
        L.check(L.load().saber_hip_stage_status(self.h))

    def __del__(self):
        try:
            if self.h:
# ... 270 lines not shown
        return rc

    def add_conv_pair(self, pair, x, ya, yb):
        self.keep.append(pair)
        return self._chk(L.load().saber_hip_net_add_conv_pair(self.h, pair.h, self.tid(x), self.tid(ya), self.tid(yb)))

    def add_fc(self, fc, x, y):
        self.keep.append(fc)
        rc = L.load().saber_hip_net_add_fc(self.h, fc.h, self.tid(x), self.tid(y))
        if rc < 0:
            L.check(rc)
        return rc

    def _chk(self, rc):
        if rc < 0:
            L.check(rc)
        return rc

    def add_quantize(self, n, c, h, w, c_pad, out_dtype, scale, x, y):
        return self._chk(L.load().saber_hip_net_add_quantize(self.h, n, c, h, w, c_pad, out_dtype, float(scale),
                                                             self.tid(x), self.tid(y)))

    def add_dequantize(self, n, c, h, w, in_dtype, scale, x, y):
        return self._chk(L.load().saber_hip_net_add_dequantize(self.h, n, c, h, w, in_dtype, float(scale),
                                                               self.tid(x), self.tid(y)))

    def add_transpose_in(self, n, c, h, w, c_pad, x, y):
        return self._chk(L.load().saber_hip_net_add_transpose_in_f32(self.h, n, c, h, w, c_pad, self.tid(x), self.tid(y)))

    def add_eltwise_i8(self, count, sa, sb, c0, c1, relu, a, b, y):
        return self._chk(L.load().saber_hip_net_add_eltwise_i8(self.h, count, float(sa), float(sb), float(c0),
                                                               float(c1), int(relu), self.tid(a), self.tid(b), self.tid(y)))

    def add_eltwise_f32(self, count, c0, c1, relu, a, b, y):
        return self._chk(L.load().saber_hip_net_add_eltwise_f32(self.h, count, float(c0), float(c1), int(relu),
                                                                self.tid(a), self.tid(b), self.tid(y)))

    def add_pool_i8(self, n, h, w, c, oh, ow, win, stride, pad, ptype, in_dtype, out_dtype, x, y):
        return self._chk(L.load().saber_hip_net_add_pool_i8(self.h, n, h, w, c, oh, ow, win[0], win[1], stride[0],
                                                            stride[1], pad[0], pad[1], ptype, in_dtype, out_dtype,
                                                            self.tid(x), self.tid(y)))

    def add_pool_f32(self, n, h, w, c, oh, ow, win, stride, pad, ptype, layout, x, y):
        return self._chk(L.load().saber_hip_net_add_pool_f32(self.h, n, h, w, c, oh, ow, win[0], win[1], stride[0],
                                                             stride[1], pad[0], pad[1], ptype, layout, self.tid(x),
                                                             self.tid(y)))

    def add_pool_f32_from_i8(self, n, h, w, c, oh, ow, win, stride, pad, ptype, in_dtype, scale, x, y):
        return self._chk(L.load().saber_hip_net_add_pool_f32_from_i8(self.h, n, h, w, c, oh, ow, win[0], win[1],
                                                                     stride[0], stride[1], pad[0], pad[1], ptype,
                                                                     in_dtype, float(scale), self.tid(x), self.tid(y)))

    def add_pool_f32_from_i8_q(self, n, h, w, c, oh, ow, win, stride, pad, ptype, in_dtype, scale, x, y, q_scale, yq):
        return self._chk(L.load().saber_hip_net_add_pool_f32_from_i8_q(
            self.h, n, h, w, c, oh, ow, win[0], win[1], stride[0], stride[1], pad[0], pad[1], ptype, in_dtype,
            float(scale), self.tid(x), self.tid(y), float(q_scale), self.tid(yq)))

    def add_fc_q(self, fc, xq, y):
        self.keep.append(fc)
        return self._chk(L.load().saber_hip_net_add_fc_q(self.h, fc.h, self.tid(xq), self.tid(y)))

    def add_concat(self, names, out, concat=None):
        tids = [self.tid(nm) for nm in names]
        chans = [self.tensors[nm][1][-1] for nm in names]
        dt = self.tensors[out][2]
        code = L.F32 if dt == torch.float32 else (L.S8 if dt == torch.int8 else L.U8)
        pixels = int(np.prod(self.tensors[out][1][:-1]))
        n = len(names)
        m = None
        if concat is not None and concat.mult is not None:
            m = (C.c_float * n)(*[float(v) for v in concat.mult])
        return self._chk(L.load().saber_hip_net_add_concat(self.h, pixels, n, (C.c_int * n)(*tids), (C.c_int * n)(*chans), m, code, self.tid(out)))

    def add_softmax(self, rows, cols, x, y):
        return self._chk(L.load().saber_hip_net_add_softmax(self.h, rows, cols, self.tid(x), self.tid(y)))

    def set_lane(self, op_index, lane):
        L.check(L.load().saber_hip_net_set_lane(self.h, op_index, lane))

    def optimize(self, flags=15):
        rc = L.load().saber_hip_net_optimize(self.h, int(flags))
        if rc < 0:
            L.check(rc)
        return rc

    def finalize(self):
        L.check(L.load().saber_hip_net_finalize(self.h))
        self.finalized = True

    def tensor(self, name):
        tid, shape, dt = self.tensors[name]
        ptr = L.load().saber_hip_net_tensor_ptr(self.h, tid)
        n = int(np.prod(shape))
        nbytes = n * (4 if dt == torch.float32 else 1)
        holder = _RawCuda(ptr, nbytes)
        return torch.as_tensor(holder, device="cuda").view(dt).view(shape)

    def num_ops(self):
        return L.load().saber_hip_net_num_ops(self.h)

    def unwritten(self, name):
        return bool(L.load().saber_hip_net_tensor_unwritten(self.h, self.tensors[name][0]))

    def num_launches(self):
        return L.load().saber_hip_net_num_launches(self.h)

    def op_name(self, i):
        return L.load().saber_hip_net_op_name(self.h, i).decode()

    def run(self):
        L.check(L.load().saber_hip_net_run(self.h, _stream()))

    def run_op(self, i):
        L.check(L.load().saber_hip_net_run_op(self.h, i, _stream()))

    def capture(self):
        cur = torch.cuda.current_stream()
        if cur.cuda_stream == 0:
            side = torch.cuda.Stream()
            side.wait_stream(cur)
            with torch.cuda.stream(side):
                L.check(L.load().saber_hip_net_capture(self.h, _stream()))
            cur.wait_stream(side)
        else:
            L.check(L.load().saber_hip_net_capture(self.h, _stream()))

    def replay(self):
        L.check(L.load().saber_hip_net_replay(self.h, _stream()))

    def autotune(self, iters=5):
        L.check(L.load().saber_hip_net_autotune(self.h, _stream(), iters))

    def choices(self):
        lib = L.load()
        return [int(lib.saber_hip_net_get_choice(self.h, i)) for i in range(self.num_ops())]

    def set_choices(self, choices):
        lib = L.load()
        assert len(choices) == self.num_ops()
        for i, c in enumerate(choices):
            L.check(lib.saber_hip_net_set_choice(self.h, i, int(c)))

    def status(self):
        L.check(L.load().saber_hip_net_status(self.h))

    def coop_fallbacks(self):
        return L.load().saber_hip_net_coop_fallbacks(self.h)

    def stages(self):
        lib = L.load()
        out = []
        for i in range(self.num_ops()):
            n = int(lib.saber_hip_net_stage_blocks(self.h, i))
            if n:
                out.append((i, n, bool(int(lib.saber_hip_net_get_choice(self.h, i)) >> 30 & 1)))
        return out

    def select_stages(self, on):
        ch = self.choices()
        for i, _, _ in self.stages():
            ch[i] = (ch[i] | (1 << 30)) if on else (ch[i] & ~(1 << 30))
        self.set_choices(ch)

    def tails(self):
        ch = self.choices()
        return [(i, n) for i, n, on in self.stages() if on and (ch[i] >> 31) & 1]

    def select_tails(self, on):
        ch = self.choices()
        for i, _, sel in self.stages():
            if sel:
                v = ((ch[i] | (1 << 31)) if on else (ch[i] & ~(1 << 31))) & 0xffffffff
                ch[i] = v - (1 << 32) if v >> 31 else v
        self.set_choices(ch)

    def heads(self):
        lib = L.load()
        ch = self.choices()
        out = []
        for i, _, on in self.stages():
            p = int(lib.saber_hip_net_stage_head(self.h, i))
            if on and p >= 0 and (ch[p] >> 29) & 1:
                out.append((p, i))
        return out

    def select_heads(self, on):
        lib = L.load()
        ch = self.choices()
        for i, _, sel in self.stages():
            p = int(lib.saber_hip_net_stage_head(self.h, i))
            if sel and p >= 0:
                ch[p] = (ch[p] | (1 << 29)) if on else (ch[p] & ~(1 << 29))
        self.set_choices(ch)

    def time_ops(self, iters=20):
        out = (C.c_float * self.num_ops())()
        L.check(L.load().saber_hip_net_time_ops(self.h, _stream(), iters, out))
        return list(out)

    def time_op_in_pass(self, index, iters=20):
        out = C.c_float()
        L.check(L.load().saber_hip_net_time_op_in_pass(self.h, _stream(), int(index), int(iters), C.byref(out)))
        return float(out.value)

    def time_pass(self, iters=20):
        out = (C.c_float * self.num_ops())()
        L.check(L.load().saber_hip_net_time_pass(self.h, _stream(), iters, out))
        return list(out)

    def op_work(self, index):
        b, f = C.c_double(), C.c_double()
        L.check(L.load().saber_hip_net_op_work(self.h, int(index), C.byref(b), C.byref(f)))
        return b.value, f.value

    def arena_bytes(self):
        return L.load().saber_hip_net_arena_bytes(self.h)

    def compact(self, keep=()):
        ids = (C.c_int * max(1, len(keep)))(*[self.tensors[k][0] for k in keep])
        L.check(L.load().saber_hip_net_compact_arena(self.h, ids, len(keep)))
        return self.arena_bytes()

    def compacted(self):
        return bool(L.load().saber_hip_net_arena_compacted(self.h))

    def tensor_of_ptr(self, t):
        return int(L.load().saber_hip_net_tensor_of_ptr(self.h, t.data_ptr()))

    def bind(self, tid, t):
        self.keep.append(t)
        L.check(L.load().saber_hip_net_bind_tensor(self.h, int(tid), t.data_ptr()))

    def num_tensors(self):
        return int(L.load().saber_hip_net_num_tensors(self.h))


class Capture:

    def __init__(self, keep=()):
        self.net = None
        self._keep = list(keep)

    def __enter__(self):
        L.check(L.load().saber_hip_capture_begin())
        return self

    def __exit__(self, et, ev, tb):
        h = C.c_void_p()
        rc = L.load().saber_hip_capture_end(C.byref(h))
        if et is None:
            L.check(rc)
            net = Net.__new__(Net)
            net.h, net.keep, net.tensors, net.finalized = h, list(self._keep), {}, False
            self.net = net
        elif h:
            L.load().saber_hip_net_destroy(h)
        return False

    def __del__(self):
        try:
            if self.h:
                L.load().saber_hip_net_destroy(self.h)
        except Exception:
            pass


class _RawCuda:
    def __init__(self, ptr, nbytes):
        self.__cuda_array_interface__ = {"shape": (nbytes,), "typestr": "|u1", "data": (int(ptr), False),
                                         "version": 2}
```

Measured before the change: 39200.

## Add cooperative multi-block stage kernel for C=64 ResNet stage

Adds a persistent cooperative kernel that runs all stage-1 (C=64) bottleneck blocks of an image in one launch, with per-XCD image placement and neighbour-tile halo synchronisation through counters. Weight streams are packed for the C=64 form, and intermediate y1 outputs that are only read inside the stage are kept private and not written to memory. Stage forming, autotune and the Python helpers are extended to expose these stages. The aim is to remove per-block launch overhead and global round trips. The risks are spin-wait and occupancy dependence, and that the stage is off unless autotune selects it.

```diff
diff --git a/anakin_amd/csrc/api_chain.hip b/anakin_amd/csrc/api_chain.hip
--- a/anakin_amd/csrc/api_chain.hip
+++ b/anakin_amd/csrc/api_chain.hip
@@ -141,6 +141,14 @@
         for (int ks = 0; ks < 2; ++ks)
             for (int mf = 0; mf < 4; ++mf) pack_frag1(a->wq_oihw.data(), C, w * 64, 4, mf, ks, out);
         for (int ks = 0; ks < 8; ++ks) pack_frag1(b->wq_oihw.data(), K1, w * 16, 1, 0, ks, out);
+    }
+}
+void pack_stage1_c64_stream(const int8_t* w3, const int8_t* wa, const int8_t* wb, std::vector<uint8_t>& out) {
+    const int C = 64, K1 = 256;
+    for (int w = 0; w < 4; ++w) {
+        for (int tap = 0; tap < 9; ++tap) pack_frag3(w3, C, w * 16, tap, 0, out);
+        for (int mf = 0; mf < 4; ++mf) pack_frag1(wa, C, w * 64, 4, mf, 0, out);
+        for (int ks = 0; ks < 4; ++ks) pack_frag1(wb, K1, w * 16, 1, 0, ks, out);
     }
 }
 int saber_hip_conv2d_stem_pair_create(saber_hip_conv_t* stem, const saber_hip_conv_t* a, const saber_hip_conv_t* b, saber_hip_stem_pair_t** out) {
@@ -237,14 +245,14 @@
         if (tail->a->d.res_stride != 2) return fail(SABER_HIP_INVALID_VALUE, "stage: the tail's shortcut must be sub-sampled by 2");
     }
     if (n > 1 && !per_image) return fail(SABER_HIP_INVALID_VALUE, "stage: several blocks need an image per XCD");
-    if (n < 2 && chains[0] && chains[0]->c1 == 128) return fail(SABER_HIP_INVALID_VALUE, "stage: at C = 128 a stage is at least two blocks");
+    if (n < 2 && chains[0] && (chains[0]->c1 == 128 || chains[0]->c1 == 64)) return fail(SABER_HIP_INVALID_VALUE, "stage: at C = 128 / 64 a stage is at least two blocks");
     const saber_hip_chain* c0 = chains[0];
     std::vector<saber_mi355x::StageBlk> blk;
     for (int k = 0; k < n; ++k) {
         const saber_hip_chain* ch = chains[k];
-        const uint8_t* stream = !ch ? nullptr : (ch->c1 == 256 ? ch->d_stream[CS_COOP4].p : (ch->c1 == 128 ? ch->d_stream_stage1.p : nullptr));
+        const uint8_t* stream = !ch ? nullptr : (ch->c1 == 256 ? ch->d_stream[CS_COOP4].p : (ch->c1 == 128 || ch->c1 == 64 ? ch->d_stream_stage1.p : nullptr));
         if (!ch || ch->c1 != c0->c1 || !ch->c3 || !ch->b || !stream || ch->c3->d.stride_h != 1)
-            return fail(SABER_HIP_INVALID_VALUE, "stage: every block must be a conv3x3 (stride 1) + conv1x1 + conv1x1 chain at C = 256 (or all at C = 128)");
+            return fail(SABER_HIP_INVALID_VALUE, "stage: every block must be a conv3x3 (stride 1) + conv1x1 + conv1x1 chain at C = 256 (or all at C = 128, or all at C = 64)");
         const saber_hip_conv_desc& da = ch->a->d;
         if (da.n != c0->a->d.n || da.h != c0->a->d.h || da.w != c0->a->d.w) return fail(SABER_HIP_INVALID_VALUE, "stage: blocks of one tensor shape");
         if (k && ((ch->c3->x_dtype == DT_U8) != (chains[k - 1]->b->d.out_dtype == SABER_HIP_U8)))
@@ -274,12 +282,13 @@
     st->tiles_per_img = st->tiles_x * ((d0.h + 1) / 2);
     st->per_image = per_image;
     const int wg_per_tile = st->c1 == 256 ? 4 : 1;
-    const bool fits = d0.n <= 8 && st->tiles_per_img * wg_per_tile <= 32 &&
+    const int wg_per_cu = st->c1 == 64 ? saber_mi355x::conv_stage1_c64_blocks_per_cu() : 1;
+    const bool fits = d0.n <= 8 && st->tiles_per_img * wg_per_tile <= 32 * wg_per_cu &&
                       (st->c1 == 256 ? st->tiles_x == 1 : (st->tiles_x == 1 || st->tiles_x == 2 || st->tiles_x == 4));
-    if ((per_image && !fits) || (st->c1 == 128 && !per_image)) {
+    if ((per_image && !fits) || (st->c1 != 256 && !per_image)) {
         delete st;
-        return fail(SABER_HIP_INVALID_VALUE, "stage: an image per XCD needs batch <= 8 and <= 32 workgroups per image (C = 256: width <= 16, <= 8 tiles "
-                    "of 2 x 16 pixels; C = 128: width <= 64, <= 32 tiles)");
+        return fail(SABER_HIP_INVALID_VALUE, "stage: an image per XCD needs batch <= 8 and every workgroup of an image resident on its XCD's 32 CUs (C = 256: "
+                    "width <= 16, <= 8 tiles of 2 x 16 pixels; C = 128: width <= 64, <= 32 tiles; C = 64: width <= 64, <= 32 x the kernel's workgroups per CU)");
     }
     const size_t tiles = (size_t)d0.n * st->tiles_per_img;
     hipError_t e = hipSuccess;
@@ -341,7 +350,8 @@
     for (int i = 0; i < k.nblk; ++i) { k.y1[i] = y1[i]; k.y2[i] = y2[i]; }
     if (y_tail) k.y1[k.nblk] = y_tail;
     k.head_y = y_head;
-    HIP_TRY(st->c1 == 256 ? saber_mi355x::launch_conv_stage4(k, y_tail != nullptr, y_head != nullptr, s) : saber_mi355x::launch_conv_stage1_c128(k, s));
+    HIP_TRY(st->c1 == 256 ? saber_mi355x::launch_conv_stage4(k, y_tail != nullptr, y_head != nullptr, s)
+                          : (st->c1 == 128 ? saber_mi355x::launch_conv_stage1_c128(k, s) : saber_mi355x::launch_conv_stage1_c64(k, s)));
     return SABER_HIP_OK;
 }
 int stage_run(saber_hip_chain_stage* st, const void* x, const void* res, void* const* y1, void* const* y2, hipStream_t s, void* y_tail, void* y_head) {
@@ -375,7 +385,7 @@
     if (g_capture) return capture_unsupported("saber_hip_conv2d_stage_run (saber_hip_net_optimize forms stages itself)");
     if (!st || !x || !res || !y1 || !y2) return fail(SABER_HIP_INVALID_VALUE, "null argument");
     for (size_t i = 0; i < st->chains.size(); ++i)
-        if (!y1[i] || !y2[i]) return fail(SABER_HIP_INVALID_VALUE, "stage: an output pointer per block");
+        if ((!y1[i] && !(st->c1 == 64 && i + 1 < st->chains.size())) || !y2[i]) return fail(SABER_HIP_INVALID_VALUE, "stage: an output pointer per block");
     return stage_run(st, x, res, y1, y2, (hipStream_t)stream);
 }
 int saber_hip_conv2d_stage_run_tail(saber_hip_chain_stage_t* st, const void* x, const void* res, void* const* y1, void* const* y2, void* y_tail,
@@ -500,9 +510,10 @@
         if (e == hipSuccess) e = hipHostMalloc((void**)&ch->h_coop_err, sizeof(unsigned), hipHostMallocMapped);
         if (e == hipSuccess) *ch->h_coop_err = 0u;
     }
-    if (e == hipSuccess && da.c == 128 && c3 && b && c3->d.stride_h == 1 && xcd_round_robin()) {
+    if (e == hipSuccess && (da.c == 128 || da.c == 64) && c3 && b && !pair2 && c3->d.stride_h == 1 && xcd_round_robin()) {
         std::vector<uint8_t> s1;
-        pack_stage1_c128_stream(c3, a, b, s1);
+        if (da.c == 128) pack_stage1_c128_stream(c3, a, b, s1);
+        else pack_stage1_c64_stream(c3->wq_oihw.data(), a->wq_oihw.data(), b->wq_oihw.data(), s1);
         e = ch->d_stream_stage1.upload(s1);
     }
     if (e == hipSuccess) e = ch->d_prm1.upload(p1);
diff --git a/anakin_amd/csrc/api_internal.h b/anakin_amd/csrc/api_internal.h
--- a/anakin_amd/csrc/api_internal.h
+++ b/anakin_amd/csrc/api_internal.h
@@ -373,6 +373,7 @@
     int tail_of = -1;
     bool head_on = false;
     int head_of = -1;
+    bool stage_y1_private = false;
     saber_hip_stem_pair* stem_pair = nullptr;
     int stem_y1 = -1, stem_y2 = -1;
     saber_hip_sep* sep = nullptr;
diff --git a/anakin_amd/csrc/api_net.hip b/anakin_amd/csrc/api_net.hip
--- a/anakin_amd/csrc/api_net.hip
+++ b/anakin_amd/csrc/api_net.hip
@@ -21,7 +21,7 @@
             void* y2[saber_mi355x::STAGE4_LONG];
             const NetOp* ops = &o;
             for (int k = 0; k < o.stage_n; ++k) {
-                y1[k] = T(ops[3 * k].chain3_y1);
+                y1[k] = ops[3 * k].stage_y1_private ? nullptr : T(ops[3 * k].chain3_y1);
                 y2[k] = T(ops[3 * k].chain3_y2);
             }
             void* const y_tail = o.tail_on ? T(ops[3 * o.stage_n].chain3_y1) : nullptr;
@@ -665,6 +665,7 @@
         if (o.out == id && (o.launch == LAUNCH_IR || (o.skip && by == LAUNCH_IR && (int)(&o - net->ops.data()) == o.absorbed_by + 1))) return 1;
         if (o.out == id && o.kind == OP_CONV && (o.launch == LAUNCH_FIRE || (o.skip && by == LAUNCH_FIRE))) return 1;
         if (o.launch == LAUNCH_STAGE && o.head_on && o.chain3_res == id) return 1;
+        if (o.chain3 && o.stage_y1_private && o.chain3_y1 == id && (o.launch == LAUNCH_STAGE || (o.skip && by == LAUNCH_STAGE))) return 1;
     }
     return 0;
 }
@@ -699,12 +700,17 @@
 }
 int saber_hip_net_inject_coop_error(saber_hip_net_t* net) {
     if (!net) return fail(SABER_HIP_INVALID_VALUE, "null argument");
+    auto res2 = [](const NetOp& o) { return o.stage && o.stage->c1 == 64; };
     for (NetOp& o : net->ops)
-        if (o.stage && o.stage_on && o.stage->h_err) { *(volatile unsigned*)o.stage->h_err = 1u; return SABER_HIP_OK; }
+        if (o.stage && !res2(o) && o.stage_on && o.stage->h_err) { *(volatile unsigned*)o.stage->h_err = 1u; return SABER_HIP_OK; }
+    for (NetOp& o : net->ops)
+        if (res2(o) && o.stage_on && o.stage->h_err) { *(volatile unsigned*)o.stage->h_err = 1u; return SABER_HIP_OK; }
     for (NetOp& o : net->ops) {
-        if (o.stage && o.stage->h_err) { *(volatile unsigned*)o.stage->h_err = 1u; return SABER_HIP_OK; }
+        if (o.stage && !res2(o) && o.stage->h_err) { *(volatile unsigned*)o.stage->h_err = 1u; return SABER_HIP_OK; }
         if (o.chain3 && o.chain3->h_coop_err) { *(volatile unsigned*)o.chain3->h_coop_err = 1u; return SABER_HIP_OK; }
     }
+    for (NetOp& o : net->ops)
+        if (res2(o) && o.stage->h_err) { *(volatile unsigned*)o.stage->h_err = 1u; return SABER_HIP_OK; }
     return fail(SABER_HIP_INVALID_VALUE, "the net has no cooperative launch site");
 }
 int saber_hip_net_num_launches(const saber_hip_net_t* net) {
diff --git a/anakin_amd/csrc/api_net_autotune.hip b/anakin_amd/csrc/api_net_autotune.hip
--- a/anakin_amd/csrc/api_net_autotune.hip
+++ b/anakin_amd/csrc/api_net_autotune.hip
@@ -24,7 +24,8 @@
 }
 int saber_hip_net_stage_blocks(const saber_hip_net_t* net, int index) {
     if (!net || index < 0 || index >= (int)net->ops.size()) return 0;
-    return net->ops[index].stage ? net->ops[index].stage_n : 0;
+    const NetOp& o = net->ops[index];
+    return o.stage ? (o.stage->c1 == 64 ? -o.stage_n : o.stage_n) : 0;
 }
 int saber_hip_net_stage_head(const saber_hip_net_t* net, int index) {
     if (!net || index < 1 || index >= (int)net->ops.size() || !net->ops[index].stage) return -1;
@@ -277,7 +278,7 @@
             else if (ok_h && wh < one * 0.99f) one = wh;
             else net_set_head(net, first, false);
         }
-        if (!ok || one >= sep) {
+        if (!ok || one >= sep * (H0.stage->c1 == 64 ? 0.99f : 1.f)) {
             *(volatile unsigned*)H0.stage->h_err = 0u;
             net_set_stage(net, first, false);
             for (int k = 0; k < H0.stage_n; ++k) {
diff --git a/anakin_amd/csrc/api_net_optimize.hip b/anakin_amd/csrc/api_net_optimize.hip
--- a/anakin_amd/csrc/api_net_optimize.hip
+++ b/anakin_amd/csrc/api_net_optimize.hip
@@ -540,7 +540,7 @@
         for (size_t i = 0; i + 2 < ops.size();) {
             auto block_ok = [&](size_t j) {
                 return j + 2 < ops.size() && ops[j].chain3 && ops[j].chain3->b && !ops[j].stage && ops[j].chain3_y2 >= 0 &&
-                       ((ops[j].chain3->c1 == 256 && ops[j].chain3->stage1) || (ops[j].chain3->c1 == 128 && ops[j].chain3->d_stream_stage1.p));
+                       ((ops[j].chain3->c1 == 256 && ops[j].chain3->stage1) || ((ops[j].chain3->c1 == 128 || ops[j].chain3->c1 == 64) && ops[j].chain3->d_stream_stage1.p));
             };
             if (!block_ok(i)) { ++i; continue; }
             std::vector<saber_hip_chain*> run{ops[i].chain3};
@@ -579,6 +579,8 @@
                     int before = 0;
                     for (size_t k = 0; k < run.size(); ++k) before += 3 - (ops[i + 3 * k].skip + ops[i + 3 * k + 1].skip + ops[i + 3 * k + 2].skip);
                     if (tail) before += 2 - (ops[jt].skip + ops[jt + 1].skip);
+                    if (run[0]->c1 == 64)
+                        for (size_t k = 0; k + 1 < run.size(); ++k) ops[i + 3 * k].stage_y1_private = readers(ops[i + 3 * k].chain3_y1) == 2;
                     const bool on = run[0]->a->d.n >= 4 && run[0]->c1 == 256;
                     net_set_stage(net, (int)i, on);
                     if (on) removed += before - 1;
diff --git a/anakin_amd/csrc/conv_stage_coop.hip b/anakin_amd/csrc/conv_stage_coop.hip
--- a/anakin_amd/csrc/conv_stage_coop.hip
+++ b/anakin_amd/csrc/conv_stage_coop.hip
@@ -768,16 +768,288 @@
 }
 
 template <int MAXB>
-static hipError_t launch_stage1(const Stage4KArgs<MAXB>& ka, hipStream_t s) {
+__global__ __launch_bounds__(256, 4) void conv_stage1_c64_kernel(const Stage4KArgs<MAXB> ka) {
+    constexpr int C1 = 64, K1 = 4 * C1, K2 = C1, NW = C1 / 16, NT = NW * 64;
+    constexpr int KS = C1 / 64;
+    constexpr int F0 = 9 * KS, F1 = 4 * KS, F2 = K1 / 64;
+    constexpr int FS = F1 - 2;
+    constexpr int PF = 7;
+    constexpr int CH1 = C1 / 16, PCH = CH1 + 1, HW = 18, HP = 4 * HW;
+    constexpr int HCH = (HP * PCH + 63) / 64 * 64;
+    constexpr int CPRW = K1 / 16;
+    constexpr int P0C = (C1 / 4 * 3 + 63) / 64 * 64, P1C = K1 / 4 * 3, P2C = (K2 / 4 * 3 + 63) / 64 * 64;
+    constexpr int MPC = C1 / 16 + 1;
+    static_assert(P1C % 64 == 0 && (32 * CPRW) % NT == 0, "DMA granularity");
+    __shared__ v4i halo[HCH];
+    __shared__ v4i tile[32 * CPRW];
+    __shared__ v4i mid[32 * MPC];
+    __shared__ v4i prm0[P0C];
+    __shared__ v4i prm1[P1C];
+    __shared__ v4i prm2[P2C];
+    SABER_TL_DECL;
+    SABER_TL(0);
+    const int tid = threadIdx.x, lane = tid & 63;
+    const int wave = __builtin_amdgcn_readfirstlane(tid >> 6);
+    const int frow = lane & 15, fq = lane >> 4;
+    const int b = blockIdx.x;
+    const int slot = b >> 3;
+    const int il = ka.mg_tpi ? (int)__umulhi((unsigned)slot, ka.mg_tpi) : slot;
+    const int rem = slot - il * ka.tiles_per_img;
+    const int n = il * 8 + (b & 7);
+    if (n >= ka.N) return;
+    const int t = n * ka.tiles_per_img + rem;
+    const int ty = ka.mg_tiles_x ? (int)__umulhi((unsigned)rem, ka.mg_tiles_x) : rem;
+    const int x0 = (rem - ty * ka.tiles_x) * 16, y0 = ty * 2;
+    const int tile_rows = ka.tiles_per_img / ka.tiles_x;
+    const int H = ka.H, W = ka.W;
+    auto pix = [&](int m, bool& ok) -> int {
+        int x = x0 + (m & 15), y = y0 + (m >> 4);
+        ok = x < W && y < H;
+        x = x < W ? x : W - 1;
+        y = y < H ? y : H - 1;
+        return (n * H + y) * W + x;
+    };
+    unsigned long long* const e_up = ka.img_ctr + ((size_t)n * (ka.tiles_per_img + 1) + ty) * 16;
+
+    auto per_block = [](int v) -> int {
+        asm volatile("" : "+v"(v));
+        return v;
+    };
+    typedef const __attribute__((address_space(4))) StageBlk* CBlk;
+    const CBlk cblk = (CBlk)ka.blk;
+    struct EltCoeff { float coeff_conv, scale_conv, coeff_res, scale_res; };
+    auto dma_halo = [&](const void* x, bool l2) {
+        const char* xg = (const char*)x;
+        for (int i = wave; i < HCH / 64; i += NW) {
+            const int L = i * 64 + per_block(lane);
+            const int hp = L / PCH, cc = L - hp * PCH;
+            const int hy = hp / HW, hx = hp - hy * HW;
+            const int gy = y0 - 1 + hy, gx = x0 - 1 + hx;
+            const bool in = hp < HP && cc < CH1 && (unsigned)gy < (unsigned)H && (unsigned)gx < (unsigned)W;
+            const char* src = in ? xg + ((size_t)((n * H + gy) * W + gx) * C1 + cc * 16) : (const char*)ka.zero;
+            if (l2 && in) lds_dma16_l2(src, halo + i * 64);
+            else lds_dma16(src, halo + i * 64);
+        }
+    };
+    auto dma_prm = [&](int k) {
+        for (int i = wave; i < P0C / 64; i += NW) lds_dma16((const v4i*)cblk[k].prm0 + i * 64 + lane, prm0 + i * 64);
+        for (int i = wave; i < P1C / 64; i += NW) lds_dma16((const v4i*)cblk[k].prm1 + i * 64 + lane, prm1 + i * 64);
+        for (int i = wave; i < P2C / 64; i += NW) lds_dma16((const v4i*)cblk[k].prm2 + i * 64 + lane, prm2 + i * 64);
+    };
+    auto stream_of = [&](const void* wstream) -> const v4i* {
+        return (const v4i*)wstream + (size_t)wave * ((F0 + F1 + F2) * 64) + lane;
+    };
+
+    dma_halo(ka.x, false);
+    for (int i = wave; i < 32 * CPRW / 64; i += NW) {
+        const int L = i * 64 + lane;
+        const int px = L / CPRW, c = (L % CPRW) ^ (px & 15);
+        bool okp;
+        const int pp_ = pix(px, okp);
+        lds_dma16((const char*)ka.res + (size_t)pp_ * K1 + c * 16, tile + i * 64);
+    }
+    dma_prm(0);
+    asm volatile("" ::: "memory");
+    v4i fr[F0 + 2];
+    {
+        const v4i* wsb = stream_of(cblk[0].wstream);
+#pragma unroll
+        for (int r = 0; r < PF; ++r) {
+            fr[r] = wsb[r * 64];
+            asm volatile("" ::: "memory");
+        }
+    }
+    wait_vm_older_than<PF>();
+    __builtin_amdgcn_s_barrier();
+    SABER_TL(1);
+    unsigned my_xcc;
+    asm volatile("s_getreg_b32 %0, hwreg(HW_REG_XCC_ID)" : "=s"(my_xcc));
+    my_xcc = (my_xcc & 7u) + 1u;
+    if (rem == 0 && tid == 0) ka.xcc[(size_t)t * 32 + 4] = my_xcc;
+
+    for (int k = 0; k < ka.nblk; ++k) {
+        const v4i z = {0, 0, 0, 0};
+        const auto& B = cblk[k];
+        v4i fs[FS + F2];
+        {
+            const v4i* wsb = stream_of(cblk[k].wstream);
+#pragma unroll
+            for (int r = PF; r < F0 + 2; ++r) {
+                fr[r] = wsb[r * 64];
+                asm volatile("" ::: "memory");
+            }
+#pragma unroll
+            for (int r = 0; r < FS; ++r) {
+                fs[r] = wsb[(F0 + 2 + r) * 64];
+                asm volatile("" ::: "memory");
+            }
+        }
+        {
+            const int xm0 = B.in0_u8 ? (int)0x80808080u : 0;
+            const int c0 = wave * 16 + fq * 4;
+            const v4i* pp = prm0 + (c0 / 4) * 3;
+            v4i acc0 = pp[2], acc1 = acc0;
+            const v4i* hb = halo + frow * PCH + fq;
+#pragma unroll
+            for (int s = 0; s < F0; ++s) {
+                const int kl = s % KS, tap = s / KS;
+                const int dy = tap / 3, dx = tap % 3;
+                v4i b0 = hb[(dy * HW + dx) * PCH + kl * 4];
+                v4i b1 = hb[((dy + 1) * HW + dx) * PCH + kl * 4];
+                b0.x ^= xm0; b0.y ^= xm0; b0.z ^= xm0; b0.w ^= xm0;
+                b1.x ^= xm0; b1.y ^= xm0; b1.z ^= xm0; b1.w ^= xm0;
+                acc0 = mma_step(fr[s], b0, acc0);
+                acc1 = mma_step(fr[s], b1, acc1);
+            }
+            const float lo0 = B.relu0 ? 0.f : -3.0e38f;
+            const float off0 = B.in_u8 ? 0.f : 128.f;
+            const unsigned xo0 = B.in_u8 ? 0u : 0x80808080u;
+            const unsigned o0 = chain_out_pack(acc0, z, __builtin_bit_cast(v4f, pp[1]), __builtin_bit_cast(v4f, pp[0]), lo0, off0, xo0);
+            const unsigned o1 = chain_out_pack(acc1, z, __builtin_bit_cast(v4f, pp[1]), __builtin_bit_cast(v4f, pp[0]), lo0, off0, xo0);
+            *(unsigned*)((char*)mid + frow * (MPC * 16) + c0) = o0;
+            *(unsigned*)((char*)mid + (16 + frow) * (MPC * 16) + c0) = o1;
+        }
+        asm volatile("s_waitcnt lgkmcnt(0)" ::: "memory");
+        __builtin_amdgcn_s_barrier();
+        SABER_TL(2);
+
+        {
+            const int ln = per_block(lane), frow = ln & 15, fq = ln >> 4;
+            const int xmask = B.in_u8 ? (int)0x80808080u : 0;
+            const int cg = wave * 64 + fq * 16;
+            const v4i* pp = prm1 + (cg / 4) * 3;
+            v4i acc[2][4];
+#pragma unroll
+            for (int m = 0; m < 2; ++m)
+#pragma unroll
+                for (int mf = 0; mf < 4; ++mf) acc[m][mf] = pp[mf * 3 + 2];
+#pragma unroll
+            for (int ks = 0; ks < KS; ++ks)
+#pragma unroll
+                for (int m = 0; m < 2; ++m) {
+                    v4i bo = mid[(m * 16 + frow) * MPC + ks * 4 + fq];
+                    bo.x ^= xmask; bo.y ^= xmask; bo.z ^= xmask; bo.w ^= xmask;
+#pragma unroll
+                    for (int mf = 0; mf < 4; ++mf) {
+                        const int f = ks * 4 + mf;
+                        acc[m][mf] = mma_step(f < 2 ? fr[F0 + f] : fs[f - 2], bo, acc[m][mf]);
+                    }
+                }
+            {
+                const v4i* wsb = stream_of(cblk[k].wstream);
+#pragma unroll
+                for (int r = FS; r < FS + F2; ++r) {
+                    fs[r] = wsb[(F0 + 2 + r) * 64];
+                    asm volatile("" ::: "memory");
+                }
+            }
+            const float lo_s8 = B.relu1 ? 0.f : -128.f;
+            const float res_lo = B.res_relu ? 0.f : -3.0e38f;
+            const EltCoeff ec = {B.coeff_conv, B.scale_conv, B.coeff_res, B.scale_res};
+#pragma unroll
+            for (int m = 0; m < 2; ++m) {
+                v4i* tp = tile + (m * 16 + frow) * CPRW + ((cg / 16) ^ frow);
+                const v4i rs = *tp;
+                v4i o;
+                o.x = (int)chain_elt_pack(acc[m][0], z, __builtin_bit_cast(v4f, pp[1]), __builtin_bit_cast(v4f, pp[0]), (unsigned)rs.x, lo_s8, res_lo, ec);
+                o.y = (int)chain_elt_pack(acc[m][1], z, __builtin_bit_cast(v4f, pp[4]), __builtin_bit_cast(v4f, pp[3]), (unsigned)rs.y, lo_s8, res_lo, ec);
+                o.z = (int)chain_elt_pack(acc[m][2], z, __builtin_bit_cast(v4f, pp[7]), __builtin_bit_cast(v4f, pp[6]), (unsigned)rs.z, lo_s8, res_lo, ec);
+                o.w = (int)chain_elt_pack(acc[m][3], z, __builtin_bit_cast(v4f, pp[10]), __builtin_bit_cast(v4f, pp[9]), (unsigned)rs.w, lo_s8, res_lo, ec);
+                *tp = o;
+            }
+        }
+        asm volatile("s_waitcnt lgkmcnt(0)" ::: "memory");
+        __builtin_amdgcn_s_barrier();
+        if (ka.y1[k]) {
+#pragma unroll
+        for (int j = 0; j < 32 * CPRW / NT; ++j) {
+            const int L = per_block(tid) + j * NT;
+            const int px = L / CPRW, c = (L % CPRW) ^ (px & 15);
+            bool okp;
+            const int pp_ = pix(px, okp);
+            if (okp) *(v4i*)((char*)ka.y1[k] + (size_t)pp_ * K1 + c * 16) = tile[L];
+        }
+        }
+        SABER_TL(4);
+        if (k + 1 < ka.nblk) {
+            const v4i* wsb = stream_of(cblk[k + 1].wstream);
+#pragma unroll
+            for (int r = 0; r < PF; ++r) {
+                fr[r] = wsb[r * 64];
+                asm volatile("" ::: "memory");
+            }
+        }
+
+        {
+            const int ln = per_block(lane), frow = ln & 15, fq = ln >> 4;
+            bool ok0, ok1;
+            const int p0 = pix(frow, ok0), p1 = pix(16 + frow, ok1);
+            const int c2 = wave * 16 + fq * 4;
+            const v4i* pp = prm2 + (c2 / 4) * 3;
+            v4i acc0 = pp[2], acc1 = acc0;
+#pragma unroll
+            for (int ks = 0; ks < F2; ++ks) {
+                const int ch = (ks * 4 + fq) ^ frow;
+                acc0 = mma_step(fs[FS + ks], tile[frow * CPRW + ch], acc0);
+                acc1 = mma_step(fs[FS + ks], tile[(16 + frow) * CPRW + ch], acc1);
+            }
+            const float lo2 = B.relu2 ? 0.f : -3.0e38f;
+            const float off2 = B.out_u8_2 ? 0.f : 128.f;
+            const unsigned xm2 = B.out_u8_2 ? 0u : 0x80808080u;
+            const unsigned o0 = chain_out_pack(acc0, z, __builtin_bit_cast(v4f, pp[1]), __builtin_bit_cast(v4f, pp[0]), lo2, off2, xm2);
+            const unsigned o1 = chain_out_pack(acc1, z, __builtin_bit_cast(v4f, pp[1]), __builtin_bit_cast(v4f, pp[0]), lo2, off2, xm2);
+            if (ok0) *(unsigned*)((char*)ka.y2[k] + (size_t)p0 * K2 + c2) = o0;
+            if (ok1) *(unsigned*)((char*)ka.y2[k] + (size_t)p1 * K2 + c2) = o1;
+        }
+        SABER_TL(6);
+        if (k + 1 < ka.nblk) {
+            asm volatile("s_waitcnt vmcnt(0)" ::: "memory");
+            __builtin_amdgcn_s_barrier();
+            unsigned long long* const e_k = e_up + (k & 1);
+            if (wave == 0 && lane == 0) {
+                (void)__hip_atomic_fetch_add(e_k, 1ull, __ATOMIC_RELAXED, __HIP_MEMORY_SCOPE_WORKGROUP);
+                (void)__hip_atomic_fetch_add(e_k + 16, 1ull, __ATOMIC_RELAXED, __HIP_MEMORY_SCOPE_WORKGROUP);
+            }
+            dma_prm(k + 1);
+            if (wave == 0) {
+                const unsigned long long one = (unsigned long long)ka.tiles_x;
+                coop_wait_mask2(e_k, (ty > 0 ? 2 * one : one) - 1, e_k + 16, (ty + 1 < tile_rows ? 2 * one : one) - 1, ka.err);
+            }
+            __builtin_amdgcn_s_barrier();
+            dma_halo(ka.y2[k], true);
+            wait_vm_older_than<0>();
+            __builtin_amdgcn_s_barrier();
+            SABER_TL(7);
+        }
+    }
+    if (tid == 0 && ka.err) {
+        const unsigned first = (unsigned)L2Reader(ka.xcc).load16((unsigned)(n * ka.tiles_per_img) * 128u + 16u).x;
+        if (first && first != my_xcc) __hip_atomic_fetch_add(ka.err, 1u, __ATOMIC_RELAXED, __HIP_MEMORY_SCOPE_SYSTEM);
+    }
+    SABER_TL_FLUSH();
+}
+
+template <int MAXB>
+static hipError_t launch_stage1(const Stage4KArgs<MAXB>& ka, int c1, hipStream_t s) {
     if (ka.nblk <= 1 || ka.nblk > MAXB || ka.N <= 0 || !ka.blk || !ka.xcc || !ka.per_image || !ka.img_ctr ||
         (ka.tiles_x != 1 && ka.tiles_x != 2 && ka.tiles_x != 4))
         return hipErrorInvalidValue;
-    const dim3 grid((ka.N + 7) / 8 * ka.tiles_per_img * 8), block(512);
-    hipLaunchKernelGGL(conv_stage1_c128_kernel<MAXB>, grid, block, 0, s, ka);
+    const dim3 grid((ka.N + 7) / 8 * ka.tiles_per_img * 8);
+    if (c1 == 64) hipLaunchKernelGGL(conv_stage1_c64_kernel<MAXB>, grid, dim3(256), 0, s, ka);
+    else hipLaunchKernelGGL(conv_stage1_c128_kernel<MAXB>, grid, dim3(512), 0, s, ka);
     return hipGetLastError();
 }
-hipError_t launch_conv_stage1_c128(const Stage4KArgs<STAGE4_SHORT>& a, hipStream_t s) { return launch_stage1(a, s); }
-hipError_t launch_conv_stage1_c128(const Stage4KArgs<STAGE4_LONG>& a, hipStream_t s) { return launch_stage1(a, s); }
+hipError_t launch_conv_stage1_c128(const Stage4KArgs<STAGE4_SHORT>& a, hipStream_t s) { return launch_stage1(a, 128, s); }
+hipError_t launch_conv_stage1_c128(const Stage4KArgs<STAGE4_LONG>& a, hipStream_t s) { return launch_stage1(a, 128, s); }
+hipError_t launch_conv_stage1_c64(const Stage4KArgs<STAGE4_SHORT>& a, hipStream_t s) { return launch_stage1(a, 64, s); }
+hipError_t launch_conv_stage1_c64(const Stage4KArgs<STAGE4_LONG>& a, hipStream_t s) { return launch_stage1(a, 64, s); }
+int conv_stage1_c64_blocks_per_cu() {
+    int nb = 0;
+    if (hipOccupancyMaxActiveBlocksPerMultiprocessor(&nb, conv_stage1_c64_kernel<STAGE4_SHORT>, 256, 0) != hipSuccess) return 0;
+    int nl = 0;
+    if (hipOccupancyMaxActiveBlocksPerMultiprocessor(&nl, conv_stage1_c64_kernel<STAGE4_LONG>, 256, 0) != hipSuccess) return 0;
+    return nb < nl ? nb : nl;
+}
 template <int MAXB>
 static hipError_t launch_stage4(const Stage4KArgs<MAXB>& ka, bool tail, bool head, hipStream_t s) {
     if (tail && (ka.nblk < 2 || ka.nblk + 1 > MAXB || !ka.y1[ka.nblk])) return hipErrorInvalidValue;
diff --git a/anakin_amd/csrc/kernels.h b/anakin_amd/csrc/kernels.h
--- a/anakin_amd/csrc/kernels.h
+++ b/anakin_amd/csrc/kernels.h
@@ -163,6 +163,9 @@
 hipError_t launch_conv_stage4(const Stage4KArgs<STAGE4_LONG>& a, bool tail, bool head, hipStream_t s);
 hipError_t launch_conv_stage1_c128(const Stage4KArgs<STAGE4_SHORT>& a, hipStream_t s);
 hipError_t launch_conv_stage1_c128(const Stage4KArgs<STAGE4_LONG>& a, hipStream_t s);
+hipError_t launch_conv_stage1_c64(const Stage4KArgs<STAGE4_SHORT>& a, hipStream_t s);
+hipError_t launch_conv_stage1_c64(const Stage4KArgs<STAGE4_LONG>& a, hipStream_t s);
+int conv_stage1_c64_blocks_per_cu();
 
 struct StagePhase {
     int type;
diff --git a/anakin_amd/saber.py b/anakin_amd/saber.py
--- a/anakin_amd/saber.py
+++ b/anakin_amd/saber.py
@@ -311,7 +311,7 @@
 
     def dispatch(self, x, res, y1s, y2s, y_tail=None):
         n = len(self.chains)
-        a = (C.c_void_p * n)(*[t.data_ptr() for t in y1s])
+        a = (C.c_void_p * n)(*[t.data_ptr() if t is not None else None for t in y1s])
         b = (C.c_void_p * n)(*[t.data_ptr() for t in y2s])
         if y_tail is None:
             L.check(L.load().saber_hip_conv2d_stage_run(self.h, _p(x), _p(res), a, b, _stream()))
@@ -888,9 +888,24 @@
         out = []
         for i in range(self.num_ops()):
             n = int(lib.saber_hip_net_stage_blocks(self.h, i))
-            if n:
+            if n > 0:
                 out.append((i, n, bool(int(lib.saber_hip_net_get_choice(self.h, i)) >> 30 & 1)))
         return out
+
+    def stages_c64(self):
+        lib = L.load()
+        out = []
+        for i in range(self.num_ops()):
+            n = int(lib.saber_hip_net_stage_blocks(self.h, i))
+            if n < 0:
+                out.append((i, -n, bool(int(lib.saber_hip_net_get_choice(self.h, i)) >> 30 & 1)))
+        return out
+
+    def select_stages_c64(self, on):
+        ch = self.choices()
+        for i, _, _ in self.stages_c64():
+            ch[i] = (ch[i] | (1 << 30)) if on else (ch[i] & ~(1 << 30))
+        self.set_choices(ch)
 
     def select_stages(self, on):
         ch = self.choices()
```

Measured after the change: 39890 (median of 6 runs). 1.8% higher.
